# HSG-AIML/MaskedSST

Measured on AMD Instinct MI355X. Metric: pretrain samples/sec, higher is better.
Workload: dtype bf16; 1 GPU; SimMIM pretrain step (fwd+bwd+AdamW), EnMAP-shape cubes 8x8x200, depth 12x2, dim 96, heads 8, mlp 64, mask 0.7/4/tube, dropout 0.1; global_batch=256, per_gpu_batch=256, parallelism=dp1

## Files before the change

include/msst.h:

```cpp
#ifndef MSST_H
#define MSST_H
#include <stdint.h>

#ifdef __cplusplus
extern "C" {
#endif

#define MSST_VERSION 109
#define MSST_DIM 96
#define MSST_DIM_HEAD 64
#define MSST_MLP 64

#define MSST_PREC_F32 0
#define MSST_PREC_BF16 1

#define MSST_KERNEL_GENERIC (16 << 8)
#define MSST_KERNEL_FWD_4WAVE (64 << 8)
#define MSST_X1_BF16 (1024 << 8)
#define MSST_FWD_HALF (4096 << 8)
#define MSST_LSE_RENORM (8192 << 8)
#define MSST_LN1_FROM_XN (2048 << 8)
#define MSST_BWD_DEFER_REDUCE (512 << 8)
#define MSST_KERNEL_ATTN_R3 (128 << 8)

// ... 37 lines not shown
} MsstBlockWeights;

int msst_tokenize_fwd(const float* img, const float* pre_g, const float* pre_b, const float* w_emb,
                      const float* b_emb, const float* post_g, const float* post_b, const float* pos_a,
                      const float* pos_b, int pos_split, const float* mask_token, const uint8_t* mask,
                      float* out, int B, int S, int N, int P, float emb_dropout_p, uint32_t seed, void* stream);

int msst_tokenize_scene_fwd(const float* scene, const float* pre_g, const float* pre_b, const float* w_emb,
                            const float* b_emb, const float* post_g, const float* post_b, const float* pos_a,
                            const float* pos_b, int pos_split, float* out, int Bs, int Hs, int Ws, int window, int stride,
                            long win0, int nwin, int S, int P, void* stream);

int msst_tokenize_scene_fwd_train(const float* scene, const float* pre_g, const float* pre_b, const float* w_emb,
                                  const float* b_emb, const float* post_g, const float* post_b, const float* pos_a,
                                  const float* pos_b, int pos_split, float* out, int Bs, int Hs, int Ws, int window, int stride,
                                  long win0, int nwin, int S, int P, float emb_dropout_p, uint32_t seed, void* stream);
int msst_tokenize_scene_bwd(const float* scene, const float* pre_g, const float* pre_b, const float* w_emb,
                            const float* b_emb, const float* post_g, const float* post_b, const float* dx0, float* slab,
                            int nchunk, float* dpre_g, float* dpre_b, float* dw_emb, float* db_emb, float* dpost_g,
                            float* dpost_b, float* dpos_a, float* dpos_b, int pos_split, int Bs, int Hs, int Ws, int window,
                            int stride, long win0, int nwin, int S, int P, float emb_dropout_p, uint32_t seed, void* stream);

int msst_scene_assemble(const float* win_logits, long win0, int nwin, float* logits, int64_t* classes, int Bs,
                        int n_classes, int Hs, int Ws, int window, int stride, int finalize, void* stream);

int msst_tokenize_scene_fwd_masked(const float* scene, const float* pre_g, const float* pre_b, const float* w_emb,
                                   const float* b_emb, const float* post_g, const float* post_b, const float* pos_a,
                                   const float* pos_b, int pos_split, const float* mask_token, const uint8_t* scene_mask, float* out,
                                   int Bs, int Hs, int Ws, int window, int stride, long win0, int nwin, int S, int P, void* stream);

int msst_scene_recon_assemble(const float* win_recon, long win0, int nwin, const float* scene, const uint8_t* scene_mask, float* cube,
                              double* band_err , int32_t* band_cnt , int32_t* cover, int Bs, int S, int P,
                              int Hs, int Ws, int window, int stride, int finalize, int blend, void* stream);

int msst_pool_spectral_fwd(const float* y, float* out, int B, int S, int N, void* stream);

int msst_scene_embed_assemble(const float* win_feat, long win0, int nwin, float* feat, int32_t* cover, int Bs, int D, int Hs, int Ws,
                              int window, int stride, int finalize, int l2norm, void* stream);

#define MSST_SAVED_XN 1
#define MSST_SAVED_LSE 2
#define MSST_SAVED_RSTD 4
long msst_block_lse_floats(int mode, int B, int S, int N, int heads);
long msst_block_tiles(int mode, int B, int S, int N);
int msst_block_fwd(const MsstBlockWeights* w , const float* x, float* y, float* x1, int mode,
                   int B, int S, int N, int heads, int prec, int max_grid, float dropout_p, uint32_t seed,
                   int layer, void* xn_out, float* lse_out, int* saved , void* stream);

int msst_block_fwd_stack(const MsstBlockWeights* const* w , int nblk, const float* x0, float* const* y ,
                         float* const* x1 , void* const* xn_out , float* const* lse_out , int mode,
                         int B, int S, int N, int heads, int prec, int max_grid, float dropout_p, uint32_t seed, int layer0,
                         int* saved , void* stream);

int msst_head_fwd(const float* y, const float* img, const int32_t* idx, const float* w_pix,
                  const float* b_pix, int per_block, float* dpred, float* pred, float* partial,
                  float* loss, int B, int S, int N, int P, int K, void* stream);

int msst_recon_fwd(const float* y, const float* img, const uint8_t* mask, const float* w_pix, const float* b_pix, int per_block,
                   int blend, float* recon, double* band_err , int32_t* band_cnt , int B, int S, int N,
                   int P, void* stream);


int msst_head_bwd(const float* y, const float* dpred, const int32_t* csr_ptr, const int32_t* csr_pos,
                  const float* w_pix, int per_block, float gscale, const float* gout, float* dy, float* slab,
                  int nchunk, float* dw_pix, float* db_pix, int B, int S, int N, int P, int K, void* stream);

typedef struct MsstBlockGrads {
    float* ln1_g; float* ln1_b; float* wqkv; float* wout; float* bo;
    float* ln2_g; float* ln2_b; float* w1; float* b1; float* w2; float* b2;
} MsstBlockGrads;

#define MSST_MLP_SLAB (64 * 96 + 96 * 64 + 64 + 96 + 96 + 96)
#define MSST_ATTN_SLAB (3 * 64 * 96 + 96 * 64)
#define MSST_LN1_SLAB 288

int msst_block_bwd(const MsstBlockWeights* w , const MsstBlockGrads* g , const float* x,
                   const float* x1, const float* dy, float* dx, float* dx1, void* dxn_part, float* slab,
                   int grid_rows, int nchunk, int mode, int B, int S, int N, int heads, int prec,
                   float dropout_p, uint32_t seed, int layer, const void* xn_saved ,
                   const float* lse_saved ,
                   void* dab_ws ,
                   void* stream);

#define MSST_TILE_QUEUE_WORDS 64
int msst_block_bwd_chain(const MsstBlockWeights* w , const MsstBlockGrads* g ,
                         const MsstBlockWeights* w_prev , const MsstBlockGrads* g_prev ,
                         const float* x, const float* x1, const float* x1_prev, const float* dy, float* dx, float* dx1,
                         void* dxn_part, float* slab, int grid_rows, int nchunk, int mode, int B, int S, int N, int heads,
                         int prec, float dropout_p, uint32_t seed, int layer, const void* xn_saved, const float* lse_saved ,
                         void* dab_ws, int first, int32_t* tile_queue , void* stream);

int msst_block_bwd_reduce(const MsstBlockGrads* g , const MsstBlockGrads* g_prev ,
                          float* slab, long slab_stride, long grad_stride, int count, int count_prev, int first,
                          int grid_rows, int nchunk, int mode, int B, int S, int N, int heads, int prec, void* stream);

int msst_tokenize_bwd(const float* img, const float* pre_g, const float* pre_b, const float* w_emb,
                      const float* b_emb, const float* post_g, const float* post_b, const uint8_t* mask,
                      const float* dx0, float* slab, int nchunk, float* dpre_g, float* dpre_b,
                      float* dw_emb, float* db_emb, float* dpost_g, float* dpost_b, float* dpos_a,
                      float* dpos_b, int pos_split, float* dmask_token, int B, int S, int N, int P,
                      float emb_dropout_p, uint32_t seed, void* stream);

int msst_tokenize_bwd_input(const float* img, const float* pre_g, const float* pre_b, const float* w_emb, const float* b_emb,
                            const float* post_g, const float* post_b, const uint8_t* mask , const float* dx0,
                            const float* dtarget , float* dimg, int B, int S, int N, int P, float emb_dropout_p,
                            uint32_t seed, void* stream);
int msst_head_bwd_target(const float* dpred, const int32_t* csr_ptr, const int32_t* csr_pos, const float* gout ,
                         float* dtarget, int B, int S, int N, int P, int K, void* stream);
int msst_tokenize_scene_bwd_input(const float* scene, const float* pre_g, const float* pre_b, const float* w_emb, const float* b_emb,
                                  const float* post_g, const float* post_b, const float* dx0, float* dscene, int Bs, int Hs, int Ws,
                                  int window, int stride, long win0, int nwin, int S, int P, float emb_dropout_p, uint32_t seed,
                                  void* stream);

int msst_cls_head_fwd(const float* y, const float* ln_g, const float* ln_b, const float* w, const float* b,
                      float* logits, int B, int S, int N, int n_classes, void* stream);
int msst_cls_head_bwd(const float* y, const float* dlogits, const float* ln_g, const float* ln_b, const float* w,
                      float* dy, float* slab, float* dln_g, float* dln_b, float* dw, float* db, int B, int S,
                      int N, int n_classes, void* stream);

int msst_spec_head_fwd(const float* y, const float* ln_g, const float* ln_b, const float* w, const float* b,
                       float* logits, int B, int S, int N, int n_classes, void* stream);
long msst_spec_head_bwd_slab(int B, int S, int N, int n_classes);
int msst_spec_head_bwd(const float* y, const float* dlogits, const float* ln_g, const float* ln_b, const float* w,
                       float* dy, float* slab, float* dln_g, float* dln_b, float* dw, float* db, int B, int S,
                       int N, int n_classes, void* stream);

long msst_pix_head_fwd_ws(int B, int N);
int msst_pix_head_fwd(const float* y, const float* ln_g, const float* ln_b, const float* w, const float* b, float* logits,
                      float* ws, int B, int S, int N, int n_classes, void* stream);
long msst_pix_head_bwd_slab(int B, int S, int N, int n_classes);
int msst_pix_head_bwd(const float* y, const float* dlogits, const float* ln_g, const float* ln_b, const float* w, float* dy,
                      float* slab, float* dln_g, float* dln_b, float* dw, float* db, int B, int S, int N, int n_classes,
                      void* stream);

int msst_scene_centre_assemble(const float* win_logits, long win0, int nwin, float* logits, int64_t* classes, int Bs,
                               int n_classes, int Hs, int Ws, int window, int stride, int finalize, void* stream);

int msst_layernorm_fwd(const float* x, const float* gamma, const float* beta, float* y, float* mean ,
                       float* rstd , long rows, int D, float eps, void* stream);
long msst_layernorm_bwd_slab(long rows, int D);
int msst_layernorm_bwd(const float* x, const float* gamma, const float* dy, float* dx, float* dgamma, float* dbeta,
                       float* slab, long rows, int D, float eps, void* stream);

// ... 54 lines not shown
```

maskedsst_amd/_lib.py:

```python
import ctypes
import os
from ctypes import c_int, c_int32, c_uint32, c_long, c_float, c_void_p, c_char_p, POINTER, Structure

HERE = os.path.dirname(os.path.abspath(__file__))
LIB_PATH = os.path.join(HERE, "libmsst.so")
HEADER_PATH = os.path.normpath(os.path.join(HERE, "..", "include", "msst.h"))

PREC_F32 = 0
PREC_BF16 = 1
MODE_SPATIAL = 0
MODE_SPECTRAL = 1
MLP_SLAB = 64 * 96 + 96 * 64 + 64 + 96 + 96 + 96
ATTN_SLAB = 3 * 64 * 96 + 96 * 64
LN1_SLAB = 288


class MsstError(RuntimeError):
    pass


class MsstPrepJob(Structure):
    _fields_ = [("src", c_void_p), ("dst", c_void_p), ("rows", c_int32), ("cols", c_int32),
                ("transpose", c_int32), ("pack", c_int32), ("scale_rows", c_int32), ("scale", c_float)]


class MsstBlockWeights(Structure):
    _fields_ = [("struct_bytes", ctypes.c_uint64)] + [(n, c_void_p) for n in (
        "wqkv", "wout", "w1", "w2", "wqkvT", "woutT", "w1T", "w2T",
        "ln1_g", "ln1_b", "bo", "ln2_g", "ln2_b", "b1", "b2", "wqkv32", "woutT32", "wqkvT32",
        "wqkv_h", "wout_h", "w1_h", "w2_h")]


class MsstBlockGrads(Structure):
    _fields_ = [(n, c_void_p) for n in (
        "ln1_g", "ln1_b", "wqkv", "wout", "bo", "ln2_g", "ln2_b", "w1", "b1", "w2", "b2")]


class MsstAdamGroup(Structure):
    _fields_ = [("start", c_long), ("end", c_long), ("lr", c_float), ("weight_decay", c_float), ("step", c_int), ("flags", c_int)]


_P = c_void_p
ADAM_DECOUPLED = 1
ADAM_MAX_GROUPS = 64
BWD_DEFER_REDUCE = 512 << 8
X1_BF16 = 1024 << 8
SAVED_XN, SAVED_LSE, SAVED_RSTD = 1, 2, 4
LN1_FROM_XN = 2048 << 8
FWD_HALF = 4096 << 8
LSE_RENORM = 8192 << 8
PREP_HALF = 256
CE_LOSS_SUM, CE_N_VALID, CE_N_CORRECT, CE_BAD_LABELS, CE_NONFINITE, CE_SUPPORT = range(6)
CE_EXT_LOSS_SUM, CE_EXT_WEIGHT_SUM = range(2)
CE_CONFUSION_MAX_CLASSES = 128
_SIGS = {
    "msst_version": (c_int, []),
    "msst_last_error": (c_char_p, []),
    "msst_prep_weights": (c_int, [_P, c_int, c_int, c_int, c_int, _P, _P]),
    "msst_tokenize_fwd": (c_int, [_P] * 9 + [c_int, _P, _P, _P, c_int, c_int, c_int, c_int, c_float, c_uint32, _P]),
    "msst_tokenize_scene_fwd": (c_int, [_P] * 9 + [c_int, _P, c_int, c_int, c_int, c_int, c_int, c_long, c_int, c_int, c_int, _P]),
    "msst_tokenize_scene_fwd_train": (c_int, [_P] * 9 + [c_int, _P, c_int, c_int, c_int, c_int, c_int, c_long, c_int, c_int, c_int,
                                              c_float, c_uint32, _P]),
    "msst_tokenize_scene_bwd": (c_int, [_P] * 9 + [c_int] + [_P] * 8 + [c_int] * 6 + [c_long, c_int, c_int, c_int, c_float, c_uint32, _P]),
    "msst_tokenize_bwd_input": (c_int, [_P] * 11 + [c_int] * 4 + [c_float, c_uint32, _P]),
    "msst_head_bwd_target": (c_int, [_P] * 5 + [c_int] * 5 + [_P]),
    "msst_tokenize_scene_bwd_input": (c_int, [_P] * 9 + [c_int] * 5 + [c_long, c_int, c_int, c_int, c_float, c_uint32, _P]),
    "msst_tokenize_scene_fwd_masked": (c_int, [_P] * 9 + [c_int, _P, _P, _P, c_int, c_int, c_int, c_int, c_int, c_long, c_int, c_int, c_int, _P]),
    "msst_scene_recon_assemble": (c_int, [_P, c_long, c_int, _P, _P, _P, _P, _P, _P] + [c_int] * 9 + [_P]),
    "msst_pool_spectral_fwd": (c_int, [_P, _P, c_int, c_int, c_int, _P]),
    "msst_scene_embed_assemble": (c_int, [_P, c_long, c_int, _P, _P] + [c_int] * 8 + [_P]),
    "msst_scene_assemble": (c_int, [_P, c_long, c_int, _P, _P, c_int, c_int, c_int, c_int, c_int, c_int, c_int, _P]),
    "msst_cls_head_fwd": (c_int, [_P] * 6 + [c_int, c_int, c_int, c_int, _P]),
    "msst_cls_head_bwd": (c_int, [_P] * 11 + [c_int, c_int, c_int, c_int, _P]),
    "msst_spec_head_fwd": (c_int, [_P] * 6 + [c_int, c_int, c_int, c_int, _P]),
    "msst_spec_head_bwd_slab": (c_long, [c_int, c_int, c_int, c_int]),
    "msst_spec_head_bwd": (c_int, [_P] * 11 + [c_int, c_int, c_int, c_int, _P]),
    "msst_pix_head_fwd_ws": (c_long, [c_int, c_int]),
    "msst_pix_head_fwd": (c_int, [_P] * 7 + [c_int, c_int, c_int, c_int, _P]),
    "msst_pix_head_bwd_slab": (c_long, [c_int, c_int, c_int, c_int]),
    "msst_pix_head_bwd": (c_int, [_P] * 11 + [c_int, c_int, c_int, c_int, _P]),
    "msst_scene_centre_assemble": (c_int, [_P, c_long, c_int, _P, _P, c_int, c_int, c_int, c_int, c_int, c_int, c_int, _P]),
    "msst_block_lse_floats": (c_long, [c_int, c_int, c_int, c_int, c_int]),
    "msst_block_tiles": (c_long, [c_int, c_int, c_int, c_int]),
    "msst_block_fwd": (c_int, [POINTER(MsstBlockWeights), _P, _P, _P, c_int, c_int, c_int, c_int, c_int,
                               c_int, c_int, c_float, c_uint32, c_int, _P, _P, POINTER(c_int), _P]),
    "msst_block_fwd_stack": (c_int, [_P, c_int, _P, _P, _P, _P, _P, c_int, c_int, c_int, c_int, c_int, c_int, c_int, c_float, c_uint32, c_int,
                                     POINTER(c_int), _P]),
    "msst_head_fwd": (c_int, [_P, _P, _P, _P, _P, c_int, _P, _P, _P, _P, c_int, c_int, c_int, c_int,
                              c_int, _P]),
    "msst_head_bwd": (c_int, [_P, _P, _P, _P, _P, c_int, c_float, _P, _P, _P, c_int, _P, _P, c_int, c_int, c_int,
                              c_int, c_int, _P]),
    "msst_block_bwd": (c_int, [POINTER(MsstBlockWeights), POINTER(MsstBlockGrads), _P, _P, _P, _P, _P, _P, _P,
                               c_int, c_int, c_int, c_int, c_int, c_int, c_int, c_int, c_float, c_uint32, c_int, _P, _P, _P, _P]),
    "msst_block_bwd_chain": (c_int, [POINTER(MsstBlockWeights), POINTER(MsstBlockGrads), POINTER(MsstBlockWeights),
                                     POINTER(MsstBlockGrads), _P, _P, _P, _P, _P, _P, _P, _P,
                                     c_int, c_int, c_int, c_int, c_int, c_int, c_int, c_int, c_float, c_uint32, c_int, _P, _P, _P,
                                     c_int, _P, _P]),
    "msst_block_bwd_reduce": (c_int, [POINTER(MsstBlockGrads), POINTER(MsstBlockGrads), _P, ctypes.c_long, ctypes.c_long,
                                      c_int, c_int, c_int, c_int, c_int, c_int, c_int, c_int, c_int, c_int, c_int, _P]),
    "msst_tokenize_bwd": (c_int, [_P] * 10 + [c_int] + [_P] * 8 + [c_int, _P, c_int, c_int, c_int, c_int, c_float,
                                  c_uint32, _P]),
    "msst_debug_stamps": (c_int, [_P]),
    "msst_debug_cu_thief": (c_int, [c_int, c_int, _P, _P]),
    "msst_debug_box_probe": (c_int, [_P, _P, c_long, _P]),
    "msst_profile_enable": (c_int, [c_int]),
    "msst_profile_select": (c_int, [ctypes.c_ulonglong]),
    "msst_profile_sample": (c_int, [c_int]),
    "msst_profile_kernels": (c_int, []),
    "msst_profile_name": (c_char_p, [c_int]),
    "msst_profile_collect": (c_int, [_P, _P]),
    "msst_layernorm_fwd": (c_int, [_P, _P, _P, _P, _P, _P, c_long, c_int, c_float, _P]),
    "msst_layernorm_bwd_slab": (c_long, [c_long, c_int]),
    "msst_layernorm_bwd": (c_int, [_P, _P, _P, _P, _P, _P, _P, c_long, c_int, c_float, _P]),
    "msst_ce_scratch_bytes": (c_long, [c_int, c_int, c_int]),
    "msst_ce_stats_fwd": (c_int, [_P, _P, _P, c_long, _P, _P, _P, _P, c_int, c_int, c_int, _P]),
    "msst_ce_bwd": (c_int, [_P, _P, _P, _P, c_int, c_int, c_int, _P]),
    "msst_ce_ext_scratch_bytes": (c_long, [c_int, c_int, c_int, c_int]),
    "msst_ce_ext_fwd": (c_int, [_P, _P, _P, c_long, _P, c_float, _P, _P, _P, _P, _P, _P, c_int, c_int, c_int, _P]),
    "msst_ce_ext_bwd": (c_int, [_P, _P, _P, _P, c_int, c_int, c_int, _P]),
    "msst_recon_fwd": (c_int, [_P, _P, _P, _P, _P, c_int, c_int, _P, _P, _P, c_int, c_int, c_int, c_int, _P]),
    "msst_adamw": (c_int, [_P, _P, _P, _P, c_long, c_float, c_float, c_float, c_float, c_float, c_int,
                           c_float, c_float, _P]),
    "msst_adam_groups": (c_int, [_P, _P, _P, _P, POINTER(MsstAdamGroup), c_int, c_int, ctypes.c_double, ctypes.c_double,
                                 c_float, c_float, _P]),
}

_lib = None


def declared_symbols():
    return sorted(_SIGS)


def header_version(path=None):
    import re
    with open(path or HEADER_PATH) as f:
        m = re.search(r"^#define\s+MSST_VERSION\s+(\d+)", f.read(), re.M)
    if not m:
        raise MsstError(f"no MSST_VERSION in {path or HEADER_PATH}")
    return int(m.group(1))


def load():
    global _lib
    if _lib is not None:
        return _lib
    if not os.path.exists(LIB_PATH):
        raise MsstError(
            f"{LIB_PATH} not found: build the HIP extension first (python -m maskedsst_amd.build). "
            "maskedsst_amd has no CPU / eager fallback.")
# ... 26 lines not shown
```

maskedsst_amd/csrc/msst_api.hip:

```cpp
#include "../../include/msst.h"
#include "msst_kernels.h"
#include <stdio.h>
#include <stdlib.h>
#include <string.h>
#include <math.h>
#include <atomic>
#include <mutex>
#include <vector>

namespace msst {

static thread_local char g_err[256] = "";

static int fail(int code, const char* what) {
    if (code > 0) snprintf(g_err, sizeof(g_err), "%s: hip error %d (%s)", what, code, hipGetErrorString((hipError_t)code));
    else if (code < 0) snprintf(g_err, sizeof(g_err), "%s: msst error %d", what, code);
    return code;
}

template <class E>
__global__ __launch_bounds__(256) void prep_weights_kernel(const MsstPrepJob* jobs, int* err_flag) {
    const MsstPrepJob j = jobs[blockIdx.y];
    const bool half = sizeof(E) == 2 && (j.pack & MSST_PREP_HALF);
    if (j.pack < 0 || (j.pack & ~MSST_PREP_HALF) > 1 || (sizeof(E) != 2 && (j.pack & MSST_PREP_HALF)) || j.rows < 1 || j.cols < 1) {
// ... 373 lines not shown
        const long rows = s1 * Hs + r1 * stride + window - a.row0;
        rc = launch_scene_recon_accumulate(a, rows * Ws, st);
    }
    if (!rc && finalize) rc = launch_scene_recon_finalize(a, st);
    return fail(rc, "msst_scene_recon_assemble");
}

int msst_pool_spectral_fwd(const float* y, float* out, int B, int S, int N, void* stream) {
    if (B < 1 || S < 1 || N < 1) return fail(MSST_ERR_BADARG, "msst_pool_spectral_fwd");
    if (N > 64 || S > 64) return fail(MSST_ERR_UNSUPPORTED, "msst_pool_spectral_fwd (N <= 64, S <= 64)");
    if (!y || !out || ((uintptr_t)y & 15)) return fail(MSST_ERR_BADARG, "msst_pool_spectral_fwd (null argument, or y not 16-byte aligned)");
    return fail(launch_pool_spectral(y, out, B, S, N, (hipStream_t)stream), "msst_pool_spectral_fwd");
}

int msst_scene_embed_assemble(const float* win_feat, long win0, int nwin, float* feat, int32_t* cover, int Bs, int D, int Hs, int Ws,
                              int window, int stride, int finalize, int l2norm, void* stream) {
    if (Bs < 1 || D < 1 || Hs < 1 || Ws < 1 || window < 1 || stride < 1 || nwin < 0 || win0 < 0)
        return fail(MSST_ERR_BADARG, "msst_scene_embed_assemble");
    if (stride > window || window > Hs || window > Ws || window * window > 64 || D > 128)
        return fail(MSST_ERR_UNSUPPORTED, "msst_scene_embed_assemble (1 <= stride <= window <= Hs, Ws; window * window <= 64, D <= 128)");
    if ((nwin > 0 && !win_feat) || !feat || (finalize && !cover)) return fail(MSST_ERR_BADARG, "msst_scene_embed_assemble (null argument)");
    int nr = 0, nq = 0;
    scene_grid(Bs, Hs, Ws, window, stride, &nr, &nq);
    const long wps = (long)nr * nq;
    if (win0 + nwin > (long)Bs * wps) return fail(MSST_ERR_BADARG, "msst_scene_embed_assemble (windows out of range)");
    if (((long)Bs * Hs * Ws + 255) / 256 > 0x7fffffffL) return fail(MSST_ERR_UNSUPPORTED, "msst_scene_embed_assemble (scene batch too large)");
    SceneEmbedArgs a;
    a.win_feat = win_feat; a.feat = feat; a.cover = cover; a.win0 = win0; a.row0 = 0; a.nwin = nwin; a.Bs = Bs; a.D = D; a.Hs = Hs;
    a.Ws = Ws; a.win = window; a.stride = stride; a.nr = nr; a.nq = nq; a.l2norm = l2norm != 0;
    hipStream_t st = (hipStream_t)stream;
    int rc = 0;
    if (nwin > 0) {
        const long g0 = win0, g1 = win0 + nwin - 1;
        const long s0 = g0 / wps, s1 = g1 / wps;
        const long r0 = (g0 - s0 * wps) / nq, r1 = (g1 - s1 * wps) / nq;
        a.row0 = s0 * Hs + r0 * stride;
        const long rows = s1 * Hs + r1 * stride + window - a.row0;
        rc = launch_scene_embed_accumulate(a, rows * Ws, st);
    }
    if (!rc && finalize) rc = launch_scene_embed_finalize(a, st);
    return fail(rc, "msst_scene_embed_assemble");
}

long msst_block_lse_floats(int mode, int B, int S, int N, int heads) {
    if (B < 1 || S < 1 || N < 1 || heads < 1 || N > 64 || S > 64) return 0;
    return (long)ntiles_of(make_tilemap(mode, B, S, N)) * heads * 64 + (long)B * S * N;
}

long msst_block_tiles(int mode, int B, int S, int N) {
    if (B < 1 || S < 1 || N < 1 || N > 64 || S > 64) return 0;
    return (long)ntiles_of(make_tilemap(mode, B, S, N));
}

int msst_block_fwd(const MsstBlockWeights* w, const float* x, float* y, float* x1, int mode, int B, int S,
                   int N, int heads, int prec, int max_grid, float dropout_p, uint32_t seed, int layer,
                   void* xn_out, float* lse_out, int* saved, void* stream) {
    if (int rc = block_shape(mode, B, S, N, heads)) return fail(rc, "msst_block_fwd (B, S, N, heads < 1, mode not 0 / 1, or sequence length > 64)");
    if (!bw_ok(w) || !x || !y || x == y) return fail(MSST_ERR_BADARG, "msst_block_fwd (null argument, or MsstBlockWeights of another header revision)");
    const int dbg = (prec >> 8) & 0xffff;
    prec &= 0xff;
    BlockArgs a;
    a.w = to_bw(w);
    a.x = x; a.y = y; a.x1 = x1;
    a.tm = make_tilemap(mode, B, S, N);
    a.ntiles = ntiles_of(a.tm);
    a.max_grid = max_grid > 0 ? max_grid : a.ntiles;
    a.H = heads;
    a.scale = 0.125f;
    a.dbg = dbg & ~8;
    a.stamps = nullptr;
#ifdef MSST_STAMPS
    a.stamps = g_stamps;
    if (g_stamps) a.dbg = dbg;
#elif defined(MSST_LAB)
    a.stamps = g_stamps;
#endif
    a.x1_bf16 = (dbg & 1024) ? 1 : 0;
    if (a.x1_bf16 && !(prec == MSST_PREC_BF16 && heads == 8 && !(dbg & (16 | 64))))
        return fail(MSST_ERR_UNSUPPORTED, "msst_block_fwd (MSST_X1_BF16 needs the role-split bf16 forward: 8 heads, no MSST_KERNEL_* flags)");
    a.half = (dbg & 4096) ? 1 : 0;
    if (a.half) {
        if (!(prec == MSST_PREC_BF16 && heads == 8 && !(dbg & (16 | 64))))
            return fail(MSST_ERR_UNSUPPORTED, "msst_block_fwd (MSST_FWD_HALF needs the role-split bf16 forward: 8 heads, no MSST_KERNEL_* flags)");
        if (!w->wqkv_h || !w->wout_h || !w->w1_h || !w->w2_h) return fail(MSST_ERR_BADARG, "msst_block_fwd (MSST_FWD_HALF without the half weight copies)");
        a.w.wqkv = w->wqkv_h; a.w.wout = w->wout_h; a.w.w1 = w->w1_h; a.w.w2 = w->w2_h;
    }
    a.drop = make_drop(dropout_p, seed, layer);
    a.xn_out = (xn_out && block_fwd_writes_xn(a, prec)) ? xn_out : nullptr;
    a.lse_out = (lse_out && block_fwd_writes_lse(a, prec)) ? lse_out : nullptr;
    if (saved) *saved = (a.xn_out ? MSST_SAVED_XN : 0) | (a.lse_out ? (MSST_SAVED_LSE | MSST_SAVED_RSTD) : 0);
    return fail(launch_block_fwd(a, prec, (hipStream_t)stream), "msst_block_fwd");
}

int msst_block_fwd_stack(const MsstBlockWeights* const* w, int nblk, const float* x0, float* const* y, float* const* x1,
                         void* const* xn_out, float* const* lse_out, int mode, int B, int S, int N, int heads, int prec, int max_grid,
                         float dropout_p, uint32_t seed, int layer0, int* saved, void* stream) {
    if (int rc = block_shape(mode, B, S, N, heads)) return fail(rc, "msst_block_fwd_stack (B, S, N, heads < 1, mode not 0 / 1, or sequence length > 64)");
    if (!w || !x0 || !y || nblk < 1) return fail(MSST_ERR_BADARG, "msst_block_fwd_stack");
    if (nblk > MSST_MAX_STACK) return fail(MSST_ERR_UNSUPPORTED, "msst_block_fwd_stack (more than 16 blocks)");
    const int dbg = (prec >> 8) & 0xffff;
    prec &= 0xff;
    if (prec != MSST_PREC_BF16 || heads != 8 || (dbg & ~(1024 | 4096))) return fail(MSST_ERR_UNSUPPORTED, "msst_block_fwd_stack (bf16, 8 heads, no MSST_KERNEL_* flags)");
    const bool half = (dbg & 4096) != 0;
    for (int j = 0; j < nblk; ++j) {
        if (!bw_ok(w[j])) return fail(MSST_ERR_BADARG, "msst_block_fwd_stack (null block, or MsstBlockWeights of another header revision)");
        if (half && (!w[j]->wqkv_h || !w[j]->wout_h || !w[j]->w1_h || !w[j]->w2_h)) return fail(MSST_ERR_BADARG, "msst_block_fwd_stack (MSST_FWD_HALF without the half weight copies)");
    }
    StackArgs sa;
    BlockArgs& a = sa.base;
    memset(&a.w, 0, sizeof(a.w));
    a.x = x0; a.y = nullptr; a.x1 = nullptr; a.xn_out = nullptr; a.lse_out = nullptr;
    a.tm = make_tilemap(mode, B, S, N);
    a.ntiles = ntiles_of(a.tm);
    a.max_grid = max_grid > 0 ? max_grid : a.ntiles;
    a.H = heads;
    a.scale = 0.125f;
    a.dbg = 0;
    a.stamps = nullptr;
    a.x1_bf16 = (dbg & 1024) ? 1 : 0;
    a.half = half ? 1 : 0;
    a.drop = make_drop(dropout_p, seed, layer0);
    if (lse_out && !block_fwd_writes_lse(a, prec)) lse_out = nullptr;
    sa.nblk = nblk;
    auto blk_of = [&](int j, const float* xin) {
        StackBlk sb;
        sb.wqkv = half ? w[j]->wqkv_h : w[j]->wqkv; sb.wout = half ? w[j]->wout_h : w[j]->wout;
        sb.w1 = half ? w[j]->w1_h : w[j]->w1; sb.w2 = half ? w[j]->w2_h : w[j]->w2;
        sb.ln1_g = w[j]->ln1_g; sb.ln1_b = w[j]->ln1_b; sb.bo = w[j]->bo; sb.ln2_g = w[j]->ln2_g; sb.ln2_b = w[j]->ln2_b; sb.b1 = w[j]->b1; sb.b2 = w[j]->b2;
        sb.x = xin; sb.y = y[j]; sb.x1 = x1 ? x1[j] : nullptr; sb.xn_out = xn_out ? xn_out[j] : nullptr; sb.lse_out = lse_out ? lse_out[j] : nullptr;
        sb.layer = layer0 + j; sb.pad_ = 0;
        return sb;
    };
    for (int j = 0; j < nblk; ++j)
        if (!bw_ok(w[j]) || !y[j] || y[j] == (j ? y[j - 1] : x0))
            return fail(MSST_ERR_BADARG, "msst_block_fwd_stack (null argument, or MsstBlockWeights of another header revision)");
    sa.b0 = blk_of(0, x0);
    memset(&sa.st, 0, sizeof(sa.st));
    bool affine = true;
    if (nblk > 1) {
        const StackBlk b1 = blk_of(1, y[0]);
        auto dist = [&](const void* p1, const void* p0, int& out) {
            const long d = (const char*)p1 - (const char*)p0;
            if (d > 0x7fffffffL || d < -0x7fffffffL) affine = false;
            out = (int)d;
        };
        dist(b1.wqkv, sa.b0.wqkv, sa.st.wqkv); dist(b1.wout, sa.b0.wout, sa.st.wout); dist(b1.w1, sa.b0.w1, sa.st.w1); dist(b1.w2, sa.b0.w2, sa.st.w2);
        dist(b1.ln1_g, sa.b0.ln1_g, sa.st.ln1_g); dist(b1.ln1_b, sa.b0.ln1_b, sa.st.ln1_b); dist(b1.bo, sa.b0.bo, sa.st.bo);
        dist(b1.ln2_g, sa.b0.ln2_g, sa.st.ln2_g); dist(b1.ln2_b, sa.b0.ln2_b, sa.st.ln2_b); dist(b1.b1, sa.b0.b1, sa.st.b1); dist(b1.b2, sa.b0.b2, sa.st.b2);
        dist(b1.y, sa.b0.y, sa.st.y); dist(b1.x1, sa.b0.x1, sa.st.x1); dist(b1.xn_out, sa.b0.xn_out, sa.st.xn_out); dist(b1.lse_out, sa.b0.lse_out, sa.st.lse_out);
        sa.st.x = sa.st.y;
        const float* xin = y[0];
        for (int j = 1; j < nblk && affine; ++j) {
            const StackBlk bj = blk_of(j, xin);
            auto same = [&](const void* pj, const void* p0, int stride) { return !p0 ? !pj : (const char*)pj == (const char*)p0 + (long)j * stride; };
            affine = same(bj.wqkv, sa.b0.wqkv, sa.st.wqkv) && same(bj.wout, sa.b0.wout, sa.st.wout) && same(bj.w1, sa.b0.w1, sa.st.w1) &&
                     same(bj.w2, sa.b0.w2, sa.st.w2) && same(bj.ln1_g, sa.b0.ln1_g, sa.st.ln1_g) && same(bj.ln1_b, sa.b0.ln1_b, sa.st.ln1_b) &&
                     same(bj.bo, sa.b0.bo, sa.st.bo) && same(bj.ln2_g, sa.b0.ln2_g, sa.st.ln2_g) && same(bj.ln2_b, sa.b0.ln2_b, sa.st.ln2_b) &&
                     same(bj.b1, sa.b0.b1, sa.st.b1) && same(bj.b2, sa.b0.b2, sa.st.b2) && same(bj.y, sa.b0.y, sa.st.y) &&
                     same(bj.x1, sa.b0.x1, sa.st.x1) && same(bj.xn_out, sa.b0.xn_out, sa.st.xn_out) && same(bj.lse_out, sa.b0.lse_out, sa.st.lse_out);
            xin = y[j];
        }
    }
    if (!affine) return fail(MSST_ERR_UNSUPPORTED, "msst_block_fwd_stack (per-block operands not a constant stride apart)");
    sa.x_rest = nblk > 1 ? reinterpret_cast<const float*>(reinterpret_cast<const char*>(y[0]) - (long)sa.st.y) : x0;
    if (saved) *saved = (xn_out ? MSST_SAVED_XN : 0) | (lse_out ? (MSST_SAVED_LSE | MSST_SAVED_RSTD) : 0);
    if (a.ntiles < 1) return 0;
    int ncu = 256, dev = 0;
    hipGetDevice(&dev);
    if (hipDeviceGetAttribute(&ncu, hipDeviceAttributeMultiprocessorCount, dev) != hipSuccess || ncu < 1) ncu = 256;
    int grid = a.max_grid < a.ntiles ? a.max_grid : a.ntiles;
    if (grid > ncu) grid = ncu;
    return fail(launch_block_fwd_rs_stack(sa, grid, (hipStream_t)stream), "msst_block_fwd_stack");
}

int msst_head_fwd(const float* y, const float* img, const int32_t* idx, const float* w_pix,
                  const float* b_pix, int per_block, float* dpred, float* pred, float* partial,
                  float* loss, int B, int S, int N, int P, int K, void* stream) {
    HeadArgs a;
    a.y = y; a.img = img; a.idx = idx; a.w_pix = w_pix; a.b_pix = b_pix; a.dpred = dpred; a.pred = pred;
    a.partial = partial; a.B = B; a.S = S; a.N = N; a.T = S * N; a.P = P; a.K = K; a.per_block = per_block;
    return fail(launch_head_fwd(a, loss, (hipStream_t)stream), "msst_head_fwd");
}

int msst_head_bwd(const float* y, const float* dpred, const int32_t* csr_ptr, const int32_t* csr_pos,
                  const float* w_pix, int per_block, float gscale, const float* gout, float* dy, float* slab,
                  int nchunk, float* dw_pix, float* db_pix, int B, int S, int N, int P, int K, void* stream) {
    if (nchunk < 1) return fail(MSST_ERR_BADARG, "msst_head_bwd");
    hipStream_t st = (hipStream_t)stream;
    HeadBwdArgs a;
    a.y = y; a.dpred = dpred; a.csr_ptr = csr_ptr; a.csr_pos = csr_pos; a.w_pix = w_pix; a.dy = dy; a.slab = slab;
    a.gscale = gscale; a.gout = gout; a.B = B; a.S = S; a.N = N; a.T = S * N; a.P = P; a.K = K; a.per_block = per_block;
    int rc = launch_head_bwd(a, nchunk, st);
    if (rc) return fail(rc, "msst_head_bwd");
    const long ss = (long)P * 96 + P;
    RSegBuilder rb;
    bool ok = true;
    if (per_block) {
        for (int c = 0; c < S && ok; ++c) {
            ok = rb.add(slab + (long)c * nchunk * ss, ss, nchunk, dw_pix + (long)c * P * 96, P * 96);
            ok = ok && rb.add(slab + (long)c * nchunk * ss + P * 96, ss, nchunk, db_pix + (long)c * P, P);
            if (rb.r.nseg > MSST_MAX_RSEG - 2 && c + 1 < S) {
                rc = launch_reduce_segs(rb.r, st);
                if (rc) return fail(rc, "msst_head_bwd(reduce)");
                rb = RSegBuilder();
            }
        }
    } else {
        ok = rb.add(slab, ss, S * nchunk, dw_pix, P * 96);
        ok = ok && rb.add(slab + P * 96, ss, S * nchunk, db_pix, P);
    }
    if (!ok) return fail(MSST_ERR_UNSUPPORTED, "msst_head_bwd(reduce table)");
    rc = launch_reduce_segs(rb.r, st);
    return fail(rc, "msst_head_bwd(reduce)");
}

struct SlabLayout {
    int grid, grid_mlp, nc;
    float *mlp, *attn, *ln1, *mlp_prev;
};
static SlabLayout slab_layout(float* slab, long ntok, int grid_rows, int nchunk, int ntiles_attn, int heads, int prec) {
    SlabLayout l;
    const int ntiles_rows = (int)((ntok + 63) / 64);
    l.grid = grid_rows < ntiles_rows ? grid_rows : ntiles_rows;
    const int gmlp2 = (prec == MSST_PREC_BF16 && PBF16::WAVES_BWD_MLP == 2) ? 2 * grid_rows : grid_rows;
    l.grid_mlp = gmlp2 < ntiles_rows ? gmlp2 : ntiles_rows;
    l.nc = nchunk < ntiles_attn ? nchunk : ntiles_attn;
    l.mlp = slab;
    l.attn = l.mlp + (long)l.grid_mlp * MSST_MLP_SLAB_N;
    l.ln1 = l.attn + (long)l.nc * heads * MSST_ATTN_SLAB_N;
    l.mlp_prev = l.ln1 + (long)l.grid * MSST_LN1_SLAB;
    return l;
}
static int reduce_block_slabs(const SlabLayout& lay, int heads, const MsstBlockGrads* g, const MsstBlockGrads* g_mlp, int ny_mlp,
                              const MsstBlockGrads* g_prev, int ny_prev, int ny, long src_ystride, long dst_ystride, hipStream_t st) {
    RSegBuilder rb;
    auto fresh = [&]() { rb = RSegBuilder(); rb.r.src_ystride = src_ystride; rb.r.dst_ystride = dst_ystride; };
    fresh();
    const long ms = MSST_MLP_SLAB_N;
    bool ok = true;
    auto add_mlp = [&](const float* sm_, int nslab, const MsstBlockGrads* gg, int nyy) {
        ok = ok && rb.add(sm_, ms, nslab, gg->w1, 6144, 0, 0, nyy);
        ok = ok && rb.add(sm_ + 6144, ms, nslab, gg->w2, 6144, 0, 0, nyy);
        ok = ok && rb.add(sm_ + 12288, ms, nslab, gg->b1, 64, 0, 0, nyy);
        ok = ok && rb.add(sm_ + 12288 + 64, ms, nslab, gg->b2, 96, 0, 0, nyy);
        ok = ok && rb.add(sm_ + 12288 + 160, ms, nslab, gg->ln2_g, 96, 0, 0, nyy);
        ok = ok && rb.add(sm_ + 12288 + 256, ms, nslab, gg->ln2_b, 96, 0, 0, nyy);
    };
    if (g_mlp) add_mlp(lay.mlp, lay.grid_mlp, g_mlp, ny_mlp);
    if (g_prev) add_mlp(lay.mlp_prev, lay.grid, g_prev, ny_prev);
    if (g) {
        ok = ok && rb.add(lay.ln1, 288, lay.grid, g->ln1_g, 96, 0, 0, ny);
        ok = ok && rb.add(lay.ln1 + 96, 288, lay.grid, g->ln1_b, 96, 0, 0, ny);
        ok = ok && rb.add(lay.ln1 + 192, 288, lay.grid, g->bo, 96, 0, 0, ny);
        const long as = (long)heads * MSST_ATTN_SLAB_N;
        const int inner = heads * 64;
        for (int h = 0; h < heads && ok; ++h) {
            const float* sh = lay.attn + (long)h * MSST_ATTN_SLAB_N;
            for (int which = 0; which < 3 && ok; ++which)
                ok = rb.add(sh + which * 6144, as, lay.nc, g->wqkv + ((long)(which * heads + h) * 64) * 96, 6144, 0, 0, ny);
            ok = ok && rb.add(sh + 3 * 6144, as, lay.nc, g->wout + h * 64, 6144, 64, inner, ny);
            if (rb.r.nseg > MSST_MAX_RSEG - 4 && h + 1 < heads) {
                int rc = launch_reduce_segs(rb.r, st);
                if (rc) return rc;
                fresh();
            }
        }
    }
    if (!ok) return MSST_ERR_UNSUPPORTED;
    return launch_reduce_segs(rb.r, st);
}

static int block_bwd_impl(const MsstBlockWeights* w, const MsstBlockGrads* g, const MsstBlockWeights* w_prev,
                          const MsstBlockGrads* g_prev, const float* x, const float* x1, const float* x1_prev,
                          const float* dy, float* dx, float* dx1, void* dxn_part, float* slab, int grid_rows,
                          int nchunk, int mode, int B, int S, int N, int heads, int prec, float dropout_p,
                          uint32_t seed, int layer, const void* xn_saved, const float* lse_saved, void* dab_ws, int chain, int first,
                          int32_t* tile_queue, hipStream_t st) {
    if (int rc = block_shape(mode, B, S, N, heads)) return fail(rc, "msst_block_bwd (B, S, N, heads < 1, mode not 0 / 1, or sequence length > 64)");
    if (!bw_ok(w) || (w_prev && !bw_ok(w_prev)) || !g || grid_rows < 1 || nchunk < 1)
        return fail(MSST_ERR_BADARG, "msst_block_bwd (null argument, or MsstBlockWeights of another header revision)");
    const int dbg = (prec >> 8) & 0xffff;
    prec &= 0xff;
    const long ntok = (long)B * S * N;
    const BlockWeights bw = to_bw(w);
    const Drop drop = make_drop(dropout_p, seed, layer);
    AttnBwdArgs aa;
    aa.tm = make_tilemap(mode, B, S, N);
    aa.ntiles = ntiles_of(aa.tm);
    const SlabLayout lay = slab_layout(slab, ntok, grid_rows, nchunk, aa.ntiles, heads, prec);
    const int grid = lay.grid, grid_mlp = lay.grid_mlp, nc = lay.nc;
    float* slab_mlp = lay.mlp;
    float* slab_attn = lay.attn;
    float* slab_ln1 = lay.ln1;
    float* slab_mlp_prev = lay.mlp_prev;
    const bool fast_rows = xn_saved && dab_ws && prec == MSST_PREC_BF16 && !(dbg & 16);
    if (chain && (!fast_rows || (w_prev && (!g_prev || !x1_prev)) || (first && !dy) || (!w_prev && !dx)))
        return fail(MSST_ERR_BADARG, "msst_block_bwd_chain (bf16 with saved LN1 rows and the dab workspace only)");
    const bool run_mlp = !chain || first;
    const int x1b = (dbg & 1024) ? 1 : 0;
    if (x1b && prec != MSST_PREC_BF16)
        return fail(MSST_ERR_UNSUPPORTED, "msst_block_bwd (MSST_X1_BF16 needs the bf16 kernels)");
    if (tile_queue) {
        hipError_t e = hipMemsetAsync(tile_queue, 0, MSST_TILE_QUEUE_WORDS * sizeof(int32_t), st);
        if (e != hipSuccess) return fail((int)e, "msst_block_bwd_chain(tile queue)");
    }
    if (run_mlp) {
        MlpBwdArgs a;
        a.w = bw; a.x1 = x1; a.dy = dy; a.dx1 = dx1; a.slab = slab_mlp; a.ntok = ntok; a.drop = drop;
        a.dab = fast_rows ? dab_ws : nullptr;
        a.x1_bf16 = x1b;
        int rc = launch_block_bwd_mlp(a, grid_mlp, prec, st);
        if (rc) return fail(rc, "msst_block_bwd(mlp)");
    }
    int nparts = heads;
    {
        aa.w = bw; aa.x = x; aa.da = dx1; aa.dxn_part = dxn_part; aa.slab = slab_attn;
        aa.xn = fast_rows ? xn_saved : nullptr; aa.dab = fast_rows ? dab_ws : nullptr;
        aa.H = heads; aa.ntok = ntok; aa.scale = 0.125f; aa.drop = drop;
        aa.queue = (tile_queue && heads / 2 <= 32) ? tile_queue : nullptr;
        aa.lse = fast_rows ? lse_saved : nullptr;
        aa.lse_renorm = (dbg & 8192) ? 1 : 0;
        aa.dbg = dbg & ~8;
        aa.stamps = nullptr;
#ifdef MSST_STAMPS
        aa.stamps = g_stamps;
        if (g_stamps) aa.dbg = dbg;
#elif defined(MSST_LAB)
        aa.stamps = g_stamps;
#endif
        int rc = launch_block_bwd_attn(aa, nc, prec, st, &nparts);
        if (rc) return fail(rc, "msst_block_bwd(attn)");
    }
    const bool fused = chain && w_prev;
    if (fused) {
        if (nparts > 4) return fail(MSST_ERR_UNSUPPORTED, "msst_block_bwd_chain (more than four d(LN1 out) partials)");
        LnMlpArgs a;
        a.w = to_bw(w_prev); a.ln1_g = w->ln1_g; a.x = x; a.dx1 = dx1; a.dxn_part = dxn_part; a.x1 = x1_prev; a.dab = dab_ws;
        a.x1_bf16 = x1b;
        a.xn = nullptr; a.rstd = nullptr; a.ln1_b = w->ln1_b;
        if (dbg & 2048) {
            if (!xn_saved || !lse_saved) return fail(MSST_ERR_BADARG, "msst_block_bwd_chain (MSST_LN1_FROM_XN needs xn_saved and lse_saved)");
            a.xn = xn_saved; a.rstd = lse_saved + (long)aa.ntiles * heads * 64;
        }
        a.slab_mlp = slab_mlp_prev; a.slab_ln1 = slab_ln1; a.ntok = ntok; a.nparts = nparts;
        a.drop_i = drop; a.drop_p = make_drop(dropout_p, seed, layer - 1);
        a.stamps = nullptr;
#ifdef MSST_STAMPS
        a.stamps = g_stamps;
#endif
        a.queue = tile_queue ? tile_queue + 32 : nullptr;
        int rc = launch_block_bwd_ln1mlp(a, grid, st);
        if (rc) return fail(rc, "msst_block_bwd_chain(ln1 + mlp)");
    } else {
        Ln1BwdArgs a;
        a.x = x; a.dx1 = dx1; a.dxn_part = dxn_part; a.ln1_g = w->ln1_g; a.dx = dx; a.slab = slab_ln1; a.ntok = ntok; a.H = nparts; a.drop = drop;
        int rc = launch_block_bwd_ln1(a, grid, prec, st);
        if (rc) return fail(rc, "msst_block_bwd(ln1)");
    }
    if (!(chain && (dbg & 512))) {
        int rc = reduce_block_slabs(lay, heads, g, run_mlp ? g : nullptr, 1, fused ? g_prev : nullptr, 1, 1, 0, 0, st);
        if (rc) return fail(rc, "msst_block_bwd(reduce)");
    }
    return 0;
}

int msst_block_bwd(const MsstBlockWeights* w, const MsstBlockGrads* g, const float* x, const float* x1,
                   const float* dy, float* dx, float* dx1, void* dxn_part, float* slab, int grid_rows,
                   int nchunk, int mode, int B, int S, int N, int heads, int prec, float dropout_p,
                   uint32_t seed, int layer, const void* xn_saved, const float* lse_saved, void* dab_ws, void* stream) {
    return block_bwd_impl(w, g, nullptr, nullptr, x, x1, nullptr, dy, dx, dx1, dxn_part, slab, grid_rows, nchunk, mode, B, S, N,
                          heads, prec, dropout_p, seed, layer, xn_saved, lse_saved, dab_ws, 0, 0, nullptr, (hipStream_t)stream);
}

int msst_block_bwd_chain(const MsstBlockWeights* w, const MsstBlockGrads* g, const MsstBlockWeights* w_prev,
                         const MsstBlockGrads* g_prev, const float* x, const float* x1, const float* x1_prev,
                         const float* dy, float* dx, float* dx1, void* dxn_part, float* slab, int grid_rows,
                         int nchunk, int mode, int B, int S, int N, int heads, int prec, float dropout_p,
                         uint32_t seed, int layer, const void* xn_saved, const float* lse_saved, void* dab_ws, int first,
                         int32_t* tile_queue, void* stream) {
    return block_bwd_impl(w, g, w_prev, g_prev, x, x1, x1_prev, dy, dx, dx1, dxn_part, slab, grid_rows, nchunk, mode, B, S, N,
                          heads, prec, dropout_p, seed, layer, xn_saved, lse_saved, dab_ws, 1, first, tile_queue, (hipStream_t)stream);
}

int msst_block_bwd_reduce(const MsstBlockGrads* g, const MsstBlockGrads* g_prev, float* slab, long slab_stride, long grad_stride,
                          int count, int count_prev, int first, int grid_rows, int nchunk, int mode, int B, int S, int N, int heads,
                          int prec, void* stream) {
    if (int rc = block_shape(mode, B, S, N, heads)) return fail(rc, "msst_block_bwd_reduce (B, S, N, heads < 1, mode not 0 / 1, or sequence length > 64)");
    if (!g || count < 1 || count_prev < 0 || count_prev > count || (count_prev && !g_prev) || !slab || grid_rows < 1 || nchunk < 1 ||
        (count > 1 && ((slab_stride & 3) || (grad_stride & 3))))
        return fail(MSST_ERR_BADARG, "msst_block_bwd_reduce");
    prec &= 0xff;
    const long ntok = (long)B * S * N;
    const TileMap tm = make_tilemap(mode, B, S, N);
    const SlabLayout lay = slab_layout(slab, ntok, grid_rows, nchunk, ntiles_of(tm), heads, prec);
    return fail(reduce_block_slabs(lay, heads, g, first ? g : nullptr, 1, count_prev ? g_prev : nullptr, count_prev, count,
                                   slab_stride, grad_stride, (hipStream_t)stream), "msst_block_bwd_reduce");
}

static int tokenize_bwd_reduce(float* slab, int nchunk, float* dpre_g, float* dpre_b, float* dw_emb, float* db_emb, float* dpost_g,
                               float* dpost_b, float* dpos_a, float* dpos_b, int pos_split, float* dmask_token, int S, int N, int P,
                               hipStream_t st) {
    int rc = 0;
    const long ss = (long)N * 96 + 96 * P + 96 * 4 + 32;
    const long bs = (long)nchunk * ss;
    float* stage = slab + (long)S * nchunk * ss;
    float* dpos_dst = pos_split ? stage : dpos_a;
    const long v0 = (long)N * 96 + 96 * P;
    RSegBuilder rb;
    bool ok = true;
    for (int c = 0; c < S && ok; ++c) {
        const float* sc = slab + c * bs;
        if (dpos_a) ok = rb.add(sc, ss, nchunk, dpos_dst + (long)c * N * 96, N * 96);
        ok = ok && rb.add(sc + N * 96, ss, nchunk, dw_emb + (long)c * 96 * P, 96 * P);
        ok = ok && rb.add(sc + v0, ss, nchunk, db_emb + (long)c * 96, 96);
        if (rb.r.nseg > MSST_MAX_RSEG - 8) {
            rc = launch_reduce_segs(rb.r, st);
            if (rc) return fail(rc, "msst_tokenize_bwd(reduce)");
            rb = RSegBuilder();
        }
    }
    ok = ok && rb.add(slab + v0 + 96, ss, S * nchunk, dpost_g, 96);
    ok = ok && rb.add(slab + v0 + 192, ss, S * nchunk, dpost_b, 96);
    if (dmask_token) ok = ok && rb.add(slab + v0 + 288, ss, S * nchunk, dmask_token, 96);
    ok = ok && rb.add(slab + v0 + 384, ss, S * nchunk, dpre_g, P);
    ok = ok && rb.add(slab + v0 + 384 + 16, ss, S * nchunk, dpre_b, P);
    if (!ok) return fail(MSST_ERR_UNSUPPORTED, "msst_tokenize_bwd(reduce table)");
    rc = launch_reduce_segs(rb.r, st);
    if (!rc && pos_split && dpos_a) rc = launch_pos_split(stage, S, N, pos_split, dpos_a, dpos_b, st);
    return fail(rc, "msst_tokenize_bwd(reduce)");
}

int msst_tokenize_bwd(const float* img, const float* pre_g, const float* pre_b, const float* w_emb,
                      const float* b_emb, const float* post_g, const float* post_b, const uint8_t* mask,
                      const float* dx0, float* slab, int nchunk, float* dpre_g, float* dpre_b,
// ... 410 lines not shown
```

maskedsst_amd/csrc/msst_bwd4.hip:

```cpp
#include <atomic>
#include "msst_dev.h"
#include "msst_kernels.h"
#include <type_traits>

#ifndef MSST_B3_D3A
#define MSST_B3_D3A 2
#endif
#ifndef MSST_B3_D3B
#define MSST_B3_D3B 5
#endif
#ifndef MSST_B3_D4
#define MSST_B3_D4 3
#endif
#ifndef MSST_B3_W4
#define MSST_B3_W4 6
#endif
#ifndef MSST_B3_W1AT
#define MSST_B3_W1AT 8
#endif
#if defined(MSST_LAB) && !defined(MSST_LAB_EXP)
#define MSST_LAB_EXP 0
#endif
#ifndef MSST_B4_LAG
#define MSST_B4_LAG 2
#endif
#ifndef MSST_B4_PRA
#define MSST_B4_PRA 0x0011
#endif
#ifndef MSST_B4_PRB
#define MSST_B4_PRB 0x0011
#endif
#define B4_PRIO(ph) do { if (grp) __builtin_amdgcn_s_setprio((MSST_B4_PRB >> (4 * (4 - (ph)))) & 3); \
                         else __builtin_amdgcn_s_setprio((MSST_B4_PRA >> (4 * (4 - (ph)))) & 3); } while (0)

namespace msst {

namespace {

typedef float f32x16 __attribute__((ext_vector_type(16)));
typedef __bf16 hbf16x8 __attribute__((ext_vector_type(8)));
typedef __attribute__((address_space(3))) char lds_char;
typedef __attribute__((address_space(3))) s16x4 lds_s16x4;
typedef __attribute__((address_space(3))) s16x8 lds_s16x8;
typedef __attribute__((address_space(3))) u32x4 lds_u32x4;

constexpr int R4_ROWBUF = 24576, R4_DA = 12288;
constexpr int R4_G0 = 49152, R4_GSZ = 49152;
constexpr int R3_Q = 0, R3_K = 8192, R3_DO = 16384, R3_V = 24576, R3_P = 32768, R3_DS = 40960;
constexpr int R4_OUT = 147456, R4_MAP = 159744, R4_SEQ = 160000, R4_SEQO = 160272, R4_QT = 160272 + 272, R4_LSE = R4_QT + 16, R4_SMEM = R4_LSE + 1024;

__device__ __forceinline__ int fz(int r) { return (((r >> 1) & 1) << 2) | ((((r >> 2) ^ (r >> 3)) & 1) << 1) | ((r >> 3) & 1); }
__device__ __forceinline__ int fz2(int r) { return (((r >> 3) & 1) << 1) | ((r >> 2) & 1); }

__device__ __forceinline__ s16x8 lds_r128(lds_char* b, unsigned off) { return *reinterpret_cast<const lds_s16x8*>(b + off); }
__device__ __forceinline__ void lds_w64(lds_char* b, unsigned off, s16x4 v) { *reinterpret_cast<lds_s16x4*>(b + off) = v; }
__device__ __forceinline__ s16x8 lds_tr2(lds_char* b, unsigned off0, unsigned off1) {
    const s16x4 lo = __builtin_amdgcn_ds_read_tr16_b64_v4i16(reinterpret_cast<lds_s16x4*>(b + off0));
    const s16x4 hi = __builtin_amdgcn_ds_read_tr16_b64_v4i16(reinterpret_cast<lds_s16x4*>(b + off1));
    s16x8 r;
    r[0] = lo[0]; r[1] = lo[1]; r[2] = lo[2]; r[3] = lo[3];
    r[4] = hi[0]; r[5] = hi[1]; r[6] = hi[2]; r[7] = hi[3];
    return r;
}

__device__ __forceinline__ f32x16 mma32(s16x8 a, s16x8 b, f32x16 c) {
    return __builtin_amdgcn_mfma_f32_32x32x16_bf16(__builtin_bit_cast(hbf16x8, a), __builtin_bit_cast(hbf16x8, b), c, 0, 0, 0);
}
__device__ __forceinline__ f32x16 zero16() {
    f32x16 z;
#pragma unroll
    for (int i = 0; i < 16; ++i) z[i] = 0.f;
    return z;
}
__device__ __forceinline__ s16x4 pk4(const f32x16& c, int q4) {
    f32x4 t = {c[4 * q4], c[4 * q4 + 1], c[4 * q4 + 2], c[4 * q4 + 3]};
    return f2bf4(t);
}
__device__ __forceinline__ s16x8 pk8(const f32x16& c, int k0) {
    const s16x4 a = pk4(c, 2 * k0), b = pk4(c, 2 * k0 + 1);
    s16x8 r;
    r[0] = a[0]; r[1] = a[1]; r[2] = a[2]; r[3] = a[3];
    r[4] = b[0]; r[5] = b[1]; r[6] = b[2]; r[7] = b[3];
    return r;
}
__device__ __forceinline__ s16x8 ld_w32b(const void* w, int base_bytes, int imm_bytes, int lane16) {
    const __amdgpu_buffer_rsrc_t rs = __builtin_amdgcn_make_buffer_rsrc(const_cast<void*>(w), 0, 0x7fffffff, 0x00020000);
    return __builtin_bit_cast(s16x8, __builtin_amdgcn_raw_buffer_load_b128(rs, lane16 + imm_bytes, base_bytes, 0));
}
__device__ __forceinline__ int launder_s(int v) {
    asm volatile("" : "+s"(v));
    return v;
}
__device__ __forceinline__ void dma16(__amdgpu_buffer_rsrc_t rs, unsigned lds_dst, unsigned voff) {
    asm volatile("s_mov_b32 m0, %0\n\tbuffer_load_dwordx4 %1, %2, 0 offen lds" :: "s"(lds_dst), "v"(voff), "s"(rs) : "memory", "m0");
}
__device__ __forceinline__ void bar3() {
    lds_barrier();
}
__device__ __forceinline__ int launder3(int v) {
    asm volatile("" : "+v"(v));
    return v;
}

__device__ __forceinline__ s16x8 ident32_frag(int f, int i, int hi) {
    const int e = i - 16 * f - 8 * hi;
    const unsigned one = 0x3F80u << ((e & 1) << 4), d = (unsigned)(e >> 1);
    u32x4 w;
#pragma unroll
    for (int k = 0; k < 4; ++k) w[k] = d == (unsigned)k ? one : 0u;
    return __builtin_bit_cast(s16x8, w);
}

}

template <bool DROP, bool QUEUE, int LSE>
__global__ __launch_bounds__(512, 1) void block_bwd_attn_r4_kernel(AttnBwdArgs a) {
    extern __shared__ __attribute__((aligned(16))) char smem_raw[];
    lds_char* const sm = (lds_char*)smem_raw;

    const int tid = threadIdx.x & 255, wv = __builtin_amdgcn_readfirstlane((int)threadIdx.x >> 6);
    const int grp = wv >> 2, wave = wv & 3;
    const int H = a.H, inner = H * 64, h = 2 * blockIdx.y + grp;
    const int gb = R4_G0 + grp * R4_GSZ;
    const TileMap tm = a.tm;
    const int L = tm.L;
    bf16_t* part = reinterpret_cast<bf16_t*>(a.dxn_part) + (long)blockIdx.y * a.ntok * 96;

    const bool roleO = wave == 3;
    const void* w1p = roleO ? a.w.woutT32 : a.w.wqkv32;
    const int f1_0 = ((roleO ? h * 64 : (wave * H + h) * 64) >> 5) * 6;
    const int f4_0 = (wave < 3 ? wave : 0) * ((3 * inner) >> 4) + ((h * 64) >> 4);
    const int p1_row = roleO ? R4_DA : 0;
    const int p1_out = gb + (wave == 0 ? R3_Q : wave == 1 ? R3_K : wave == 2 ? R3_V : R3_DO);
    const bool pathX = wave == 0 || wave == 3;
    const int p3_a1 = gb + ((wave == 0 || wave == 1) ? R3_DS : R3_P);
    const int p3_a2 = gb + (wave == 0 ? R3_K : wave == 1 ? R3_Q : wave == 2 ? R3_DO : R3_V);

    f32x16 G[2][3];
#pragma unroll
    for (int i = 0; i < 2; ++i)
#pragma unroll
        for (int j = 0; j < 3; ++j) G[i][j] = zero16();

    unsigned* const rowmap = reinterpret_cast<unsigned*>(smem_raw + R4_MAP);
    if (threadIdx.x < 64) {
        const int sq = tid / L, ps = tid - sq * L;
        rowmap[tid] = ((unsigned)((sq >= tm.TS ? 0xffff : sq) & 0xffff) << 16) | (unsigned)ps;
    }
    __syncthreads();
    int kvalid = 0;
    if (LSE && L < 64) {
        const int l_ = tid & 63, qr = 16 * wave + (l_ & 15);
        const int qlo_ = qr - (int)(rowmap[qr] & 0xffffu), qhi_ = qlo_ + L;
        for (int t = 0; t < 4; ++t)
            for (int r = 0; r < 4; ++r) { const int key = 16 * t + 4 * (l_ >> 4) + r; kvalid |= (int)(key >= qlo_ && key < qhi_) << (4 * t + r); }
    }
    unsigned need;
    {
        const int r0 = 16 * wave, r1 = 16 * wave + 15;
        const int klo = r0 - (int)(rowmap[r0] & 0xffffu), khi = min(63, r1 - (int)(rowmap[r1] & 0xffffu) + L - 1);
        unsigned m = 0;
        for (int t = 0; t < 4; ++t) m |= (unsigned)(16 * t <= khi && 16 * t + 15 >= klo) << t;
        need = (unsigned)__builtin_amdgcn_readfirstlane((int)m);
    }
    auto row_slot = [&](int j) -> unsigned {
        const int t_ = launder3(tid);
        const int row = t_ >> 2, s = 4 * j + (t_ & 3);
        return (unsigned)(row * 192 + (((s & ~3) | ((s & 3) ^ fz2(row))) << 4));
    };
    const __amdgpu_buffer_rsrc_t rows_x = __builtin_amdgcn_make_buffer_rsrc(const_cast<void*>(a.xn), 0, (int)(a.ntok * 192), 0x00020000);
    const __amdgpu_buffer_rsrc_t rows_d = __builtin_amdgcn_make_buffer_rsrc(const_cast<void*>(a.dab), 0, (int)(a.ntok * 192), 0x00020000);
    int* const seqbase = reinterpret_cast<int*>(smem_raw + R4_SEQ);
    int* const seqout = reinterpret_cast<int*>(smem_raw + R4_SEQO);
    auto fill_seqbase = [&](int* table, int tile_) {
        const int sx = launder3(tid) & 63;
        const int q = tile_ * tm.TS + sx;
        int base = -1;
        if (tile_ < a.ntiles && sx < tm.TS && q < tm.nseq) {
            if (tm.mode == 0) base = q * tm.N;
            else { const int b = tm.nshift >= 0 ? (q >> tm.nshift) : q / tm.N; base = b * tm.T + (q - b * tm.N); }
        }
        table[sx] = base;
    };
    int* const qt = reinterpret_cast<int*>(smem_raw + R4_QT);
    int qpend = 0;
    if (wv == 3) {
        int t0 = (int)blockIdx.x;
        if (QUEUE) {
            int r = 0;
            if ((tid & 63) == 0) { r = __hip_atomic_fetch_add(a.queue + blockIdx.y, 2, __ATOMIC_RELAXED, __HIP_MEMORY_SCOPE_AGENT); qt[0] = r; qt[1] = r + 1; }
            t0 = __builtin_amdgcn_readfirstlane(r);
        }
        fill_seqbase(seqbase, t0);
        if ((tid & 63) == 0) { seqbase[64] = -1; seqout[64] = -1; }
    }
    __syncthreads();
    unsigned rinv[3], rsx[3];
#pragma unroll
    for (int jj = 0; jj < 3; ++jj) {
        const int p = 192 * wave + 64 * jj + (tid & 63);
        const int row = p / 12, sl = p - 12 * row;
        const int s_ = (sl & ~3) | ((sl & 3) ^ fz2(row));
        const unsigned sp = rowmap[row];
        rsx[jj] = (unsigned)(R4_SEQ + 4 * min((int)(sp >> 16), 64));
        rinv[jj] = (sp & 0xffffu) * (unsigned)(tm.mode == 0 ? 192 : 192 * tm.N) + (unsigned)s_ * 16u;
    }
    const __amdgpu_buffer_rsrc_t lse_rs = __builtin_amdgcn_make_buffer_rsrc(const_cast<float*>(a.lse), 0, LSE ? (int)min((long)a.ntiles * H * 256, 0x7fffffffL) : 0, 0x00020000);
    auto dma_lse = [&](int tile_, int buf) {
        if (!LSE || wv != 0) return;
        const unsigned dst = (unsigned)(R4_LSE + (buf ? 512 : 0));
        const unsigned voff = tile_ < a.ntiles ? (unsigned)(((tile_ * H + 2 * (int)blockIdx.y) * 64 + (launder3(tid) & 63)) * 4) : 0x80000000u;
        asm volatile("s_mov_b32 m0, %0\n\tbuffer_load_dword %1, %2, 0 offen lds" :: "s"(dst), "v"(voff), "s"(lse_rs) : "memory", "m0");
        asm volatile("s_mov_b32 m0, %0\n\tbuffer_load_dword %1, %2, 0 offen lds" :: "s"(dst + 256), "v"(voff + 256u), "s"(lse_rs) : "memory", "m0");
    };
    auto dma_rows = [&](int buf) {
        int base[3];
#pragma unroll
        for (int jj = 0; jj < 3; ++jj) base[jj] = *reinterpret_cast<const __attribute__((address_space(3))) int*>(sm + rsx[jj]);
#pragma unroll
        for (int jj = 0; jj < 3; ++jj) {
            const int bs = base[jj];
            const unsigned voff = bs < 0 ? 0x80000000u : (unsigned)bs * 192u + rinv[jj];
            const unsigned dst = (unsigned)(buf + 3072 * wave + 1024 * jj);
            dma16(rows_x, dst, voff);
            dma16(rows_d, dst + R4_DA, voff);
        }
    };
    if (!grp) { dma_rows(0); dma_lse(QUEUE ? __builtin_amdgcn_readfirstlane(qt[0]) : (int)blockIdx.x, 0); wait_vm0(); }
    unsigned cinv, csx;
    {
        const unsigned sp = rowmap[tid >> 2];
        csx = (unsigned)(R4_SEQO + 4 * min((int)(sp >> 16), 64));
        cinv = (sp & 0xffffu) * (unsigned)(tm.mode == 0 ? 192 : 192 * tm.N) + (unsigned)(tid & 3) * 16u;
    }
    auto copy_out = [&]() {
        const int bs = *reinterpret_cast<const __attribute__((address_space(3))) int*>(sm + csx);
        u32x4 v[3];
#pragma unroll
        for (int j = 0; j < 3; ++j) v[j] = *reinterpret_cast<const lds_u32x4*>(sm + R4_OUT + row_slot(j));
        const __amdgpu_buffer_rsrc_t rp = __builtin_amdgcn_make_buffer_rsrc(part, 0, (int)(a.ntok * 192), 0x00020000);
        const unsigned voff = bs < 0 ? 0x80000000u : (unsigned)bs * 192u + cinv;
#pragma unroll
        for (int j = 0; j < 3; ++j) __builtin_amdgcn_raw_buffer_store_b128(v[j], rp, voff + 64 * j, 0, 0);
    };
    s16x8 w1[2][6];
    auto load_w1 = [&]() {
        const int l16 = (launder3(tid) & 63) * 16;
        const int b1 = launder_s(f1_0 * 1024);
#pragma unroll
        for (int dt = 0; dt < 2; ++dt)
#pragma unroll
            for (int ks = 0; ks < 6; ++ks) {
                const int fi = 6 * dt + ks;
                w1[dt][ks] = ld_w32b(w1p, b1 + (fi >> 2) * 4096, (fi & 3) * 1024, l16);
            }
    };
    load_w1();
    lds_barrier();
    if (grp) {
#pragma unroll
        for (int i = 0; i < MSST_B4_LAG; ++i) lds_barrier();
    }

    s16x8 idf_h[2];
    {
        const int t0_ = launder3(tid);
#pragma unroll
        for (int f2 = 0; f2 < 2; ++f2) idf_h[f2] = ident32_frag(f2, t0_ & 31, (t0_ >> 5) & 1);
    }
    int xb = 0;
    int ks = 0;
    for (int tile = QUEUE ? __builtin_amdgcn_readfirstlane(qt[0]) : (int)blockIdx.x; tile < a.ntiles;
         xb = R4_ROWBUF - xb, ++ks, tile = QUEUE ? __builtin_amdgcn_readfirstlane(qt[ks & 3]) : tile + (int)gridDim.x) {
        const int p1_in = xb + p1_row, p3_x = p1_in;
#if defined(MSST_STAMPS)
        const bool stamp_on = (a.dbg & 8) && a.stamps && blockIdx.x == 7 && blockIdx.y == 1 && (threadIdx.x & 63) == 0 && tile == (int)blockIdx.x + 20 * (int)gridDim.x;
#define R4_STAMP(i) do { if (stamp_on) a.stamps[16 * wv + (i)] = __builtin_readcyclecounter(); } while (0)
#else
#define R4_STAMP(i) do { } while (0)
#endif
        R4_STAMP(0);
        B4_PRIO(1);
        unsigned p2a[4];
        {
            const int t_ = launder3(tid);
            const int l31 = t_ & 31, hi = (t_ >> 5) & 1;
            const int f2v = fz2(l31);
            unsigned bin[2];
#pragma unroll
            for (int p = 0; p < 2; ++p) bin[p] = p1_in + l31 * 192 + (((hi ^ f2v) << 4) ^ (p << 5));
            f32x16 c[2][2];
#pragma unroll
            for (int i = 0; i < 2; ++i)
#pragma unroll
                for (int j = 0; j < 2; ++j) c[i][j] = zero16();
            const unsigned L7 = p1_out + l31 * 128 + (fz(l31) << 4) + 8 * hi;
            auto ep1 = [&](int rt, int i) {
                const int dt = i >> 2, q4 = i & 3;
                lds_w64(sm, (L7 ^ ((4 * dt + q4) << 4)) + rt * 4096, pk4(c[dt][rt], q4));
            };
            auto p2a_part = [&](int part) {
                const int l = t_ & 63, g = l >> 4, c16 = l & 15, fzc = fz(c16);
                if (part == 0) {
                    p2a[0] = gb + c16 * 128 + ((g ^ fzc) << 4);
                    p2a[1] = gb + c16 * 128 + (((4 + g) ^ fzc) << 4);
                    asm volatile("" : "+v"(p2a[0]));
                    asm volatile("" : "+v"(p2a[1]));
                } else {
                    p2a[2] = gb + (16 * wave + c16) * 128 + (((g >> 1) ^ fzc) << 4) + 8 * (g & 1);
                    p2a[3] = (unsigned)(16 * wave + c16 - (int)(rowmap[16 * wave + c16] & 0xffffu));
                    asm volatile("" : "+v"(p2a[2]));
                    asm volatile("" : "+v"(p2a[3]));
                }
            };
            s16x8 fb[4];
            auto rd1 = [&](int s_) {
                const int rt = s_ / 6, ks = s_ % 6;
                fb[s_ & 3] = lds_r128(sm, bin[ks & 1] + 64 * (ks >> 1) + rt * 32 * 192);
            };
#ifdef MSST_LAB
            if ((MSST_LAB_EXP & 1) && !roleO) { p2a_part(0); p2a_part(1); } else
#ifdef MSST_LAB_QKV
            if (a.stamps && !roleO) {
                p2a_part(0); p2a_part(1);
                const char* src = reinterpret_cast<const char*>(a.stamps) + ((long)(tile * H + h) * 3 + wave) * 8192 + (t_ & 63) * 16;
#pragma unroll
                for (int i = 0; i < 8; ++i) {
                    const unsigned dst = (unsigned)(size_t)sm + p1_out + i * 1024;
                    asm volatile("s_mov_b32 m0, %0\n\tglobal_load_lds_dwordx4 %1, off" :: "s"(dst), "v"(src + i * 1024) : "memory", "m0");
                }
            } else
#endif
#endif
            {
            rd1(0); rd1(1); rd1(2);
#pragma unroll
            for (int s_ = 0; s_ < 12; ++s_) {
                const int rt = s_ / 6, ks = s_ % 6;
                if (s_ + 3 < 12) rd1(s_ + 3);
                MSST_SCHED_FENCE();
                c[0][rt] = mma32(w1[0][ks], fb[s_ & 3], c[0][rt]);
                if (s_ == 2) p2a_part(0);
                if (s_ >= 7 && s_ <= 10) ep1(0, 2 * (s_ - 7));
                MSST_SCHED_FENCE();
                c[1][rt] = mma32(w1[1][ks], fb[s_ & 3], c[1][rt]);
                if (s_ == 3) p2a_part(1);
                if (s_ >= 7 && s_ <= 10) ep1(0, 2 * (s_ - 7) + 1);
                MSST_SCHED_FENCE();
            }
            R4_STAMP(12);
#pragma unroll
            for (int i = 0; i < 8; ++i) ep1(1, i);
            }
        }
        R4_STAMP(1);
        bar3();
        R4_STAMP(2);
        B4_PRIO(2);
        if (wv == 3) {
            fill_seqbase(seqbase, QUEUE ? qt[(ks + 1) & 3] : tile + (int)gridDim.x);
            if (QUEUE && (tid & 63) == 0) qpend = __hip_atomic_fetch_add(a.queue + blockIdx.y, 1, __ATOMIC_RELAXED, __HIP_MEMORY_SCOPE_AGENT);
        }
        if (wv == 7) fill_seqbase(seqout, tile);
        {
            typedef PBF16 P;
            const int t_ = launder3(tid);
            const int l = t_ & 63, g = l >> 4, c16 = l & 15;
            const int qlo = (int)p2a[3], qhi = qlo + L;
            unsigned ak[2], aq[2];
#pragma unroll
            for (int ks2 = 0; ks2 < 2; ++ks2) {
                ak[ks2] = p2a[ks2];
                aq[ks2] = ak[ks2] + wave * 2048;
            }
            const unsigned L8 = p2a[2];
            f32x4 pr[4], dp[4];
            f32x4 dm[4];
#pragma unroll
            for (int t = 0; t < 4; ++t) dm[t] = zero4();
            const float cs = a.scale * 1.44269504088896340736f;
            int kv_ = kvalid;
            asm volatile("" : "+v"(kv_));
            float lse2 = 0.f;
            if (LSE) lse2 = *reinterpret_cast<const __attribute__((address_space(3))) float*>(sm + R4_LSE + (xb ? 512 : 0) + grp * 256 + (16 * wave + c16) * 4);
            if (DROP) {
                const unsigned t16 = a.drop.thr << 16;
#pragma unroll
                for (int t = 0; t < 4; ++t) {
                    unsigned ha, hb;
                    drop_bits(a.drop, 1, (unsigned)(((tile * H + h) * 64 + wave * 16 + c16) * 16 + t * 4 + g), ha, hb);
                    dm[t][0] = (ha << 16) >= t16 ? a.drop.scale : 0.f;
                    dm[t][1] = ha >= t16 ? a.drop.scale : 0.f;
                    dm[t][2] = (hb << 16) >= t16 ? a.drop.scale : 0.f;
                    dm[t][3] = hb >= t16 ? a.drop.scale : 0.f;
                }
            }
            auto softmax_phase = [&](auto mode_tag) {
                constexpr int NM = decltype(mode_tag)::value;
                constexpr bool MASKED = NM >= 0;
                const unsigned nm = NM > 0 ? (unsigned)NM : NM == 0 ? need : 0xfu;
                auto on = [&](int t) { return NM < 0 || ((nm >> t) & 1u); };
                {
                    s16x8 fq[2], fk[2][4];
#pragma unroll
                    for (int ks2 = 0; ks2 < 2; ++ks2) {
                        fq[ks2] = lds_r128(sm, R3_Q + aq[ks2]);
#pragma unroll
                        for (int t = 0; t < 4; ++t) if (NM == 0 || on(t)) fk[ks2][t] = lds_r128(sm, R3_K + ak[ks2] + t * 2048);
                    }
#pragma unroll
                    for (int t = 0; t < 4; ++t) pr[t] = zero4();
#pragma unroll
                    for (int ks2 = 0; ks2 < 2; ++ks2)
// ... 83 lines not shown
                    for (int t = 0; t < 4; ++t) if (on(t)) lvl[n++] = dp[t];
                    if (NM == 0) {
                        dsum = (dp[0] + dp[1]) + (dp[2] + dp[3]);
                    } else {
                        dsum = n == 4 ? (lvl[0] + lvl[1]) + (lvl[2] + lvl[3]) : n == 3 ? (lvl[0] + lvl[1]) + lvl[2] : n == 2 ? lvl[0] + lvl[1] : lvl[0];
                    }
                }
                float delta = -colgroup_sum((dsum[0] + dsum[1]) + (dsum[2] + dsum[3]));
#pragma unroll
                for (int t = 0; t < 4; ++t) {
                    if (!on(t)) { lds_w64(sm, R3_DS + (L8 ^ (t << 5)), s16x4{0, 0, 0, 0}); continue; }
                    f32x4 d4;
#pragma unroll
                    for (int r = 0; r < 4; ++r) d4[r] = fmaf(pr[t][r], delta, dp[t][r]);
                    lds_w64(sm, R3_DS + (L8 ^ (t << 5)), f2bf4(d4));
                }
            };
            {
                if (L == 64) softmax_phase(std::integral_constant<int, -1>{});
                else switch (need) {
                    case 0x3: softmax_phase(std::integral_constant<int, 0x3>{}); break;
                    case 0x7: softmax_phase(std::integral_constant<int, 0x7>{}); break;
                    case 0xe: softmax_phase(std::integral_constant<int, 0xe>{}); break;
                    case 0xc: softmax_phase(std::integral_constant<int, 0xc>{}); break;
                    case 0x6: softmax_phase(std::integral_constant<int, 0x6>{}); break;
                    case 0xf: softmax_phase(std::integral_constant<int, 0xf>{}); break;
                    default: softmax_phase(std::integral_constant<int, 0>{}); break;
                }
            }
        }
        {
            s16x8 w4[MSST_B3_W4];
            const int t_ = launder3(tid);
            const int l = t_ & 63, l31 = l & 31, hi = l >> 5, i = l & 15, u = (l >> 4) & 1, b = (i >> 1) & 1, r1 = (i >> 3) & 1;
            const unsigned Lt = (8 * hi + (i >> 2)) * 128 + (((2 * u + b) ^ ((r1 << 2) | (hi << 1) | hi)) << 4) + 8 * (i & 1);
            unsigned tr[2][2];
#pragma unroll
            for (int ct = 0; ct < 2; ++ct)
#pragma unroll
                for (int aa = 0; aa < 2; ++aa) tr[ct][aa] = (Lt ^ ((ct << 6) | (aa << 5))) + 512 * aa;
            const unsigned a1 = p3_a1 + l31 * 128 + ((hi ^ fz(l31)) << 4);
            f32x16 c[2][2];
#pragma unroll
            for (int ii = 0; ii < 2; ++ii)
#pragma unroll
                for (int j = 0; j < 2; ++j) c[ii][j] = zero16();
            s16x8 pa[2][4];
            s16x8 fb0[4];
#pragma unroll
            for (int kk = 0; kk < 4; ++kk) fb0[kk] = lds_tr2(sm, p3_a2 + tr[0][0] + 2048 * kk, p3_a2 + tr[0][1] + 2048 * kk);
            R4_STAMP(3);
            bar3();
            R4_STAMP(4);
            if (!grp) { dma_rows(R4_ROWBUF - xb); dma_lse(QUEUE ? __builtin_amdgcn_readfirstlane(qt[(ks + 1) & 3]) : tile + (int)gridDim.x, R4_ROWBUF - xb); }
            B4_PRIO(3);
            auto phase3 = [&](auto role_tag) {
                constexpr int ROLE = decltype(role_tag)::value;
                constexpr bool PX = ROLE < 2, WR = ROLE != 1;
                s16x8 fa[4][2], fb1[4];
                auto issue_a = [&](int kk) {
                    if (PX) {
                        fa[kk][0] = lds_r128(sm, a1 ^ (kk << 5));
                        fa[kk][1] = lds_r128(sm, (a1 ^ (kk << 5)) + 4096);
                    } else {
                        fa[kk][0] = lds_tr2(sm, p3_a1 + tr[0][0] + 2048 * kk, p3_a1 + tr[0][1] + 2048 * kk);
                        fa[kk][1] = lds_tr2(sm, p3_a1 + tr[1][0] + 2048 * kk, p3_a1 + tr[1][1] + 2048 * kk);
                    }
                };
                const unsigned L7 = p3_a2 + l31 * 128 + (fz(l31) << 4) + 8 * hi;
                s16x4 q0[2][4];
                auto ep3 = [&](int ct, int q4) {
                    q0[ct][q4] = pk4(c[ct][0], q4);
                    asm volatile("" : "+v"(q0[ct][q4]));
                    if (WR) lds_w64(sm, (L7 ^ ((4 * ct + q4) << 4)), q0[ct][q4]);
                };
                s16x4 q1[4];
                auto ep3b = [&](int q4) {
                    q1[q4] = pk4(c[0][1], q4);
                    asm volatile("" : "+v"(q1[q4]));
                    if (WR) lds_w64(sm, (L7 ^ (q4 << 4)) + 4096, q1[q4]);
                };
                issue_a(0); issue_a(1);
#pragma unroll
                for (int st = 0; st < 16; ++st) {
                    const int tl = st >> 2, kk = st & 3, ct = tl & 1, dt = tl >> 1;
                    if (st + 2 < 4) issue_a(st + 2);
                    if (st < 4) fb1[st] = lds_tr2(sm, p3_a2 + tr[1][0] + 2048 * st, p3_a2 + tr[1][1] + 2048 * st);
                    MSST_SCHED_FENCE();
                    c[ct][dt] = mma32(fa[kk][ct], dt ? fb1[kk] : fb0[kk], c[ct][dt]);
                    if (tl == 1) ep3(0, kk);
                    if (tl == 2) ep3(1, kk);
                    if (tl == 3) ep3b(kk);
                    MSST_SCHED_FENCE();
                }
                R4_STAMP(11);
#pragma unroll
                for (int kk = 0; kk < 4; ++kk) {
                    s16x8 r;
                    const s16x4 lo = q0[kk >> 1][2 * (kk & 1)], hi4 = q0[kk >> 1][2 * (kk & 1) + 1];
                    r[0] = lo[0]; r[1] = lo[1]; r[2] = lo[2]; r[3] = lo[3];
                    r[4] = hi4[0]; r[5] = hi4[1]; r[6] = hi4[2]; r[7] = hi4[3];
                    pa[0][kk] = r;
                }
#pragma unroll
                for (int kk = 0; kk < 2; ++kk) {
                    s16x8 r;
                    const s16x4 lo = q1[2 * kk], hi4 = q1[2 * kk + 1];
                    r[0] = lo[0]; r[1] = lo[1]; r[2] = lo[2]; r[3] = lo[3];
                    r[4] = hi4[0]; r[5] = hi4[1]; r[6] = hi4[2]; r[7] = hi4[3];
                    pa[1][kk] = r;
                    pa[1][2 + kk] = pk8(c[1][1], kk);
                }
                if (WR) {
#pragma unroll
                    for (int q4 = 0; q4 < 4; ++q4) lds_w64(sm, (L7 ^ ((4 + q4) << 4)) + 4096, pk4(c[1][1], q4));
                }
            };
            if (wave == 0) phase3(std::integral_constant<int, 0>{});
            else if (wave == 3) phase3(std::integral_constant<int, 1>{});
            else phase3(std::integral_constant<int, 2>{});
            const unsigned L4 = (4 * hi + (i >> 2)) * 192 + (((2 * u + b) ^ hi) << 4) + 8 * (i & 1);
            unsigned tx[2];
#pragma unroll
            for (int aa = 0; aa < 2; ++aa) tx[aa] = p3_x + (L4 ^ (aa << 5)) + 8 * aa * 192;
            auto wgrad = [&](auto lo_c, auto hi_c) {
                constexpr int LO = decltype(lo_c)::value, HI = decltype(hi_c)::value;
                if constexpr (HI > LO) {
                    s16x8 fx[MSST_B3_D3B + 1];
                    swpipe<HI - LO, MSST_B3_D3B>(
                        [&](int s0) {
                            const int st = s0 + LO, kk = st / 3, mt = st % 3;
                            fx[s0 % (MSST_B3_D3B + 1)] = lds_tr2(sm, tx[0] + 3072 * kk + 64 * mt, tx[1] + 3072 * kk + 64 * mt);
                        },
                        [&](int s0) {
                            const int st = s0 + LO, kk = st / 3, mt = st % 3;
                            G[0][mt] = mma32(pa[0][kk], fx[s0 % (MSST_B3_D3B + 1)], G[0][mt]);
                            G[1][mt] = mma32(pa[1][kk], fx[s0 % (MSST_B3_D3B + 1)], G[1][mt]);
                        });
                }
            };
            const int l16 = l * 16;
            const int b4 = launder_s(roleO ? 0 : f4_0 * 1024), b4s = launder_s(roleO ? 0 : (inner >> 4) * 1024);
            auto ld_w4 = [&](int k12) -> s16x8 {
                return ld_w32b(a.w.wqkvT32, b4 + (k12 >> 2) * b4s, (k12 & 3) * 1024, l16);
            };
#pragma unroll
            for (int k12 = 0; k12 < MSST_B3_W4; ++k12) w4[k12] = ld_w4(k12);
            if (!grp && ks != 0) copy_out();
            R4_STAMP(5);
            bar3();
            R4_STAMP(6);
            B4_PRIO(4);
            wgrad(std::integral_constant<int, 0>{}, std::integral_constant<int, 12>{});
            R4_STAMP(9);
            if (roleO) {
                if (QUEUE && !grp && (tid & 63) == 0) qt[(ks + 2) & 3] = qpend;
                load_w1();
            } else {
                f32x16 c4[2];
                c4[0] = zero16(); c4[1] = zero16();
                if (grp) {
                    s16x8 fs[2][2], idf[2];
#pragma unroll
                    for (int rt = 0; rt < 2; ++rt)
#pragma unroll
                        for (int f2 = 0; f2 < 2; ++f2)
                            fs[rt][f2] = lds_r128(sm, R4_OUT + (32 * rt + l31) * 192 + ((4 * wave + ((2 * f2 + hi) ^ fz2(l31))) << 4));
#pragma unroll
                    for (int f2 = 0; f2 < 2; ++f2) idf[f2] = idf_h[f2];
#pragma unroll
                    for (int f2 = 0; f2 < 2; ++f2) {
                        c4[0] = mma32(idf[f2], fs[0][f2], c4[0]);
                        c4[1] = mma32(idf[f2], fs[1][f2], c4[1]);
                    }
                }
                s16x8 fb4[MSST_B3_D4 + 1][2];
                swpipe<12, MSST_B3_D4>(
                    [&](int k12) {
                        const int which = k12 >> 2, ks = k12 & 3;
                        const int reg = gb + (which == 0 ? R3_K : which == 1 ? R3_Q : R3_DO);
                        fb4[k12 % (MSST_B3_D4 + 1)][0] = lds_tr2(sm, reg + tr[0][0] + 2048 * ks, reg + tr[0][1] + 2048 * ks);
                        fb4[k12 % (MSST_B3_D4 + 1)][1] = lds_tr2(sm, reg + tr[1][0] + 2048 * ks, reg + tr[1][1] + 2048 * ks);
                    },
                    [&](int k12) {
                        c4[0] = mma32(w4[k12 % MSST_B3_W4], fb4[k12 % (MSST_B3_D4 + 1)][0], c4[0]);
                        c4[1] = mma32(w4[k12 % MSST_B3_W4], fb4[k12 % (MSST_B3_D4 + 1)][1], c4[1]);
                        if (k12 + MSST_B3_W4 < 12) w4[k12 % MSST_B3_W4] = ld_w4(k12 + MSST_B3_W4);
                        if (k12 == MSST_B3_W1AT) load_w1();
                    });
                R4_STAMP(10);
                const unsigned L9 = R4_OUT + l31 * 192 + (fz2(l31) << 4) + 8 * hi + 64 * wave;
#pragma unroll
                for (int rt = 0; rt < 2; ++rt)
#pragma unroll
                    for (int q4 = 0; q4 < 4; ++q4) {
                        const unsigned o = (L9 ^ (q4 << 4)) + rt * 6144;
                        f32x4 t4 = {c4[rt][4 * q4], c4[rt][4 * q4 + 1], c4[rt][4 * q4 + 2], c4[rt][4 * q4 + 3]};
                        lds_w64(sm, o, f2bf4(t4));
                    }
            }
            if (!grp) wait_vm0();
        }
        R4_STAMP(7);
        bar3();
        R4_STAMP(8);
    }
    if (!grp) {
#pragma unroll
        for (int i = 0; i < MSST_B4_LAG; ++i) lds_barrier();
    } else if (ks > 0) {
        copy_out();
    }

    {
        float* slab = a.slab + ((long)blockIdx.x * H + h) * MSST_ATTN_SLAB_N;
        const int l = tid & 63, l31 = l & 31, hi = l >> 5;
#pragma unroll
        for (int dt = 0; dt < 2; ++dt)
#pragma unroll
            for (int mt = 0; mt < 3; ++mt)
#pragma unroll
                for (int r = 0; r < 16; ++r) {
                    const int d = 32 * dt + (r & 3) + 8 * (r >> 2) + 4 * hi, m = 32 * mt + l31;
                    if (roleO) slab[3 * 6144 + m * 64 + d] = G[dt][mt][r];
                    else slab[wave * 6144 + d * 96 + m] = wave < 2 ? G[dt][mt][r] * a.scale : G[dt][mt][r];
                }
    }
}

int launch_block_bwd_attn_r4(const AttnBwdArgs& a, int nchunk, hipStream_t st) {
    static std::atomic<bool> attr_set{false};
    if (a.tm.L > 64 || a.tm.L < 1 || (a.H & 1)) return MSST_ERR_UNSUPPORTED;
    if (!a.xn || !a.dab || !a.w.wqkv32 || !a.w.woutT32 || !a.w.wqkvT32 || nchunk < 1 || nchunk > a.ntiles) return MSST_ERR_BADARG;
    if (a.ntok * 192 >= 0x7ffffff0L) return MSST_ERR_UNSUPPORTED;
    typedef void (*kern_t)(AttnBwdArgs);
    const kern_t kerns[12] = {&block_bwd_attn_r4_kernel<false, false, 0>, &block_bwd_attn_r4_kernel<true, false, 0>,
                              &block_bwd_attn_r4_kernel<false, true, 0>, &block_bwd_attn_r4_kernel<true, true, 0>,
                              &block_bwd_attn_r4_kernel<false, false, 1>, &block_bwd_attn_r4_kernel<true, false, 1>,
                              &block_bwd_attn_r4_kernel<false, true, 1>, &block_bwd_attn_r4_kernel<true, true, 1>,
                              &block_bwd_attn_r4_kernel<false, false, 2>, &block_bwd_attn_r4_kernel<true, false, 2>,
                              &block_bwd_attn_r4_kernel<false, true, 2>, &block_bwd_attn_r4_kernel<true, true, 2>};
    if (a.lse && (long)a.ntiles * a.H * 256 >= 0x7ffffff0L) return MSST_ERR_UNSUPPORTED;
    if (!attr_set) {
        for (int i = 0; i < 12; ++i) {
            hipError_t e = hipFuncSetAttribute(reinterpret_cast<const void*>(kerns[i]), hipFuncAttributeMaxDynamicSharedMemorySize, R4_SMEM);
            if (e != hipSuccess) return (int)e;
        }
        attr_set = true;
    }
    ProfScope ps(K_BWD_ATTN, st);
    hipLaunchKernelGGL(kerns[(a.drop.thr ? 1 : 0) + (a.queue ? 2 : 0) + (a.lse ? (a.lse_renorm ? 8 : 4) : 0)], dim3(nchunk, a.H / 2), dim3(512), R4_SMEM, st, a);
    return (int)hipGetLastError();
}

}
```

maskedsst_amd/csrc/msst_fwd3.hip:

```cpp
#include <atomic>
#include "msst_dev.h"
#include "msst_kernels.h"
#include <type_traits>

#ifndef MSST_F3_RING
#define MSST_F3_RING 4
#endif
#ifndef MSST_F3_RPRIO
#define MSST_F3_RPRIO 1
#endif
#ifndef MSST_F3_BAND
#define MSST_F3_BAND 1
#endif
#ifndef MSST_F3_GROUP
#define MSST_F3_GROUP 10
#endif
#if defined(MSST_LAB) && !defined(MSST_LAB_X1OLD)
#define MSST_LAB_X1OLD 0
#endif
#if !defined(MSST_LAB) || !defined(MSST_LAB_NOLSE)
#define MSST_F3_LSE_STORE 1
#else
#define MSST_F3_LSE_STORE 0
#endif
// ... 67 lines not shown
    } else return P::mma(a, b, c);
}
template <bool HALF>
__device__ __forceinline__ frag pack2f(f32x4 lo, f32x4 hi) {
    const s16x4 a = cv4<HALF>(lo), b = cv4<HALF>(hi);
    frag r;
    r[0] = a[0]; r[1] = a[1]; r[2] = a[2]; r[3] = a[3];
    r[4] = b[0]; r[5] = b[1]; r[6] = b[2]; r[7] = b[3];
    return r;
}

__device__ __forceinline__ frag ld_w_gather3(const elem* w, int K, int row32, int k0, int voff) {
    const int f = (row32 >> 4) * (K >> 5) + (k0 >> 5);
    const __amdgpu_buffer_rsrc_t rs = __builtin_amdgcn_make_buffer_rsrc(const_cast<elem*>(w), 0, 0x7fffffff, 0x00020000);
    const u32x4 v = __builtin_amdgcn_raw_buffer_load_b128(rs, voff, f * 1024, 0);
    return __builtin_bit_cast(frag, v);
}

#ifndef MSST_F3_WOFF
#define MSST_F3_WOFF 1
#endif
__device__ __forceinline__ frag ld_wb3(const elem* w, int voff, int soff) {
    const __amdgpu_buffer_rsrc_t rs = __builtin_amdgcn_make_buffer_rsrc(const_cast<elem*>(w), 0, 0x7fffffff, 0x00020000);
    return __builtin_bit_cast(frag, __builtin_amdgcn_raw_buffer_load_b128(rs, voff, soff, 0));
}
__device__ __forceinline__ void load_pair3(int pi, frag (&out)[2], const elem* wqkv, int H, int h, const int (&voff)[2], int hb, int HB, int l16) {
    if (MSST_F3_WOFF) {
        if (pi < 12) {
            const int st = pi / 3, ks = pi % 3;
            const int o = hb + (st >> 1) * HB + (st & 1) * 6144 + ks * 1024;
            out[0] = ld_wb3(wqkv, l16, o);
            out[1] = ld_wb3(wqkv, l16, o + 3072);
        } else {
            const int mm = (pi - 12) / 3, ks = (pi - 12) % 3;
            const int o = hb + 2 * HB + mm * 6144 + ks * 1024;
            out[0] = ld_wb3(wqkv, voff[0], o);
            out[1] = ld_wb3(wqkv, voff[1], o);
        }
    } else if (pi < 12) {
        const int st = pi / 3, ks = pi % 3;
        const int r0 = ((st >> 1) * H + h) * 64 + (st & 1) * 32;
        out[0] = P::ld_w(wqkv, 96, r0, ks * 32);
        out[1] = P::ld_w(wqkv, 96, r0 + 16, ks * 32);
    } else {
        const int mm = (pi - 12) / 3, ks = (pi - 12) % 3;
        const int r32 = (2 * H + h) * 64 + mm * 32;
        out[0] = ld_w_gather3(wqkv, 96, r32, ks * 32, voff[0]);
        out[1] = ld_w_gather3(wqkv, 96, r32, ks * 32, voff[1]);
    }
}

}

template <bool DROP, bool STACK, bool HALF>
__global__ __launch_bounds__(512, 2) void block_fwd_rs_kernel(typename std::conditional<STACK, StackArgs, BlockArgs>::type args) {
    const BlockArgs& a = [&]() -> const BlockArgs& { if constexpr (STACK) return args.base; else return args; }();
    typedef Fwd3Smem SM;
    constexpr int LDX = SM::LDX, LDH = SM::LDH, LDO = SM::LDO;
    extern __shared__ __attribute__((aligned(16))) char smem_raw[];
    SM& sm = *reinterpret_cast<SM*>(smem_raw);

    const int tid = threadIdx.x, wv = __builtin_amdgcn_readfirstlane(tid >> 6), l = tid & 63, g = l >> 4, c = l & 15;
    const int H = a.H, inner = H * 64;
    const TileMap tm = a.tm;
    const int L = tm.L;
    const int G = (int)gridDim.x;
    const int nmine = ((int)blockIdx.x < a.ntiles) ? (a.ntiles - 1 - (int)blockIdx.x) / G + 1 : 0;
    int nsteps = nmine;
    if constexpr (STACK) {
        const int nblk = args.nblk;
        const int ng = max(1, nmine / MSST_F3_GROUP), gbase = nmine / ng, gextra = nmine - gbase * ng;
        const int p1 = max(gbase + 1, 3), p0 = max(gbase, 3);
        nsteps = nmine ? nblk * (gextra * p1 + (ng - gextra) * p0) : 0;
        for (int s_ = tid; s_ < nsteps; s_ += 512) {
            const int head = gextra * nblk * p1;
            int j, r, pp, sz, before;
            if (s_ < head) { j = s_ / (nblk * p1); r = s_ - j * nblk * p1; pp = p1; sz = gbase + 1; before = j * (gbase + 1); }
            else { j = gextra + (s_ - head) / (nblk * p0); r = s_ - head - (j - gextra) * nblk * p0; pp = p0; sz = gbase; before = gextra * (gbase + 1) + (j - gextra) * gbase; }
            const int blk = r / pp, pos = r - blk * pp;
            const unsigned idle = pos >= sz ? 1u : 0u;
            sm.steptab[s_] = (unsigned)(before + min(pos, sz - 1)) | ((unsigned)blk << 16) | ((unsigned)((j * nblk + blk) & 1) << 24) | (idle << 31);
        }
    }
    if constexpr (STACK) {
        static_assert(offsetof(StackBlk, lse_out) == 15 * 8 && offsetof(StackStride, lse_out) == 15 * 4, "blktab follows StackBlk's member order");
        for (int e = tid; e < args.nblk * 16; e += 512) {
            const int j = e >> 4, f = e & 15;
            auto kp = (const __attribute__((address_space(4))) char*)__builtin_amdgcn_kernarg_segment_ptr();
            const char* p0 = *(const char* const __attribute__((address_space(4)))*)(kp + offsetof(StackArgs, b0) + f * 8);
            const int stride = *(const int __attribute__((address_space(4)))*)(kp + offsetof(StackArgs, st) + f * 4);
            const char* pj = p0 ? p0 + (long)j * stride : nullptr;
            if (f == BT_X && j) pj = reinterpret_cast<const char*>(args.x_rest) + (long)j * args.st.y;
            sm.blktab[j][f] = pj;
        }
    }
    constexpr unsigned F3_IDLE = 0x80000000u;
    auto load_word = [&](int k) -> unsigned {
        if constexpr (STACK) return (k >= 0 && k < nsteps) ? (unsigned)__builtin_amdgcn_readfirstlane((int)sm.steptab[k]) : F3_IDLE;
        else return (k >= 0 && k < nmine) ? (unsigned)k : F3_IDLE;
    };
    int kc = 0;
    unsigned swm2 = F3_IDLE, swm1 = F3_IDLE, sw0 = F3_IDLE, swp1 = F3_IDLE, swp2 = F3_IDLE;
    auto step_word = [&](int k) -> unsigned {
        if constexpr (!STACK) return load_word(k);
        else { const int d = k - kc; return d == 0 ? sw0 : d == 1 ? swp1 : d == -1 ? swm1 : d == 2 ? swp2 : d == -2 ? swm2 : load_word(k); }
    };
    auto words_init = [&]() { kc = 0; swm2 = F3_IDLE; swm1 = F3_IDLE; sw0 = load_word(0); swp1 = load_word(1); swp2 = load_word(2); };
    auto words_advance = [&]() { swm2 = swm1; swm1 = sw0; sw0 = swp1; swp1 = swp2; swp2 = load_word(kc + 3); };
    auto tile_at = [&](int k) -> int {
        const unsigned w_ = step_word(k);
        return (w_ >> 31) ? -1 : (int)blockIdx.x + (int)(w_ & 0xffffu) * G;
    };
    auto blk_at = [&](int k) -> int { if constexpr (STACK) return (int)((step_word(k) >> 16) & 0xffu); else return 0; };
    auto slot_at = [&](int k) -> int { if constexpr (STACK) return (int)((step_word(k) >> 24) & 1u); else return 0; };
    auto in_walk = [&](int k) -> bool { return k >= 0 && k < nsteps; };
    auto epoch_differs = [&](int k1, int k0) -> bool {
        if constexpr (STACK) return in_walk(k1) && in_walk(k0) && ((step_word(k1) ^ step_word(k0)) & 0x01ff0000u) != 0u;
        else return false;
    };
    auto at_blk = [&](const void* p0, int stride, int blk) -> const char* { return reinterpret_cast<const char*>(p0) + (long)blk * (long)stride; };
    auto step_blk = [&](int k) -> StepBlk {
        StepBlk q;
        if constexpr (STACK) {
            const int j = blk_at(k);
            const StackBlk& b0 = args.b0;
            const StackStride& st = args.st;
            q.wqkv = reinterpret_cast<const elem*>(at_blk(b0.wqkv, st.wqkv, j)); q.wout = reinterpret_cast<const elem*>(at_blk(b0.wout, st.wout, j));
            q.x = reinterpret_cast<const float*>(sm.blktab[j][BT_X]);
            q.y = reinterpret_cast<float*>(const_cast<char*>(sm.blktab[j][BT_X + 1]));
            q.x1 = reinterpret_cast<float*>(const_cast<char*>(sm.blktab[j][BT_X + 2]));
            q.xn_out = reinterpret_cast<elem*>(const_cast<char*>(sm.blktab[j][BT_X + 3]));
            q.layer = b0.layer + j;
        } else {
            q.wqkv = reinterpret_cast<const elem*>(a.w.wqkv); q.wout = reinterpret_cast<const elem*>(a.w.wout);
            q.x = a.x; q.y = a.y; q.x1 = a.x1; q.xn_out = reinterpret_cast<elem*>(a.xn_out); q.layer = a.drop.layer;
        }
        return q;
    };
    auto drop_at = [&](int k) -> Drop { Drop d = a.drop; if constexpr (STACK) d.layer = args.b0.layer + blk_at(k); return d; };
    auto lnp_at = [&](int k) -> const float* { return sm.lnp[slot_at(k)]; };
    struct LnpRegs { float v[7]; };
    auto fetch_lnp = [&](int blk, int t96) -> LnpRegs {
        const float *g1, *b1_, *bo, *g2, *b2_, *bb2, *bb1;
        if constexpr (STACK) {
            auto fp_ = [&](int f) { return reinterpret_cast<const float*>(sm.blktab[blk][f]); };
            g1 = fp_(BT_LN1G); b1_ = fp_(BT_LN1G + 1); bo = fp_(BT_LN1G + 2); g2 = fp_(BT_LN1G + 3); b2_ = fp_(BT_LN1G + 4); bb1 = fp_(BT_LN1G + 5); bb2 = fp_(BT_LN1G + 6);
        }
        else { g1 = a.w.ln1_g; b1_ = a.w.ln1_b; bo = a.w.bo; g2 = a.w.ln2_g; b2_ = a.w.ln2_b; bb2 = a.w.b2; bb1 = a.w.b1; }
        LnpRegs r;
        r.v[0] = g1[t96]; r.v[1] = b1_[t96]; r.v[2] = bo[t96]; r.v[3] = g2[t96]; r.v[4] = b2_[t96]; r.v[5] = bb2[t96];
        r.v[6] = bb1[t96 < 64 ? t96 : 0];
        return r;
    };
    auto commit_lnp = [&](int slot, int t96, const LnpRegs& r) {
        float* lnp = sm.lnp[slot];
#pragma unroll
        for (int i = 0; i < 6; ++i) lnp[96 * i + t96] = r.v[i];
        if (t96 < 64) lnp[576 + t96] = r.v[6];
    };
    auto load_lnp = [&](int slot, int blk, int t96) { commit_lnp(slot, t96, fetch_lnp(blk, t96)); };
    auto mlp_w = [&](int blk, int which) -> const char* {
        if constexpr (STACK) return sm.blktab[blk][BT_W1 + which];
        else return reinterpret_cast<const char*>(which ? a.w.w2 : a.w.w1);
    };

    if (STACK) __syncthreads();
    words_init();
    if (tid < 96) load_lnp(slot_at(0), blk_at(0), tid);
#pragma unroll
    for (int i3 = 0; i3 < 3; ++i3) {
        const int f = wv * 3 + i3;
        dma_frag(f < 12 ? mlp_w(blk_at(0), 0) + f * 1024 : mlp_w(blk_at(0), 1) + (f - 12) * 1024, sm.wmlp + f * 1024);
    }
    wait_vm0();
    if (tid < 64) {
        const int sq = tid / L, ps = tid - sq * L;
        sm.rowmap[tid] = ((unsigned)(sq >= tm.TS ? 0xffff : sq) << 16) | (unsigned)ps;
    }
    auto fill_seq = [&](int k, int t64) {
        const int tile_ = tile_at(k);
        const int q = tile_ * tm.TS + t64;
        int base = -1;
        if (tile_ >= 0 && t64 < tm.TS && q < tm.nseq) {
            if (tm.mode == 0) base = q * tm.N;
            else { const int b = tm.nshift >= 0 ? (q >> tm.nshift) : q / tm.N; base = b * tm.T + (q - b * tm.N); }
        }
        sm.seqb[k & 3][t64] = base;
    };
    if (tid < 64) { fill_seq(0, tid); fill_seq(1, tid); }
    if (tid >= 64 && tid < 128) {
        const int r = tid - 64, sq = r / L;
        unsigned long long m = ~0ull;
        if (sq < tm.TS && L < 64) m = ((1ull << L) - 1ull) << (sq * L);
        sm.vm[r] = m;
    }
    __syncthreads();
    auto tok_of = [&](int k, int r) -> long {
        const unsigned sp = sm.rowmap[r];
        const int base = sm.seqb[k & 3][min((int)(sp >> 16), 63)];
        return ((sp >> 16) == 0xffffu || base < 0) ? -1 : (long)(base + (int)(sp & 0xffffu) * (tm.mode == 0 ? 1 : tm.N));
    };

    if (wv < 4) {
        int voff[2];
#pragma unroll
        for (int hi = 0; hi < 2; ++hi) {
            const int rs = 8 * (c >> 2) + (c & 3) + 4 * hi;
            voff[hi] = ((rs >> 4) * 3) * 1024 + (g * 16 + (rs & 15)) * 16;
        }
        bool band = L < 64 && MSST_F3_BAND;
#pragma unroll
        for (int j = 0; j < 4; ++j) {
            const int s_lo = (16 * j) / L, s_hi = min((16 * j + 15) / L, tm.TS - 1);
            const int k_lo = s_lo * L, k_hi = (s_hi + 1) * L - 1;
            const unsigned allow = j == 0 ? 0x3u : j == 1 ? 0x7u : j == 2 ? 0xeu : 0xcu;
            for (int t = 0; t < 4; ++t)
                if (s_lo <= s_hi && 16 * t <= k_hi && 16 * t + 15 >= k_lo && !((allow >> t) & 1u)) band = false;
// ... 490 lines not shown
            if (k >= 2 && epoch_differs(k - 1, k - 2)) {
                const int bk = blk_at(k - 1);
#pragma unroll
                for (int i6 = 0; i6 < 6; ++i6) {
                    const int f = rw * 6 + i6;
                    dma_frag_async(f < 12 ? mlp_w(bk, 0) + f * 1024 : mlp_w(bk, 1) + (f - 12) * 1024, sm.wmlp + f * 1024);
                }
            }
            lnp_switch = k + 1 < nsteps && epoch_differs(k + 1, k);
            if (lnp_switch && rt < 96) lnp_regs = fetch_lnp(blk_at(k + 1), rt);
        }
        if (have_prev) { request_xr(k - 1); outproj(1); F3_STAMP(1); epilogue1(k - 1); copy_lse(k - 1, 1); }
        F3_STAMP(2);
        if constexpr (STACK) {
            if (lnp_switch && rt < 96) commit_lnp(slot_at(k + 1), rt, lnp_regs);
            wait_vm0();
        }
        lds_barrier();
        F3_STAMP(3);
        if (MSST_F3_RPRIO02 != MSST_F3_RPRIO) __builtin_amdgcn_s_setprio(MSST_F3_RPRIO);
        if (have_prev) ln2(k - 1);
        if (rt < 64) fill_seq(k + 2, rt);
        if (have_cur) zero_acc();
        request_fw(0, have_cur ? k : k - 1);
        F3_STAMP(4);
        lds_barrier();
        F3_STAMP(5);
        if (MSST_F3_RPRIO02 != MSST_F3_RPRIO) __builtin_amdgcn_s_setprio(MSST_F3_RPRIO02);
        if (MSST_F3_LN1Q == 2 && k + 1 < nsteps) request_ln1(k + 1);
        if (have_cur) outproj(0);
        F3_STAMP(6);
        if (have_prev) { store_x1_bf16(k - 1); mlp1(k - 1); }
        if (have_cur) copy_lse(k, 0);
        if (MSST_F3_LN1Q == 2 && k + 1 < nsteps) ln1(k + 1);
        if (MSST_F3_LN1Q == 3 && k + 1 < nsteps) request_ln1(k + 1);
        F3_STAMP(7);
        lds_barrier();
        F3_STAMP(8);
        if (MSST_F3_RPRIO02 != MSST_F3_RPRIO) __builtin_amdgcn_s_setprio(MSST_F3_RPRIO);
        if (have_prev) mlp2(k - 1);
        F3_STAMP(9);
        if (MSST_F3_LN1Q == 3 && k + 1 < nsteps) ln1(k + 1);
        request_fw(1, have_cur ? k : k - 1);
        F3_STAMP(10);
        lds_barrier();
        F3_STAMP(11);
        if constexpr (STACK) words_advance();
    }
}

static int fwd3_attrs() {
    static std::atomic<bool> attr_set{false};
    if (attr_set) return 0;
    const void* ks[8] = {reinterpret_cast<const void*>(&block_fwd_rs_kernel<false, false, false>), reinterpret_cast<const void*>(&block_fwd_rs_kernel<true, false, false>),
                         reinterpret_cast<const void*>(&block_fwd_rs_kernel<false, true, false>), reinterpret_cast<const void*>(&block_fwd_rs_kernel<true, true, false>),
                         reinterpret_cast<const void*>(&block_fwd_rs_kernel<false, false, true>), reinterpret_cast<const void*>(&block_fwd_rs_kernel<true, false, true>),
                         reinterpret_cast<const void*>(&block_fwd_rs_kernel<false, true, true>), reinterpret_cast<const void*>(&block_fwd_rs_kernel<true, true, true>)};
    for (int i = 0; i < 8; ++i) {
        hipError_t e = hipFuncSetAttribute(ks[i], hipFuncAttributeMaxDynamicSharedMemorySize, (int)sizeof(Fwd3Smem));
        if (e != hipSuccess) return (int)e;
    }
    attr_set = true;
    return 0;
}

int block_fwd_stack_max_steps() { return F3_MAX_STEPS; }

int launch_block_fwd_rs_stack(const StackArgs& sa, int grid, hipStream_t st) {
    const BlockArgs& a = sa.base;
    if (a.H != 8 || sa.nblk < 1 || sa.nblk > MSST_MAX_STACK || grid < 1) return MSST_ERR_UNSUPPORTED;
    const int nmine = (a.ntiles + grid - 1) / grid;
    if (sa.nblk * (nmine < 3 ? 3 : nmine) > F3_MAX_STEPS) return MSST_ERR_UNSUPPORTED;
    int rc = fwd3_attrs();
    if (rc) return rc;
    ProfScope ps(K_BLOCK_FWD, st);
    const size_t smem = sizeof(Fwd3Smem);
    if (a.half) {
        if (a.drop.thr) hipLaunchKernelGGL((block_fwd_rs_kernel<true, true, true>), dim3(grid), dim3(512), smem, st, sa);
        else hipLaunchKernelGGL((block_fwd_rs_kernel<false, true, true>), dim3(grid), dim3(512), smem, st, sa);
    } else {
        if (a.drop.thr) hipLaunchKernelGGL((block_fwd_rs_kernel<true, true, false>), dim3(grid), dim3(512), smem, st, sa);
        else hipLaunchKernelGGL((block_fwd_rs_kernel<false, true, false>), dim3(grid), dim3(512), smem, st, sa);
    }
    return (int)hipGetLastError();
}

int launch_block_fwd_rs(const BlockArgs& a, int grid, hipStream_t st) {
    const size_t smem = sizeof(Fwd3Smem);
    if (a.H != 8) return MSST_ERR_UNSUPPORTED;
    int rc = fwd3_attrs();
    if (rc) return rc;
    ProfScope ps(K_BLOCK_FWD, st);
    if (a.half) {
        if (a.drop.thr) hipLaunchKernelGGL((block_fwd_rs_kernel<true, false, true>), dim3(grid), dim3(512), smem, st, a);
        else hipLaunchKernelGGL((block_fwd_rs_kernel<false, false, true>), dim3(grid), dim3(512), smem, st, a);
    } else {
        if (a.drop.thr) hipLaunchKernelGGL((block_fwd_rs_kernel<true, false, false>), dim3(grid), dim3(512), smem, st, a);
        else hipLaunchKernelGGL((block_fwd_rs_kernel<false, false, false>), dim3(grid), dim3(512), smem, st, a);
    }
    return (int)hipGetLastError();
}

}
```

maskedsst_amd/csrc/msst_kernels.h:

```cpp
#pragma once
#include <hip/hip_runtime.h>
#include <stdint.h>
#include "msst_dev.h"

#define MSST_PREC_F32 0
#define MSST_PREC_BF16 1
#define MSST_ERR_UNSUPPORTED (-2)
#define MSST_ERR_BADARG (-3)
#define MSST_ADAM_MAX_GROUPS 64

namespace msst {

struct BlockWeights {
    const void* wqkv;
    const void* wout;
    const void* w1;
    const void* w2;
    const void* wqkvT;
    const void* woutT;
    const void* w1T;
    const void* w2T;
    const float* ln1_g; const float* ln1_b; const float* bo;
    const float* ln2_g; const float* ln2_b; const float* b1; const float* b2;
    const void* wqkv32; const void* woutT32; const void* wqkvT32;
};

struct BlockArgs {
    BlockWeights w;
    const float* x;
    float* y;
    float* x1;
    int x1_bf16;
    int half;
    void* xn_out;
    float* lse_out;
    TileMap tm;
    int ntiles, max_grid, H;
    float scale;
    int dbg;
    unsigned long long* stamps;
    Drop drop;
};

#define MSST_MAX_STACK 16
struct StackBlk {
    const void* wqkv; const void* wout; const void* w1; const void* w2;
    const float* ln1_g; const float* ln1_b; const float* bo; const float* ln2_g; const float* ln2_b; const float* b1; const float* b2;
    const float* x; float* y; float* x1; void* xn_out; float* lse_out;
    int layer, pad_;
};
struct StackStride {
    int wqkv, wout, w1, w2, ln1_g, ln1_b, bo, ln2_g, ln2_b, b1, b2, x, y, x1, xn_out, lse_out;
};
struct StackArgs {
    BlockArgs base;
    int nblk;
    StackBlk b0;
    StackStride st;
    const float* x_rest;
};
static_assert(sizeof(StackArgs) <= 4096, "StackArgs travels as a kernel argument");

struct TokArgs {
    const float* img;
    const float* pre_g; const float* pre_b;
    const float* w_emb;
    const float* b_emb;
    const float* post_g; const float* post_b;
    const float* pos_a;
    const float* pos_b;
    const float* mask_token;
    const uint8_t* mask;
    float* out;
    int B, S, N, T, P, pos_split;
    Drop drop;
    long win0;
    int Hs, Ws, win, stride, nq, wps;
};

template <class Args>
__device__ __forceinline__ const float* scene_window_origin(const Args& a, int b) {
    const long i = a.win0 + b;
    const long s = i / a.wps;
    const int rem = (int)(i - s * a.wps), r = rem / a.nq, q = rem - r * a.nq;
    return a.img + ((s * a.S * a.P) * a.Hs + (long)r * a.stride) * a.Ws + (long)q * a.stride;
}

__device__ __forceinline__ const uint8_t* scene_window_mask(const TokArgs& a, int b, int c) {
    const long i = a.win0 + b;
    const long s = i / a.wps;
    const int rem = (int)(i - s * a.wps), r = rem / a.nq, q = rem - r * a.nq;
    return a.mask + (((s * a.S + c) * a.Hs) + (long)r * a.stride) * a.Ws + (long)q * a.stride;
}

// ... 12 lines not shown
    int64_t* classes;
    long win0, row0;
    int nwin, Bs, NC, Hs, Ws, win, stride, nr, nq;
};
int launch_scene_accumulate(const SceneArgs& a, long pixels, hipStream_t st);
int launch_scene_finalize(const SceneArgs& a, hipStream_t st);

struct HeadArgs {
    const float* y;
    const float* img;
    const int* idx;
    const float* w_pix;
    const float* b_pix;
    float* dpred;
    float* pred;
    float* partial;
    int B, S, N, T, P, K, per_block;
};

struct HeadBwdArgs {
    const float* y; const float* dpred; const int* csr_ptr; const int* csr_pos; const float* w_pix;
    float* dy; float* slab; float gscale;
    const float* gout;
    int B, S, N, T, P, K, per_block;
};

#define MSST_MLP_SLAB_N (64 * 96 + 96 * 64 + 64 + 96 + 96 + 96)
#define MSST_ATTN_SLAB_N (3 * 64 * 96 + 96 * 64)

struct MlpBwdArgs {
    BlockWeights w;
    const float* x1; const float* dy; float* dx1; float* slab;
    void* dab;
    long ntok;
    Drop drop;
    int x1_bf16;
};

struct AttnBwdArgs {
    BlockWeights w;
    const float* x; const float* da; void* dxn_part; float* slab;
    const void* dab;
    const void* xn;
    TileMap tm;
    int ntiles, H;
    long ntok;
    float scale;
    int dbg;
    unsigned long long* stamps;
    Drop drop;
    int* queue;
    const float* lse;
    int lse_renorm;
};

struct Ln1BwdArgs {
    const float* x; const float* dx1; const void* dxn_part; const float* ln1_g; float* dx; float* slab;
    long ntok;
    int H;
    Drop drop;
};

struct LnMlpArgs {
    BlockWeights w;
    const float* ln1_g;
    const float* ln1_b;
    const void* xn;
    const float* rstd;
    const float* x;
    float* dx1;
    const void* dxn_part;
    const float* x1;
    int x1_bf16;
    void* dab;
    float* slab_mlp;
    float* slab_ln1;
    long ntok;
    int nparts;
    Drop drop_i, drop_p;
    unsigned long long* stamps;
    int* queue;
};

struct TokBwdArgs {
    const float* img; const float* pre_g; const float* pre_b; const float* w_emb; const float* b_emb;
    const float* post_g; const float* post_b; const uint8_t* mask; const float* dx0; float* slab;
    int B, S, N, T, P;
    Drop drop;
};
struct TokSceneBwdArgs : TokBwdArgs {
    long win0;
    int Hs, Ws, win, stride, nq, wps;
};

struct TokInArgs {
    const float* img; const float* pre_g; const float* pre_b; const float* w_emb; const float* b_emb;
    const float* post_g; const float* post_b;
    const uint8_t* mask;
    const float* dx0;
    const float* dtarget;
    float* dimg;
    int B, S, N, T, P;
    Drop drop;
    long win0;
    int Hs, Ws, win, stride, nq, wps;
};
// ... 39 lines not shown
int launch_spec_head_bwd_rows(const SpecHeadArgs& a, hipStream_t st);
int launch_spec_head_wgrad(const SpecHeadArgs& a, hipStream_t st);
int launch_spec_head_wgrad_finish(const SpecHeadArgs& a, const float* A, const float* db, float* dw, float* dg, float* dbeta,
                                  hipStream_t st);
struct PixHeadArgs {
    const float* y; const float* ln_g; const float* ln_b; const float* w; const float* b; const float* dlogits;
    float* logits; float* xn; float* dy; float* slab;
    int B, S, N, T, NC, G;
};
int pix_head_groups(int B);
long pix_head_bwd_slab_floats(int B, int N, int NC);
int launch_pix_head_fwd(const PixHeadArgs& a, hipStream_t st);
int launch_pix_head_bwd(const PixHeadArgs& a, hipStream_t st);
int launch_scene_centre_scatter(const SceneArgs& a, hipStream_t st);
int launch_scene_centre_fill(const SceneArgs& a, hipStream_t st);

int launch_tokenize_fwd(const TokArgs& a, hipStream_t st);
int launch_tokenize_scene_fwd(const TokArgs& a, hipStream_t st);
int launch_tokenize_scene_fwd_masked(const TokArgs& a, hipStream_t st);
int launch_head_bwd(const HeadBwdArgs& a, int nchunk, hipStream_t st);
struct RSeg {
    const float* src; float* dst;
    long slab_stride;
    int nslab, n, row_len, row_stride, blk0, vec4;
    int ny;
};
#define MSST_MAX_RSEG 72
struct RSegs { RSeg s[MSST_MAX_RSEG]; int nseg; int nblocks; int ny_max; long src_ystride, dst_ystride; };
struct RSegBuilder {
    RSegs r;
    RSegBuilder() { r.nseg = 0; r.nblocks = 0; r.ny_max = 1; r.src_ystride = 0; r.dst_ystride = 0; }
    bool add(const float* src, long slab_stride, int nslab, float* dst, int n, int row_len = 0, int row_stride = 0, int ny = 1) {
        if (r.nseg >= MSST_MAX_RSEG) return false;
        if (ny < 1) return true;
        RSeg& g = r.s[r.nseg++];
        g.ny = ny;
        if (ny > r.ny_max) r.ny_max = ny;
        g.src = src; g.dst = dst; g.slab_stride = slab_stride; g.nslab = nslab; g.n = n;
        g.row_len = row_len > 0 ? row_len : n; g.row_stride = row_stride > 0 ? row_stride : n;
        g.blk0 = r.nblocks;
        g.vec4 = (n % 4 == 0 && g.row_len % 4 == 0 && g.row_stride % 4 == 0 && slab_stride % 4 == 0 &&
                  ((uintptr_t)src % 16) == 0 && ((uintptr_t)dst % 16) == 0) ? 1 : 0;
        const int per_block = g.vec4 ? 128 : 32;
        r.nblocks += (n + per_block - 1) / per_block;
        return true;
    }
};
static_assert(sizeof(RSegs) <= 4096, "RSegs travels as a kernel argument");
int launch_reduce_segs(const RSegs& r, hipStream_t st);
int launch_block_bwd_mlp(const MlpBwdArgs& a, int grid, int prec, hipStream_t st);
int launch_block_bwd_attn(const AttnBwdArgs& a, int nchunk, int prec, hipStream_t st, int* nparts);
int launch_block_bwd_attn_r3(const AttnBwdArgs& a, int nchunk, hipStream_t st);
int launch_block_bwd_attn_r4(const AttnBwdArgs& a, int nchunk, hipStream_t st);
int launch_block_bwd_ln1(const Ln1BwdArgs& a, int grid, int prec, hipStream_t st);
int launch_block_bwd_ln1mlp(const LnMlpArgs& a, int grid, hipStream_t st);
int launch_tokenize_bwd(const TokBwdArgs& a, int nchunk, hipStream_t st);
int launch_tokenize_scene_bwd(const TokSceneBwdArgs& a, int nchunk, hipStream_t st);
int launch_pos_split(const float* dpos, int S, int N, int split, float* dpe, float* dce, hipStream_t st);
int launch_adamw(float* p, const float* g, float* m, float* v, long n, float lr, float b1, float b2, float eps,
                 float wd, int step, float clamp, float gscale, hipStream_t st);
struct AdamSeg {
    long start, end;
    long a0, a1;
    float step_size, bc2_sqrt, wd, decay;
    int blk0, pad;
};
struct AdamTable {
    AdamSeg s[MSST_ADAM_MAX_GROUPS];
    float b2, omb1, omb2, eps, gscale;
    int nseg, nblocks;
};
constexpr int ADAM_QPB = 1024;
static_assert(sizeof(AdamTable) <= 4096, "AdamTable travels as a kernel argument");
int launch_adam_groups(float* p, const float* g, float* m, float* v, const AdamTable& t, hipStream_t st);
int launch_cu_thief(int nblocks, int us, unsigned* sink, hipStream_t st);
int launch_box_probe(double* out4, void* scratch, long bytes, hipStream_t st);
int launch_block_fwd_rs(const BlockArgs& a, int grid, hipStream_t st);
int launch_block_fwd_rs_stack(const StackArgs& a, int grid, hipStream_t st);
int block_fwd_stack_max_steps();
int launch_block_fwd(const BlockArgs& a, int prec, hipStream_t st);
bool block_fwd_writes_xn(const BlockArgs& a, int prec);
bool block_fwd_writes_lse(const BlockArgs& a, int prec);
int launch_head_fwd(const HeadArgs& a, float* loss, hipStream_t st);
int launch_layernorm_fwd(const float* x, const float* g, const float* b, float* y, float* mean, float* rstd, long rows, int D,
                         float eps, hipStream_t st);
int layernorm_bwd_grid(long rows, int D);
int launch_layernorm_bwd(const float* x, const float* g, const float* dy, float* dx, float* slab, int grid, long rows, int D,
                         float eps, hipStream_t st);
struct CeArgs {
    const float* logits; const int64_t* labels; const int64_t* skip;
    float* d;
    float* loss;
    int64_t* record;
    float* partial;
    int* slab;
    long rows, ignore_index;
    int NC, M;
};
int ce_workgroups(long rows);
int launch_ce_fwd(const CeArgs& a, hipStream_t st);
int launch_ce_finish(const CeArgs& a, hipStream_t st);
int launch_ce_bwd(const float* d, const int64_t* record, const float* gout, float* dlogits, long n, hipStream_t st);
constexpr int CE_CONF_MAX_CLASSES = 128;
struct CeExtArgs {
    CeArgs c;
    const float* w;
// ... 49 lines not shown
```

maskedsst_amd/engine.py:

```python
import collections
import ctypes
import os

import numpy as np
import torch

from . import _lib
from ._lib import (MsstBlockWeights, MsstBlockGrads, MsstPrepJob, PREC_BF16, PREC_F32, MODE_SPATIAL,
                   MODE_SPECTRAL, MLP_SLAB, ATTN_SLAB, LN1_SLAB)
from .flat import FlatParams

D = 96
DH = 64
STACK_MAX_TILES = 12
MLP = 64
_MODE = {"spatial": MODE_SPATIAL, "spectral": MODE_SPECTRAL}

_Head = collections.namedtuple("_Head", "fwd bwd linear shape fwd_ws bwd_slab assemble")
_HEADS = {
    "cls": _Head("msst_cls_head_fwd", "msst_cls_head_bwd", 1, lambda B, nc, N: (B, nc, N), None,
                 lambda lib, B, S, N, nc: B * (nc * 97 + 192), "msst_scene_assemble"),
    "spec": _Head("msst_spec_head_fwd", "msst_spec_head_bwd", 1, lambda B, nc, N: (B, nc, N), None,
                  lambda lib, B, S, N, nc: lib.msst_spec_head_bwd_slab(B, S, N, nc), "msst_scene_assemble"),
    "pix": _Head("msst_pix_head_fwd", "msst_pix_head_bwd", 2, lambda B, nc, N: (B, nc),
                 lambda lib, B, S, N, nc: lib.msst_pix_head_fwd_ws(B, N),
                 lambda lib, B, S, N, nc: lib.msst_pix_head_bwd_slab(B, S, N, nc), "msst_scene_centre_assemble"),
}


def _prec_of(name):
    name = (name or os.environ.get("MSST_PRECISION", "bf16")).lower()
    if name in ("fp32", "f32", "32-true", "float32"):
        return PREC_F32
    if name in ("bf16", "bf16-mixed", "bfloat16"):
        return PREC_BF16
    raise ValueError(f"unknown precision {name!r} (use 'bf16' or 'fp32')")


def _kernel_flags():
    v = int(os.environ.get("MSST_DBG", "0"))
    allowed = 16 | 64 | 128
    if v & 8:
        allowed |= 8 | 0x300
    return (v & allowed) << 8


def _stream():
    return ctypes.c_void_p(torch.cuda.current_stream().cuda_stream)


def _p(t):
    return ctypes.c_void_p(t.data_ptr()) if t is not None else ctypes.c_void_p(0)


def recon_fwd(y, img, mask_u8, w_pix, b_pix, per_block, blend, S, N, P, stats=True, lib=None):
    lib = lib or _lib.load()
    for t in (y, img, mask_u8):
        if not t.is_cuda:
            raise RuntimeError("maskedsst_amd runs on an MI355X only (tensor is on %s); there is no CPU fallback" % t.device)
    B = y.shape[0]
    if (y.dtype, img.dtype, mask_u8.dtype) != (torch.float32, torch.float32, torch.uint8):
        raise ValueError("recon_fwd takes fp32 y and img and a uint8 mask")
    if tuple(y.shape) != (B, S * N, D) or img.numel() != B * S * P * N or mask_u8.numel() != B * S * N:
        raise ValueError(f"recon_fwd: y {tuple(y.shape)}, img {tuple(img.shape)}, mask {tuple(mask_u8.shape)} do not fit "
                         f"B = {B}, S = {S}, N = {N}, P = {P}")
    y, img, mask_u8 = y.contiguous(), img.contiguous(), mask_u8.contiguous()
    tables = []
    for t, n in ((w_pix, P * D), (b_pix, P)):
        if torch.is_tensor(t):
            if not t.is_cuda or t.dtype != torch.float32 or t.numel() != (S if per_block else 1) * n:
                raise ValueError("recon_fwd: to_pixels tables must be fp32 cuda tensors [S or 1, P, 96] and [S or 1, P]")
            t = t.contiguous()
        tables.append(t)
    recon = torch.empty(B, S * P, N, dtype=torch.float32, device=y.device)
    err = torch.empty(B, S * P, dtype=torch.float64, device=y.device) if stats else None
    cnt = torch.empty(B, S * P, dtype=torch.int32, device=y.device) if stats else None
    wp, bp = (_p(t) if torch.is_tensor(t) else t for t in tables)
    _lib.check(lib.msst_recon_fwd(_p(y), _p(img), _p(mask_u8), wp, bp, int(bool(per_block)), int(bool(blend)), _p(recon), _p(err),
                                  _p(cnt), B, S, N, P, _stream()), "msst_recon_fwd")
    return recon, err, cnt


class Engine:
    def __init__(self, encoder, mim):
        self.enc = encoder
        self.mim = mim
        self.lib = _lib.load()
        self.fp = FlatParams(encoder, mim)
        self.prec = _prec_of(getattr(encoder, "precision", None))
        self.max_grid = int(os.environ.get("MSST_MAX_GRID", "0"))
        self.grid_rows = int(os.environ.get("MSST_BWD_GRID", "0")) or (self._cu_count() if torch.cuda.is_available() else 256)
        self.attn_chunks = int(os.environ.get("MSST_ATTN_CHUNKS", "0")) or \
            (self.default_attn_chunks() if torch.cuda.is_available() else 64)
        self.tok_chunks = int(os.environ.get("MSST_TOK_CHUNKS", "64"))
        self.bucket_hook = None
        self.tile_queue = False
        self._tpw = {}
        self._wbuf = None
        self._jobs = None
        self._bw = None
        self._zero_mask = None
# ... 210 lines not shown
        self.ensure()
        B = img.shape[0]
        S, N, P = self.S, self.N, self.P
        T = S * N
        img = img.contiguous().float()
        out = torch.empty(B, T, D, dtype=torch.float32, device=img.device)
        if mask_u8 is None:
            mask_u8 = self._zero_mask_for(B * T, img.device)
        fp = self.fp
        if not with_pos:
            if getattr(self, "_zero_pos", None) is None or self._zero_pos.numel() < T * D:
                self._zero_pos = torch.zeros(T * D, dtype=torch.float32, device=img.device)
            split, pos_a, pos_b = 0, self._zero_pos.data_ptr(), 0
        else:
            split, pos_a, pos_b = self._pos_tables()
        mt = fp.ptr("mask_token") if self.mim is not None else fp.ptr("post_b")
        V = ctypes.c_void_p
        _lib.check(self.lib.msst_tokenize_fwd(
            _p(img), V(fp.ptr("pre_g")), V(fp.ptr("pre_b")), V(fp.ptr("embed.w.0")), V(fp.ptr("embed.b.0")),
            V(fp.ptr("post_g")), V(fp.ptr("post_b")), V(pos_a), V(pos_b), split, V(mt), _p(mask_u8), _p(out),
            B, S, N, P, emb_drop[0], emb_drop[1], _stream()), "msst_tokenize_fwd")
        return out

    TILE_WINDOWS_PER_LAUNCH = 65535

    def tile_grid(self, tiles):
        s = self.enc.num_spatial_patches_sqrt
        return s, tiles.shape[-2] // s, tiles.shape[-1] // s

    def tokenize_windows(self, img, emb_drop=(0.0, 0), tiles=False):
        if not tiles:
            return self.tokenize(img, None, emb_drop=emb_drop)
        self._require_cuda(img)
        self.ensure()
        B, _, Ht, Wt = img.shape
        S, N, P = self.S, self.N, self.P
        s, nr, nq = self.tile_grid(img)
        total = B * nr * nq
        out = torch.empty(total, S * N, D, dtype=torch.float32, device=img.device)
        chunk = total if (P == 10 and s == 8) else min(total, self.TILE_WINDOWS_PER_LAUNCH)
        if chunk < total and emb_drop[0] > 0:
            raise NotImplementedError(f"embedding dropout over {total} windows in one step needs more than one launch of the generic "
                                      f"tokenizer ({self.TILE_WINDOWS_PER_LAUNCH} windows each): use fewer tiles per step")
        fp = self.fp
        split, pos_a, pos_b = self._pos_tables()
        V = ctypes.c_void_p
        for win0 in range(0, total, chunk):
            _lib.check(self.lib.msst_tokenize_scene_fwd_train(
                _p(img), V(fp.ptr("pre_g")), V(fp.ptr("pre_b")), V(fp.ptr("embed.w.0")), V(fp.ptr("embed.b.0")),
                V(fp.ptr("post_g")), V(fp.ptr("post_b")), V(pos_a), V(pos_b), split, _p(out[win0:]), B, Ht, Wt, s, s, win0,
                min(chunk, total - win0), S, P, emb_drop[0], emb_drop[1], _stream()), "msst_tokenize_scene_fwd_train")
        return out

    def blocks_fwd(self, x0, save=True, drop=(0.0, 0)):
        acts = [x0]
        x1s = []
        flags = _kernel_flags()
        role_split = self._role_split(flags)
        x1_bf16 = save and role_split and os.environ.get("MSST_X1_BF16", "1") != "0"
        want_lse = save and role_split and os.environ.get("MSST_LSE", "1") != "0"
        layers = self._layers()
        want_stack = os.environ.get("MSST_FWD_STACK", "auto")
        stacked = role_split and want_stack != "0"
        i0 = 0
        self.fwd_launch_blocks = []
        while i0 < len(layers):
            i1 = i0
            while i1 < len(layers) and layers[i1][0] == layers[i0][0] and i1 - i0 < 16:
                i1 += 1
            use = stacked and (want_stack == "1" or self._tiles_per_workgroup(layers[i0][0], x0.shape[0]) <= STACK_MAX_TILES)
            if use and self._fwd_stack(acts, x1s, i0, i1, save, drop, x1_bf16, want_lse):
                self.fwd_launch_blocks.append(i1 - i0)
            else:
                for i in range(i0, i1):
                    self._fwd_block(acts, x1s, i, save, drop, x1_bf16, want_lse, flags)
                self.fwd_launch_blocks += [1] * (i1 - i0)
            i0 = i1
        return acts, x1s

    def blocks_fwd_pingpong(self, x0, drop=(0.0, 0), other=None, n=None, stream=None):
        B = x0.shape[0] if n is None else n
        S, N, H = self.S, self.N, self.enc.heads
        flags = _kernel_flags()
        prec = self.prec | flags | self._half_flag(flags)
        x, y = x0, torch.empty_like(x0) if other is None else other
        wrote = ctypes.c_int(0)
        st = _stream() if stream is None else stream
        for i, (sname, _) in enumerate(self._layers()):
            _lib.check(self.lib.msst_block_fwd(ctypes.byref(self._bw[i]), _p(x), _p(y), None, _MODE[sname], B, S, N, H, prec, self.max_grid,
                                               drop[0], drop[1], i, None, None, ctypes.byref(wrote), st), "msst_block_fwd")
            x, y = y, x
        return x

    def _tiles_per_workgroup(self, sname, B):
        mode = _MODE[sname]
        key = (mode, B)
        hit = self._tpw.get(key)
        if hit is None:
            tiles = int(self.lib.msst_block_tiles(mode, B, self.S, self.N))
            grid = max(1, min(tiles, self._cu_count(), self.max_grid if self.max_grid > 0 else tiles))
            hit = self._tpw[key] = -(-tiles // grid)
        return hit

    def _role_split(self, flags):
        return self.prec == PREC_BF16 and self.enc.heads == 8 and flags == 0

    def _half_flag(self, flags):
        self.fwd_half = self._role_split(flags) and os.environ.get("MSST_FWD_HALF", "1") != "0" and self.half_ok()
        return _lib.FWD_HALF if self.fwd_half else 0

    def _attach_saved(self, x1, wrote, xn, lse):
        x1._msst_xn = xn if (wrote & _lib.SAVED_XN) else None
        x1._msst_lse = lse if (lse is not None and (wrote & _lib.SAVED_LSE)) else None
        x1._msst_rstd = bool(wrote & _lib.SAVED_RSTD) and x1._msst_lse is not None
        x1._msst_half = bool(self.fwd_half)

    def _fwd_block(self, acts, x1s, i, save, drop, x1_bf16, want_lse, flags):
        x = acts[-1]
        B = x.shape[0]
        S, N, H = self.S, self.N, self.enc.heads
        sname, l = self._layers()[i]
        y = torch.empty_like(x)
        x1 = (torch.empty(x.shape, dtype=torch.bfloat16, device=x.device) if x1_bf16 else torch.empty_like(x)) if save else None
        xn = torch.empty(x.shape, dtype=torch.bfloat16, device=x.device) if (save and self.prec != PREC_F32) else None
        mode = _MODE[sname]
        lse = None
        if xn is not None and want_lse:
            lse = torch.empty(int(self.lib.msst_block_lse_floats(mode, B, S, N, H)), dtype=torch.float32, device=x.device)
        wrote = ctypes.c_int(0)
        _lib.check(self.lib.msst_block_fwd(ctypes.byref(self._bw[i]), _p(x), _p(y), _p(x1), mode, B, S, N, H,
                                           self.prec | flags | (_lib.X1_BF16 if x1_bf16 else 0) | self._half_flag(flags), self.max_grid, drop[0], drop[1], i, _p(xn), _p(lse),
                                           ctypes.byref(wrote), _stream()),
                   "msst_block_fwd")
        if x1 is not None:
            self._attach_saved(x1, wrote.value, xn, lse)
        acts.append(y)
        x1s.append(x1)

    def _fwd_stack(self, acts, x1s, i0, i1, save, drop, x1_bf16, want_lse):
        x0 = acts[-1]
        B = x0.shape[0]
        S, N, H = self.S, self.N, self.enc.heads
        dev = x0.device
        n = i1 - i0
        mode = _MODE[self._layers()[i0][0]]
        def slices(dtype, shape=None):
            t = torch.empty((n,) + tuple(shape if shape is not None else x0.shape), dtype=dtype, device=dev)
            return [t[j] for j in range(n)]
        ys = slices(x0.dtype)
        x1 = slices(torch.bfloat16 if x1_bf16 else torch.float32) if save else None
        xn = slices(torch.bfloat16) if save else None
        lse = slices(torch.float32, (int(self.lib.msst_block_lse_floats(mode, B, S, N, H)),)) if (save and want_lse) else None
        wv = (ctypes.POINTER(MsstBlockWeights) * n)(*[ctypes.pointer(self._bw[i0 + j]) for j in range(n)])
        VP = ctypes.c_void_p * n

        def arr(ts):
            return VP(*[t.data_ptr() for t in ts]) if ts is not None else None
        wrote = ctypes.c_int(0)
        rc = self.lib.msst_block_fwd_stack(wv, n, _p(x0), arr(ys), arr(x1), arr(xn), arr(lse), mode, B, S, N, H,
                                           self.prec | (_lib.X1_BF16 if x1_bf16 else 0) | self._half_flag(0), self.max_grid, drop[0], drop[1], i0,
                                           ctypes.byref(wrote), _stream())
        if rc == -2:
            return False
        _lib.check(rc, "msst_block_fwd_stack")
        for j in range(n):
            acts.append(ys[j])
            if save:
                self._attach_saved(x1[j], wrote.value, xn[j], lse[j] if lse is not None else None)
                x1s.append(x1[j])
            else:
                x1s.append(None)
        return True

    def head_fwd(self, y, img, idx32, want_pred=False):
        B, T, _ = y.shape
        S, N, P = self.S, self.N, self.P
        K = idx32.shape[1]
        dev = y.device
        dpred = torch.empty(B, K, P, dtype=torch.float32, device=dev)
        pred = torch.empty(B, K, P, dtype=torch.float32, device=dev) if want_pred else None
        partial = torch.empty(B * ((K + 63) // 64), dtype=torch.float32, device=dev)
        loss = torch.empty((), dtype=torch.float32, device=dev)
        per_block = 1 if hasattr(self.mim.to_pixels, "layers") else 0
        V = ctypes.c_void_p
        _lib.check(self.lib.msst_head_fwd(
            _p(y), _p(img), _p(idx32), V(self.fp.ptr("to_pixels.w.0")), V(self.fp.ptr("to_pixels.b.0")), per_block,
            _p(dpred), _p(pred), _p(partial), _p(loss), B, S, N, P, K, _stream()), "msst_head_fwd")
        return loss, dpred, pred

    def recon_fwd(self, y, img, mask_u8, blend=True, stats=True):
        per_block = 1 if hasattr(self.mim.to_pixels, "layers") else 0
        V = ctypes.c_void_p
        return recon_fwd(y, img, mask_u8, V(self.fp.ptr("to_pixels.w.0")), V(self.fp.ptr("to_pixels.b.0")), per_block, blend,
                         self.S, self.N, self.P, stats=stats, lib=self.lib)

    def reconstruct(self, img, mask_u8, blend=True):
        self._require_cuda(img)
        if self.mim is None:
            raise RuntimeError("reconstruct needs the SimMIM wrapper's mask token and to_pixels (a bare encoder has neither)")
        img = img.contiguous().float()
        with torch.no_grad():
            self.prep_weights()
            x0 = self.tokenize(img, mask_u8)
            acts, _ = self.blocks_fwd(x0, save=False)
            return self.recon_fwd(acts[-1], img, mask_u8, blend)

    def tokenize_scene_masked(self, scene, scene_mask_u8, stride, win0, nwin, out=None):
        self._require_cuda(scene)
        self._require_cuda(scene_mask_u8)
        if self.mim is None:
            raise RuntimeError("tokenize_scene_masked needs the SimMIM wrapper's mask token (a bare encoder has none)")
        self.ensure()
        Bs, _, Hs, Ws = scene.shape
        S, N, P = self.S, self.N, self.P
# ... 52 lines not shown
            return cube, err, cnt, cover

    def _fire(self, bucket):
        if self.bucket_hook is not None:
            for name, start, end in self.fp.buckets:
                if name == bucket:
                    self.bucket_hook(name, start, end)

    def head_bwd(self, y, dpred, csr_ptr, csr_pos, gout=None):
        B, T, _ = y.shape
        S, N, P = self.S, self.N, self.P
        K = dpred.shape[1]
        dev = y.device
        nchunk = max(1, min(B, int(os.environ.get("MSST_HEAD_CHUNKS", "0")) or 512 // max(S, 1)))
        dy = torch.empty_like(y)
        slab = torch.empty(S * nchunk * (P * 96 + P), dtype=torch.float32, device=dev)
        per_block = 1 if hasattr(self.mim.to_pixels, "layers") else 0
        gscale = 1.0 / (B * K * P) / K
        V = ctypes.c_void_p
        g = self.fp.grad
        _lib.check(self.lib.msst_head_bwd(
            _p(y), _p(dpred), _p(csr_ptr), _p(csr_pos), V(self.fp.ptr("to_pixels.w.0")), per_block, gscale, _p(gout),
            _p(dy), _p(slab), nchunk, V(self.fp.ptr("to_pixels.w.0", g)), V(self.fp.ptr("to_pixels.b.0", g)),
            B, S, N, P, K, _stream()), "msst_head_bwd")
        self._fire("head")
        return dy

    def _grad_stride(self, nlayers):
        blocks = [f"{sname}.{l}" for sname, l in self._layers()[:nlayers]]
        d = self.fp.block_stride(blocks, [n for n, _ in MsstBlockGrads._fields_])
        return -d if d is not None and d < 0 and d % 4 == 0 else None

    def _bwd_workspace(self, B, device):
        H = self.enc.heads
        ntok = B * self.S * self.N
        esz = 4 if self.prec == PREC_F32 else 2
        dx1 = torch.empty(ntok * 96, dtype=torch.float32, device=device)
        part = torch.empty(H * ntok * 96 * esz, dtype=torch.uint8, device=device)
        slab = torch.empty(self.grid_rows * (3 * MLP_SLAB + LN1_SLAB) + self.attn_chunks * H * ATTN_SLAB, dtype=torch.float32, device=device)
        dab = torch.empty(ntok * 96, dtype=torch.bfloat16, device=device) if self.prec != PREC_F32 else None
        return dx1, part, slab, dab

    def blocks_bwd(self, acts, x1s, dy, drop=(0.0, 0)):
        H = self.enc.heads
        ntok = dy.shape[0] * self.S * self.N
        ws = self._bwd_workspace(dy.shape[0], dy.device)
        x1_bf16 = len(x1s) > 0 and all(t.dtype == torch.bfloat16 for t in x1s)
        if not x1_bf16 and any(t.dtype != torch.float32 for t in x1s):
            raise ValueError("saved x1 rows of mixed dtypes")
        nparts = H // 2 if H % 2 == 0 else H
        chain = (self.prec == PREC_BF16 and _kernel_flags() == 0 and all(getattr(t, "_msst_xn", None) is not None for t in x1s)
                 and nparts <= 4 and os.environ.get("MSST_BWD_CHAIN", "1") != "0" and self.enc.depth > 0
                 and ntok * 384 < 2 ** 31 - 16 and nparts * ntok * 192 < 2 ** 31 - 16)
        ln1_from_xn = (chain and x1_bf16 and os.environ.get("MSST_LN1_XN", "1") != "0"
                       and all(getattr(t, "_msst_rstd", False) for t in x1s) and self.ln1_xn_ok())
        self.last_bwd_ln1_from_xn = bool(ln1_from_xn)
        if chain:
            return self._blocks_bwd_chained(acts, x1s, dy, drop, ws,
                                            (_lib.X1_BF16 if x1_bf16 else 0) | (_lib.LN1_FROM_XN if ln1_from_xn else 0))
        return self._blocks_bwd_unchained(acts, x1s, dy, drop, ws)

    def _blocks_bwd_chained(self, acts, x1s, dy, drop, ws, x1flags):
        B = dy.shape[0]
        S, N, H = self.S, self.N, self.enc.heads
        dev = dy.device
        dx1, part, slab, dab = ws
        layers = self._layers()
        queue = None
        if self.tile_queue or os.environ.get("MSST_TILE_QUEUE", "0") == "1":
            if getattr(self, "_queue_ws", None) is None or self._queue_ws.device != dev:
                self._queue_ws = torch.zeros(64, dtype=torch.int32, device=dev)
            queue = self._queue_ws
        last = len(layers) - 1
        dx0 = torch.empty_like(dy)
        null_w = ctypes.POINTER(MsstBlockWeights)()
        null_g = ctypes.POINTER(MsstBlockGrads)()
        gstride = self._grad_stride(len(layers))
        defer = gstride is not None and os.environ.get("MSST_BWD_DEFER", "0") == "1"
        nslab_r = (slab.numel() + 3) // 4 * 4
        if defer:
            slab = torch.empty(nslab_r * len(layers), dtype=torch.float32, device=dev)
        run_start = last
        for i in reversed(range(len(layers))):
            sname, l = layers[i]
            prev = i > 0
            x1 = x1s[i]
            slab_i = slab[(last - i) * nslab_r:] if defer else slab
            _lib.check(self.lib.msst_block_bwd_chain(
                ctypes.byref(self._bw[i]), ctypes.byref(self._bg[i]),
                ctypes.byref(self._bw[i - 1]) if prev else null_w, ctypes.byref(self._bg[i - 1]) if prev else null_g,
                _p(acts[i]), _p(x1), _p(x1s[i - 1]) if prev else _p(None), _p(dy) if i == last else _p(None),
                _p(None) if prev else _p(dx0), _p(dx1), _p(part), _p(slab_i), self.grid_rows, self.attn_chunks, _MODE[sname],
                B, S, N, H, self.prec | x1flags | (_lib.LSE_RENORM if getattr(x1, "_msst_half", False) else 0) |
                (_lib.BWD_DEFER_REDUCE if defer else 0), drop[0], drop[1], i, _p(x1._msst_xn), _p(getattr(x1, "_msst_lse", None)), _p(dab),
                1 if i == last else 0, _p(queue), _stream()),
                "msst_block_bwd_chain")
            if not defer:
                self._fire(f"{sname}.{l}")
            elif i == 0 or layers[i - 1][0] != sname:
                count = run_start - i + 1
                _lib.check(self.lib.msst_block_bwd_reduce(
                    ctypes.byref(self._bg[run_start]), ctypes.byref(self._bg[run_start - 1]) if run_start > 0 else null_g,
                    _p(slab[(last - run_start) * nslab_r:]), nslab_r, gstride, count, count if i > 0 else count - 1,
                    1 if run_start == last else 0, self.grid_rows, self.attn_chunks, _MODE[sname], B, S, N, H, self.prec, _stream()),
                    "msst_block_bwd_reduce")
                for j in range(run_start, i - 1, -1):
                    self._fire(f"{layers[j][0]}.{layers[j][1]}")
                run_start = i - 1
        return dx0

    def _blocks_bwd_unchained(self, acts, x1s, dy, drop, ws):
        layers = self._layers()
        g, other = dy, torch.empty_like(dy)
        for i in reversed(range(len(layers))):
            self.block_bwd_single(i, acts[i], x1s[i], g, other, drop=drop, ws=ws)
            g, other = other, g
            self._fire(f"{layers[i][0]}.{layers[i][1]}")
        return g

    def block_bwd_single(self, i, x, x1, dy, dx=None, drop=(0.0, 0), ws=None):
        dx1, part, slab, dab = ws if ws is not None else self._bwd_workspace(dy.shape[0], dy.device)
        if dx is None:
            dx = torch.empty_like(dy)
        if x1.dtype not in (torch.float32, torch.bfloat16):
            raise ValueError("saved x1 rows must be fp32 or bf16")
        x1flag = _lib.X1_BF16 if x1.dtype == torch.bfloat16 else 0
        _lib.check(self.lib.msst_block_bwd(
            ctypes.byref(self._bw[i]), ctypes.byref(self._bg[i]), _p(x), _p(x1), _p(dy), _p(dx),
            _p(dx1), _p(part), _p(slab), self.grid_rows, self.attn_chunks, _MODE[self._layers()[i][0]], dy.shape[0], self.S, self.N, self.enc.heads,
            self.prec | _kernel_flags() | x1flag | (_lib.LSE_RENORM if getattr(x1, "_msst_half", False) else 0),
            drop[0], drop[1], i, _p(getattr(x1, "_msst_xn", None)), _p(getattr(x1, "_msst_lse", None)), _p(dab), _stream()), "msst_block_bwd")
        return dx

    def tokenize_bwd(self, img, mask_u8, dx0, emb_drop=(0.0, 0), with_pos=True):
        B = img.shape[0]
        S, N, P = self.S, self.N, self.P
        dev = img.device
        nchunk = max(1, min(B, self.tok_chunks))
        ss = N * 96 + 96 * P + 96 * 4 + 32
        slab = torch.empty(S * nchunk * ss + S * N * 96, dtype=torch.float32, device=dev)
        fp, g = self.fp, self.fp.grad
        V = ctypes.c_void_p
        split, dpa, dpb = self._pos_tables(g) if with_pos else (0, 0, 0)
        dmt = fp.ptr("mask_token", g) if (self.mim is not None and with_pos) else 0
        _lib.check(self.lib.msst_tokenize_bwd(
            _p(img), V(fp.ptr("pre_g")), V(fp.ptr("pre_b")), V(fp.ptr("embed.w.0")), V(fp.ptr("embed.b.0")),
            V(fp.ptr("post_g")), V(fp.ptr("post_b")), _p(mask_u8), _p(dx0), _p(slab), nchunk,
            V(fp.ptr("pre_g", g)), V(fp.ptr("pre_b", g)), V(fp.ptr("embed.w.0", g)), V(fp.ptr("embed.b.0", g)),
            V(fp.ptr("post_g", g)), V(fp.ptr("post_b", g)), V(dpa), V(dpb), split, V(dmt), B, S, N, P,
# ... 61 lines not shown
    def trainable(self):
        if self.fp.flat is None or getattr(self, "_trainable_key", None) != self.fp.version:
            groups, _ = self.fp._ordered()
            self._trainable = [(n, p) for _, g in groups for n, p in g]
            self._trainable_key = self.fp.version if self.fp.flat is not None else None
        return self._trainable

    def dropout_state(self):
        p = float(self.enc.dropout_p) if self.enc.training else 0.0
        if p <= 0.0:
            return 0.0, 0
        if not 0.0 < p < 1.0:
            raise ValueError(f"dropout probability {p} outside (0, 1)")
        seed = int(torch.randint(0, 2 ** 31 - 1, (1,)).item())
        rank = int(getattr(self.mim, "dp_rank", 0)) if self.mim is not None else 0
        if rank:
            seed = (seed ^ (rank * 0x9E3779B1)) & 0x7FFFFFFF
        return p, seed

    def _upload(self, dev, *arrays):
        if getattr(self, "_up", None) is None:
            self._up = {"sets": [None, None], "k": 0}
        up = self._up
        k = up["k"]
        up["k"] = 1 - k
        cur = up["sets"][k]
        sig = tuple((a.shape, a.dtype) for a in arrays)
        if cur is None or cur["sig"] != sig:
            cur = {"sig": sig,
                   "pin": [torch.empty(a.shape, dtype=torch.from_numpy(a).dtype, pin_memory=True) for a in arrays],
                   "ev": torch.cuda.Event()}
            up["sets"][k] = cur
        else:
            cur["ev"].synchronize()
        out = []
        for pin, a in zip(cur["pin"], arrays):
            pin.numpy()[...] = a
            d = torch.empty(pin.shape, dtype=pin.dtype, device=dev)
            d.copy_(pin, non_blocking=True)
            out.append(d)
        cur["ev"].record(torch.cuda.current_stream(dev))
        return out

    def simmim_loss(self, img, bool_mask, idx):
        self._require_cuda(img)
        self.ensure()
        dev = img.device
        T = self.S * self.N
        img = img.contiguous().float()
        from .masking import inverse_csr
        bm = bool_mask.cpu().numpy() if torch.is_tensor(bool_mask) else np.asarray(bool_mask)
        ix = idx.cpu().numpy() if torch.is_tensor(idx) else np.asarray(idx)
        ptr, pos = inverse_csr(ix, T)
        mask_u8, idx32, csr_ptr, csr_pos = self._upload(dev, bm.astype(np.uint8), ix.astype(np.int32), ptr, pos)
        names = [n for n, _ in self.trainable()]
        params = [p for _, p in self.trainable()]
        if not torch.is_grad_enabled() or not (img.requires_grad or any(p.requires_grad for p in params)):
            self.prep_weights()
            x0 = self.tokenize(img, mask_u8)
            acts, _ = self.blocks_fwd(x0, save=False, drop=self.dropout_state())
            loss, _, _ = self.head_fwd(acts[-1], img, idx32)
            return loss
        return _SimMIMLossFn.apply(self, names, self.dropout_state(), img, mask_u8, idx32, csr_ptr, csr_pos, *params)

    def _block_param_names(self):
        return [n for n, _ in self.trainable() if n.startswith(("spatial.", "spectral."))]

    def _embed_param_names(self):
        return [n for n, _ in self.trainable() if n.startswith(("embed.", "pre_", "post_"))]

    def transformer(self, tokens):
        self._require_cuda(tokens)
        self.ensure()
        drop = self.dropout_state()
        tokens = tokens.contiguous().float()
        by_name = dict(self.trainable())
        names = self._block_param_names()
        params = [by_name[n] for n in names]
        if torch.is_grad_enabled() and (tokens.requires_grad or any(p.requires_grad for p in params)):
            return _TransformerFn.apply(self, names, drop, tokens, *params)
        self.prep_weights()
        acts, _ = self.blocks_fwd(tokens, save=False, drop=drop)
        return acts[-1]

    def embed_patches(self, patches):
        self._require_cuda(patches)
        self.ensure()
        B, S, N, P = patches.shape
        want_input = torch.is_grad_enabled() and patches.requires_grad
        img = (patches if want_input else patches.detach()).permute(0, 1, 3, 2).reshape(B, S * P, N).contiguous().float()
        by_name = dict(self.trainable())
        names = self._embed_param_names()
        params = [by_name[n] for n in names]
        if torch.is_grad_enabled() and (want_input or any(p.requires_grad for p in params)):
            return _EmbedFn.apply(self, names, img, *params)
        return self.tokenize(img, None, with_pos=False)

    def features(self, img):
        enc = self.enc
        params = [q for _, q in self.trainable()]
        if torch.is_grad_enabled() and (img.requires_grad or any(q.requires_grad for q in params)):
            self._require_cuda(img)
            patches = enc.to_patch_embedding.to_patch(img.contiguous().float())
            tokens = self.embed_patches(patches).reshape(img.shape[0], -1, D)
            pos = enc.get_pos_embeddings() if enc.spectral_pos_embed else enc.pos_embedding[:, :tokens.shape[1]]
            tokens = tokens + pos
            if enc.training and float(enc.emb_dropout_p) > 0:
                tokens = torch.nn.functional.dropout(tokens, p=float(enc.emb_dropout_p), training=True)
            return self.transformer(tokens)
        pe = float(enc.emb_dropout_p) if enc.training else 0.0
        emb_drop = (pe, int(torch.randint(0, 2 ** 31 - 1, (1,)).item())) if pe > 0 else (0.0, 0)
        x0 = self.tokenize(img, None, with_pos=True, emb_drop=emb_drop)
        with torch.no_grad():
            return self.transformer(x0)

    def _head_kind(self):
# ... 131 lines not shown
        S, N, P = self.S, self.N, self.P
        w = self.enc.num_spatial_patches_sqrt
        self.prep_weights()
        split, pos_a, pos_b = self._pos_tables()
        bufs = [torch.empty(chunk, S * N, D, dtype=torch.float32, device=scene.device) for _ in range(2)]
        V = ctypes.c_void_p
        for win0 in range(0, total, chunk):
            n = min(chunk, total - win0)
            _lib.check(self.lib.msst_tokenize_scene_fwd(
                _p(scene), V(fp.ptr("pre_g")), V(fp.ptr("pre_b")), V(fp.ptr("embed.w.0")), V(fp.ptr("embed.b.0")),
                V(fp.ptr("post_g")), V(fp.ptr("post_b")), V(pos_a), V(pos_b), split, _p(bufs[0]), Bs, Hs, Ws, w, stride, win0, n, S, P, st),
                "msst_tokenize_scene_fwd")
            yield win0, n, self.blocks_fwd_pingpong(bufs[0], other=bufs[1], n=n, stream=st)

    def encode_scene(self, scene, stride, normalize=False, max_windows=2048):
        self._require_cuda(scene)
        with torch.no_grad():
            scene = scene.contiguous().float()
            Bs, _, Hs, Ws = scene.shape
            S, N = self.S, self.N
            w = self.enc.num_spatial_patches_sqrt
            total, chunk = self._scene_chunking(scene, stride, max_windows)
            dev = scene.device
            win_feat = torch.empty(chunk, D, N, dtype=torch.float32, device=dev)
            feat = torch.empty(Bs, D, Hs, Ws, dtype=torch.float32, device=dev)
            cover = torch.empty(Bs, Hs, Ws, dtype=torch.int32, device=dev)
            st = _stream()
            for win0, n, y in self._scene_encoder_chunks(scene, stride, total, chunk, st):
                _lib.check(self.lib.msst_pool_spectral_fwd(_p(y), _p(win_feat), n, S, N, st), "msst_pool_spectral_fwd")
                _lib.check(self.lib.msst_scene_embed_assemble(_p(win_feat), win0, n, _p(feat), _p(cover), Bs, D, Hs, Ws, w, stride,
                                                              int(win0 + n == total), int(bool(normalize)), st),
                           "msst_scene_embed_assemble")
            return feat, cover

    def simmim_forward_stages(self, img, bool_mask, idx, drop=(0.0, 0)):
        self._require_cuda(img)
        self.prep_weights()
        dev = img.device
        img = img.contiguous().float()
        mask_u8 = bool_mask.to(device=dev, dtype=torch.uint8).contiguous()
        idx32 = idx.to(device=dev, dtype=torch.int32).contiguous()
        tok_embed = self.tokenize(img, None, with_pos=False)
        x0 = self.tokenize(img, mask_u8)
        acts, x1s = self.blocks_fwd(x0, drop=drop)
        loss, dpred, pred = self.head_fwd(acts[-1], img, idx32, want_pred=True)
        L = self.enc.depth
        return dict(loss=loss, tok_embed=tok_embed, tok_masked=x0, after_spatial=acts[L], enc_out=acts[-1],
                    pred=pred, dpred=dpred, acts=acts, x1s=x1s)


class _SimMIMLossFn(torch.autograd.Function):

    @staticmethod
    def forward(ctx, eng, names, drop, img, mask_u8, idx32, csr_ptr, csr_pos, *params):
        eng.prep_weights()
        x0 = eng.tokenize(img, mask_u8)
        acts, x1s = eng.blocks_fwd(x0, save=True, drop=drop)
        ctx.drop = drop
        loss, dpred, _ = eng.head_fwd(acts[-1], img, idx32)
        ctx.eng = eng
        ctx.names = names
        ctx.stash = (img, mask_u8, csr_ptr, csr_pos, acts, x1s, dpred)
        return loss

    @staticmethod
    def backward(ctx, gout):
        eng = ctx.eng
        img, mask_u8, csr_ptr, csr_pos, acts, x1s, dpred = ctx.stash
        ctx.stash = None
        needs = ctx.needs_input_grad[8:]
        _refuse_accumulation(eng, ctx.names, needs)
        gout = gout.contiguous().float()
        dy = eng.head_bwd(acts[-1], dpred, csr_ptr, csr_pos, gout)
        dx0 = eng.blocks_bwd(acts, x1s, dy, drop=ctx.drop)
        dimg = None
        if ctx.needs_input_grad[3]:
            dimg = eng.tokenize_input_bwd(img, mask_u8, dx0, eng.head_bwd_target(dpred, csr_ptr, csr_pos, gout))
        if any(needs):
            eng.tokenize_bwd(img, mask_u8, dx0)
        return (None, None, None, dimg) + (None,) * 4 + _grad_views(eng, ctx.names, needs)


def _refuse_accumulation(eng, names, needs=None):
    by_name = dict(eng.trainable())
    lo, hi = eng.fp.grad.data_ptr(), eng.fp.grad.data_ptr() + 4 * eng.fp.grad.numel()
    for i, n in enumerate(names):
        if needs is not None and not needs[i]:
            continue
        p = by_name[n]
        if p.grad is not None and lo <= p.grad.data_ptr() < hi:
            raise RuntimeError(
                "maskedsst_amd hands autograd views of its flat gradient buffer: drop the previous gradients "
                "with optimizer.zero_grad(set_to_none=True) (the torch default) before the next backward; "
                "in-place gradient accumulation across backward calls is not supported")


def _grad_views(eng, names, needs=None):
    return tuple(eng.fp.view(n, eng.fp.grad) if needs is None or needs[i] else None for i, n in enumerate(names))


class _TransformerFn(torch.autograd.Function):

    @staticmethod
    def forward(ctx, eng, names, drop, tokens, *params):
        eng.prep_weights()
        acts, x1s = eng.blocks_fwd(tokens, save=True, drop=drop)
        ctx.eng, ctx.names, ctx.drop = eng, names, drop
        ctx.stash = (acts[:-1], x1s)
        return acts[-1]

    @staticmethod
    def backward(ctx, dy):
        eng = ctx.eng
        acts, x1s = ctx.stash
        ctx.stash = None
        needs = ctx.needs_input_grad[4:]
        _refuse_accumulation(eng, ctx.names, needs)
        dx0 = eng.blocks_bwd(acts, x1s, dy.contiguous().float().clone(), drop=ctx.drop)
        return (None, None, None, dx0) + _grad_views(eng, ctx.names, needs)


class _EmbedFn(torch.autograd.Function):

    @staticmethod
    def forward(ctx, eng, names, img, *params):
        ctx.eng, ctx.names = eng, names
        ctx.stash = (img,)
        return eng.tokenize(img, None, with_pos=False)

    @staticmethod
    def backward(ctx, dtok):
        eng = ctx.eng
        (img,) = ctx.stash
# ... 58 lines not shown
```

Baseline: 11060 samples/s.

## Skip dead spectral tiles in last block forward and chained backward

Builds per-batch live/dead tile lists from the loss-target indices, so the final spectral block's attention tiles whose outputs never reach the loss are not computed. The forward kernels walk only live tiles (optionally zeroing dead outputs), and the chained attention backward walks a per-chunk live list held in extra LDS. This removes compute for tokens that do not affect the masked reconstruction loss. In exchange it adds host-side list construction and upload each step, extra validation paths, and a strict coupling between forward and backward configuration.

```diff
diff --git a/include/msst.h b/include/msst.h
--- a/include/msst.h
+++ b/include/msst.h
@@ -113,6 +113,20 @@
                          int B, int S, int N, int heads, int prec, int max_grid, float dropout_p, uint32_t seed, int layer0,
                          int* saved , void* stream);
 
+typedef struct MsstTileLists {
+    int struct_bytes;
+    int nlive, ndead, zero_y;
+    const int32_t* live;
+    const int32_t* dead;
+} MsstTileLists;
+int msst_block_fwd_live(const MsstBlockWeights* w , const float* x, float* y, float* x1, int mode,
+                        int B, int S, int N, int heads, int prec, int max_grid, float dropout_p, uint32_t seed,
+                        int layer, void* xn_out, float* lse_out, int* saved , const MsstTileLists* lists , void* stream);
+int msst_block_fwd_stack_live(const MsstBlockWeights* const* w , int nblk, const float* x0, float* const* y ,
+                              float* const* x1 , void* const* xn_out , float* const* lse_out , int mode,
+                              int B, int S, int N, int heads, int prec, int max_grid, float dropout_p, uint32_t seed, int layer0,
+                              int* saved , const MsstTileLists* lists , void* stream);
+
 int msst_head_fwd(const float* y, const float* img, const int32_t* idx, const float* w_pix,
                   const float* b_pix, int per_block, float* dpred, float* pred, float* partial,
                   float* loss, int B, int S, int N, int P, int K, void* stream);
@@ -150,6 +164,13 @@
                          void* dxn_part, float* slab, int grid_rows, int nchunk, int mode, int B, int S, int N, int heads,
                          int prec, float dropout_p, uint32_t seed, int layer, const void* xn_saved, const float* lse_saved ,
                          void* dab_ws, int first, int32_t* tile_queue , void* stream);
+
+int msst_block_bwd_chain_live(const MsstBlockWeights* w , const MsstBlockGrads* g ,
+                              const MsstBlockWeights* w_prev , const MsstBlockGrads* g_prev ,
+                              const float* x, const float* x1, const float* x1_prev, const float* dy, float* dx, float* dx1,
+                              void* dxn_part, float* slab, int grid_rows, int nchunk, int mode, int B, int S, int N, int heads,
+                              int prec, float dropout_p, uint32_t seed, int layer, const void* xn_saved, const float* lse_saved,
+                              void* dab_ws, int first, int32_t* tile_queue , const MsstTileLists* lists , void* stream);
 
 int msst_block_bwd_reduce(const MsstBlockGrads* g , const MsstBlockGrads* g_prev ,
                           float* slab, long slab_stride, long grad_stride, int count, int count_prev, int first,
diff --git a/maskedsst_amd/_lib.py b/maskedsst_amd/_lib.py
--- a/maskedsst_amd/_lib.py
+++ b/maskedsst_amd/_lib.py
@@ -34,6 +34,10 @@
 class MsstBlockGrads(Structure):
     _fields_ = [(n, c_void_p) for n in (
         "ln1_g", "ln1_b", "wqkv", "wout", "bo", "ln2_g", "ln2_b", "w1", "b1", "w2", "b2")]
+
+
+class MsstTileLists(Structure):
+    _fields_ = [("struct_bytes", c_int), ("nlive", c_int), ("ndead", c_int), ("zero_y", c_int), ("live", c_void_p), ("dead", c_void_p)]
 
 
 class MsstAdamGroup(Structure):
@@ -86,6 +90,10 @@
                                c_int, c_int, c_float, c_uint32, c_int, _P, _P, POINTER(c_int), _P]),
     "msst_block_fwd_stack": (c_int, [_P, c_int, _P, _P, _P, _P, _P, c_int, c_int, c_int, c_int, c_int, c_int, c_int, c_float, c_uint32, c_int,
                                      POINTER(c_int), _P]),
+    "msst_block_fwd_live": (c_int, [POINTER(MsstBlockWeights), _P, _P, _P, c_int, c_int, c_int, c_int, c_int,
+                                    c_int, c_int, c_float, c_uint32, c_int, _P, _P, POINTER(c_int), POINTER(MsstTileLists), _P]),
+    "msst_block_fwd_stack_live": (c_int, [_P, c_int, _P, _P, _P, _P, _P, c_int, c_int, c_int, c_int, c_int, c_int, c_int, c_float, c_uint32,
+                                          c_int, POINTER(c_int), POINTER(MsstTileLists), _P]),
     "msst_head_fwd": (c_int, [_P, _P, _P, _P, _P, c_int, _P, _P, _P, _P, c_int, c_int, c_int, c_int,
                               c_int, _P]),
     "msst_head_bwd": (c_int, [_P, _P, _P, _P, _P, c_int, c_float, _P, _P, _P, c_int, _P, _P, c_int, c_int, c_int,
@@ -96,6 +104,10 @@
                                      POINTER(MsstBlockGrads), _P, _P, _P, _P, _P, _P, _P, _P,
                                      c_int, c_int, c_int, c_int, c_int, c_int, c_int, c_int, c_float, c_uint32, c_int, _P, _P, _P,
                                      c_int, _P, _P]),
+    "msst_block_bwd_chain_live": (c_int, [POINTER(MsstBlockWeights), POINTER(MsstBlockGrads), POINTER(MsstBlockWeights),
+                                          POINTER(MsstBlockGrads), _P, _P, _P, _P, _P, _P, _P, _P,
+                                          c_int, c_int, c_int, c_int, c_int, c_int, c_int, c_int, c_float, c_uint32, c_int, _P, _P, _P,
+                                          c_int, _P, POINTER(MsstTileLists), _P]),
     "msst_block_bwd_reduce": (c_int, [POINTER(MsstBlockGrads), POINTER(MsstBlockGrads), _P, ctypes.c_long, ctypes.c_long,
                                       c_int, c_int, c_int, c_int, c_int, c_int, c_int, c_int, c_int, c_int, c_int, _P]),
     "msst_tokenize_bwd": (c_int, [_P] * 10 + [c_int] + [_P] * 8 + [c_int, _P, c_int, c_int, c_int, c_int, c_float,
diff --git a/maskedsst_amd/csrc/msst_api.hip b/maskedsst_amd/csrc/msst_api.hip
--- a/maskedsst_amd/csrc/msst_api.hip
+++ b/maskedsst_amd/csrc/msst_api.hip
@@ -449,9 +449,20 @@
     return (long)ntiles_of(make_tilemap(mode, B, S, N));
 }
 
-int msst_block_fwd(const MsstBlockWeights* w, const float* x, float* y, float* x1, int mode, int B, int S,
-                   int N, int heads, int prec, int max_grid, float dropout_p, uint32_t seed, int layer,
-                   void* xn_out, float* lse_out, int* saved, void* stream) {
+static int tile_lists(const MsstTileLists* lists, int ntiles, bool forward, TileLists* tl) {
+    *tl = TileLists();
+    if (!lists) return 0;
+    if (lists->struct_bytes != (int)sizeof(MsstTileLists) || !lists->live || !lists->dead || lists->nlive < 1 || lists->ndead < 1 ||
+        lists->ndead >= ntiles)
+        return MSST_ERR_BADARG;
+    if (forward ? lists->nlive + lists->ndead != ntiles : (long)lists->nlive > 2L * ntiles) return MSST_ERR_BADARG;
+    tl->live = lists->live; tl->dead = lists->dead; tl->nlive = lists->nlive; tl->ndead = lists->ndead; tl->zero_y = lists->zero_y ? 1 : 0;
+    return 0;
+}
+
+static int block_fwd_impl(const MsstBlockWeights* w, const float* x, float* y, float* x1, int mode, int B, int S,
+                          int N, int heads, int prec, int max_grid, float dropout_p, uint32_t seed, int layer,
+                          void* xn_out, float* lse_out, int* saved, const MsstTileLists* lists, void* stream) {
     if (int rc = block_shape(mode, B, S, N, heads)) return fail(rc, "msst_block_fwd (B, S, N, heads < 1, mode not 0 / 1, or sequence length > 64)");
     if (!bw_ok(w) || !x || !y || x == y) return fail(MSST_ERR_BADARG, "msst_block_fwd (null argument, or MsstBlockWeights of another header revision)");
     const int dbg = (prec >> 8) & 0xffff;
@@ -486,12 +497,29 @@
     a.xn_out = (xn_out && block_fwd_writes_xn(a, prec)) ? xn_out : nullptr;
     a.lse_out = (lse_out && block_fwd_writes_lse(a, prec)) ? lse_out : nullptr;
     if (saved) *saved = (a.xn_out ? MSST_SAVED_XN : 0) | (a.lse_out ? (MSST_SAVED_LSE | MSST_SAVED_RSTD) : 0);
+    if (lists) {
+        if (!(prec == MSST_PREC_BF16 && heads == 8 && !(dbg & (16 | 64)))) return fail(MSST_ERR_UNSUPPORTED, "msst_block_fwd_live (the role-split bf16 forward only: 8 heads, no MSST_KERNEL_* flags)");
+        if (int rc = tile_lists(lists, a.ntiles, true, &a.tl)) return fail(rc, "msst_block_fwd_live (MsstTileLists)");
+        if (a.max_grid > a.tl.nlive) a.max_grid = a.tl.nlive;
+    }
     return fail(launch_block_fwd(a, prec, (hipStream_t)stream), "msst_block_fwd");
 }
 
-int msst_block_fwd_stack(const MsstBlockWeights* const* w, int nblk, const float* x0, float* const* y, float* const* x1,
-                         void* const* xn_out, float* const* lse_out, int mode, int B, int S, int N, int heads, int prec, int max_grid,
-                         float dropout_p, uint32_t seed, int layer0, int* saved, void* stream) {
+int msst_block_fwd(const MsstBlockWeights* w, const float* x, float* y, float* x1, int mode, int B, int S,
+                   int N, int heads, int prec, int max_grid, float dropout_p, uint32_t seed, int layer,
+                   void* xn_out, float* lse_out, int* saved, void* stream) {
+    return block_fwd_impl(w, x, y, x1, mode, B, S, N, heads, prec, max_grid, dropout_p, seed, layer, xn_out, lse_out, saved, nullptr, stream);
+}
+
+int msst_block_fwd_live(const MsstBlockWeights* w, const float* x, float* y, float* x1, int mode, int B, int S,
+                        int N, int heads, int prec, int max_grid, float dropout_p, uint32_t seed, int layer,
+                        void* xn_out, float* lse_out, int* saved, const MsstTileLists* lists, void* stream) {
+    return block_fwd_impl(w, x, y, x1, mode, B, S, N, heads, prec, max_grid, dropout_p, seed, layer, xn_out, lse_out, saved, lists, stream);
+}
+
+static int block_fwd_stack_impl(const MsstBlockWeights* const* w, int nblk, const float* x0, float* const* y, float* const* x1,
+                                void* const* xn_out, float* const* lse_out, int mode, int B, int S, int N, int heads, int prec, int max_grid,
+                                float dropout_p, uint32_t seed, int layer0, int* saved, const MsstTileLists* lists, void* stream) {
     if (int rc = block_shape(mode, B, S, N, heads)) return fail(rc, "msst_block_fwd_stack (B, S, N, heads < 1, mode not 0 / 1, or sequence length > 64)");
     if (!w || !x0 || !y || nblk < 1) return fail(MSST_ERR_BADARG, "msst_block_fwd_stack");
     if (nblk > MSST_MAX_STACK) return fail(MSST_ERR_UNSUPPORTED, "msst_block_fwd_stack (more than 16 blocks)");
@@ -562,12 +590,26 @@
     sa.x_rest = nblk > 1 ? reinterpret_cast<const float*>(reinterpret_cast<const char*>(y[0]) - (long)sa.st.y) : x0;
     if (saved) *saved = (xn_out ? MSST_SAVED_XN : 0) | (lse_out ? (MSST_SAVED_LSE | MSST_SAVED_RSTD) : 0);
     if (a.ntiles < 1) return 0;
+    if (int rc = tile_lists(lists, a.ntiles, true, &a.tl)) return fail(rc, "msst_block_fwd_stack_live (MsstTileLists)");
     int ncu = 256, dev = 0;
     hipGetDevice(&dev);
     if (hipDeviceGetAttribute(&ncu, hipDeviceAttributeMultiprocessorCount, dev) != hipSuccess || ncu < 1) ncu = 256;
-    int grid = a.max_grid < a.ntiles ? a.max_grid : a.ntiles;
+    const int nwalk = a.tl.live ? a.tl.nlive : a.ntiles;
+    int grid = a.max_grid < nwalk ? a.max_grid : nwalk;
     if (grid > ncu) grid = ncu;
     return fail(launch_block_fwd_rs_stack(sa, grid, (hipStream_t)stream), "msst_block_fwd_stack");
+}
+
+int msst_block_fwd_stack(const MsstBlockWeights* const* w, int nblk, const float* x0, float* const* y, float* const* x1,
+                         void* const* xn_out, float* const* lse_out, int mode, int B, int S, int N, int heads, int prec, int max_grid,
+                         float dropout_p, uint32_t seed, int layer0, int* saved, void* stream) {
+    return block_fwd_stack_impl(w, nblk, x0, y, x1, xn_out, lse_out, mode, B, S, N, heads, prec, max_grid, dropout_p, seed, layer0, saved, nullptr, stream);
+}
+
+int msst_block_fwd_stack_live(const MsstBlockWeights* const* w, int nblk, const float* x0, float* const* y, float* const* x1,
+                              void* const* xn_out, float* const* lse_out, int mode, int B, int S, int N, int heads, int prec, int max_grid,
+                              float dropout_p, uint32_t seed, int layer0, int* saved, const MsstTileLists* lists, void* stream) {
+    return block_fwd_stack_impl(w, nblk, x0, y, x1, xn_out, lse_out, mode, B, S, N, heads, prec, max_grid, dropout_p, seed, layer0, saved, lists, stream);
 }
 
 int msst_head_fwd(const float* y, const float* img, const int32_t* idx, const float* w_pix,
@@ -672,7 +714,7 @@
                           const float* dy, float* dx, float* dx1, void* dxn_part, float* slab, int grid_rows,
                           int nchunk, int mode, int B, int S, int N, int heads, int prec, float dropout_p,
                           uint32_t seed, int layer, const void* xn_saved, const float* lse_saved, void* dab_ws, int chain, int first,
-                          int32_t* tile_queue, hipStream_t st) {
+                          int32_t* tile_queue, hipStream_t st, const MsstTileLists* lists = nullptr) {
     if (int rc = block_shape(mode, B, S, N, heads)) return fail(rc, "msst_block_bwd (B, S, N, heads < 1, mode not 0 / 1, or sequence length > 64)");
     if (!bw_ok(w) || (w_prev && !bw_ok(w_prev)) || !g || grid_rows < 1 || nchunk < 1)
         return fail(MSST_ERR_BADARG, "msst_block_bwd (null argument, or MsstBlockWeights of another header revision)");
@@ -693,6 +735,14 @@
     const bool fast_rows = xn_saved && dab_ws && prec == MSST_PREC_BF16 && !(dbg & 16);
     if (chain && (!fast_rows || (w_prev && (!g_prev || !x1_prev)) || (first && !dy) || (!w_prev && !dx)))
         return fail(MSST_ERR_BADARG, "msst_block_bwd_chain (bf16 with saved LN1 rows and the dab workspace only)");
+    if (lists) {
+        if (!chain || !w_prev || !(dbg & 2048) || !(dbg & 1024) || (dbg & (16 | 128)) || (heads & 1) || !lse_saved)
+            return fail(MSST_ERR_UNSUPPORTED, "msst_block_bwd_chain_live (needs the two-head attention backward, a block before it, MSST_X1_BF16 and MSST_LN1_FROM_XN)");
+        if (int rc = tile_lists(lists, aa.ntiles, false, &aa.tl)) return fail(rc, "msst_block_bwd_chain_live (MsstTileLists)");
+        const int nc_ = nchunk < aa.ntiles ? nchunk : aa.ntiles;
+        if (!tile_queue && ((long)aa.tl.nlive + nc_ - 1) / nc_ > block_bwd_attn_live_max_steps())
+            return fail(MSST_ERR_UNSUPPORTED, "msst_block_bwd_chain_live (walk list longer than 511 steps per chunk)");
+    }
     const bool run_mlp = !chain || first;
     const int x1b = (dbg & 1024) ? 1 : 0;
     if (x1b && prec != MSST_PREC_BF16)
@@ -777,6 +827,16 @@
                          int32_t* tile_queue, void* stream) {
     return block_bwd_impl(w, g, w_prev, g_prev, x, x1, x1_prev, dy, dx, dx1, dxn_part, slab, grid_rows, nchunk, mode, B, S, N,
                           heads, prec, dropout_p, seed, layer, xn_saved, lse_saved, dab_ws, 1, first, tile_queue, (hipStream_t)stream);
+}
+
+int msst_block_bwd_chain_live(const MsstBlockWeights* w, const MsstBlockGrads* g, const MsstBlockWeights* w_prev,
+                              const MsstBlockGrads* g_prev, const float* x, const float* x1, const float* x1_prev,
+                              const float* dy, float* dx, float* dx1, void* dxn_part, float* slab, int grid_rows,
+                              int nchunk, int mode, int B, int S, int N, int heads, int prec, float dropout_p,
+                              uint32_t seed, int layer, const void* xn_saved, const float* lse_saved, void* dab_ws, int first,
+                              int32_t* tile_queue, const MsstTileLists* lists, void* stream) {
+    return block_bwd_impl(w, g, w_prev, g_prev, x, x1, x1_prev, dy, dx, dx1, dxn_part, slab, grid_rows, nchunk, mode, B, S, N,
+                          heads, prec, dropout_p, seed, layer, xn_saved, lse_saved, dab_ws, 1, first, tile_queue, (hipStream_t)stream, lists);
 }
 
 int msst_block_bwd_reduce(const MsstBlockGrads* g, const MsstBlockGrads* g_prev, float* slab, long slab_stride, long grad_stride,
diff --git a/maskedsst_amd/csrc/msst_bwd4.hip b/maskedsst_amd/csrc/msst_bwd4.hip
--- a/maskedsst_amd/csrc/msst_bwd4.hip
+++ b/maskedsst_amd/csrc/msst_bwd4.hip
@@ -47,7 +47,9 @@
 constexpr int R4_ROWBUF = 24576, R4_DA = 12288;
 constexpr int R4_G0 = 49152, R4_GSZ = 49152;
 constexpr int R3_Q = 0, R3_K = 8192, R3_DO = 16384, R3_V = 24576, R3_P = 32768, R3_DS = 40960;
-constexpr int R4_OUT = 147456, R4_MAP = 159744, R4_SEQ = 160000, R4_SEQO = 160272, R4_QT = 160272 + 272, R4_LSE = R4_QT + 16, R4_SMEM = R4_LSE + 1024;
+constexpr int R4_OUT = 147456, R4_MAP = 159744, R4_SEQ = 160000, R4_SEQO = 160272, R4_QT = 160272 + 272, R4_LSE = R4_QT + 16, R4_SMEM = R4_LSE + 1024,
+              R4_WALK = R4_SMEM, R4_WALK_N = 512, R4_SMEM_LIVE = R4_WALK + 4 * R4_WALK_N;
+static_assert(R4_SMEM_LIVE <= 160 * 1024, "LDS of a CU");
 
 __device__ __forceinline__ int fz(int r) { return (((r >> 1) & 1) << 2) | ((((r >> 2) ^ (r >> 3)) & 1) << 1) | ((r >> 3) & 1); }
 __device__ __forceinline__ int fz2(int r) { return (((r >> 3) & 1) << 1) | ((r >> 2) & 1); }
@@ -113,7 +115,7 @@
 
 }
 
-template <bool DROP, bool QUEUE, int LSE>
+template <bool DROP, bool QUEUE, int LSE, bool LIVE>
 __global__ __launch_bounds__(512, 1) void block_bwd_attn_r4_kernel(AttnBwdArgs a) {
     extern __shared__ __attribute__((aligned(16))) char smem_raw[];
     lds_char* const sm = (lds_char*)smem_raw;
@@ -125,6 +127,29 @@
     const TileMap tm = a.tm;
     const int L = tm.L;
     bf16_t* part = reinterpret_cast<bf16_t*>(a.dxn_part) + (long)blockIdx.y * a.ntok * 96;
+    const int* const walk_list = LIVE ? a.tl.live : nullptr;
+    const int nwalk = LIVE ? a.tl.nlive : 0;
+    auto walk = [&](int p) -> int { return walk_list ? ((unsigned)p < (unsigned)nwalk ? walk_list[p] : a.ntiles) : p; };
+    if (LIVE && !QUEUE) {
+        for (int k = (int)threadIdx.x; k < R4_WALK_N; k += 512)
+            *reinterpret_cast<__attribute__((address_space(3))) int*>(sm + R4_WALK + 4 * k) = walk((int)blockIdx.x + k * (int)gridDim.x);
+    }
+    if (LIVE && a.tl.dead) {
+        for (int di = (int)blockIdx.x; di < a.tl.ndead; di += (int)gridDim.x) {
+            const int dtile = a.tl.dead[di];
+            if (dtile < 0 || dtile >= a.ntiles) continue;
+            for (int e = (int)threadIdx.x; e < 64 * 12; e += 512) {
+                const int r = e / 12, s16 = e - 12 * r;
+                const int sq = r / L, ps = r - sq * L, q = dtile * tm.TS + sq;
+                if (sq >= tm.TS || q >= tm.nseq) continue;
+                long tok;
+                if (tm.mode == 0) tok = (long)q * tm.N + ps;
+                else { const int b = tm.nshift >= 0 ? (q >> tm.nshift) : q / tm.N; tok = (long)b * tm.T + (long)ps * tm.N + (q - b * tm.N); }
+                const u32x4 z = {0u, 0u, 0u, 0u};
+                *reinterpret_cast<u32x4*>(reinterpret_cast<char*>(part) + tok * 192 + 16 * s16) = z;
+            }
+        }
+    }
 
     const bool roleO = wave == 3;
     const void* w1p = roleO ? a.w.woutT32 : a.w.wqkv32;
@@ -188,9 +213,9 @@
         int t0 = (int)blockIdx.x;
         if (QUEUE) {
             int r = 0;
-            if ((tid & 63) == 0) { r = __hip_atomic_fetch_add(a.queue + blockIdx.y, 2, __ATOMIC_RELAXED, __HIP_MEMORY_SCOPE_AGENT); qt[0] = r; qt[1] = r + 1; }
+            if ((tid & 63) == 0) { r = __hip_atomic_fetch_add(a.queue + blockIdx.y, 2, __ATOMIC_RELAXED, __HIP_MEMORY_SCOPE_AGENT); qt[0] = walk(r); qt[1] = walk(r + 1); r = qt[0]; }
             t0 = __builtin_amdgcn_readfirstlane(r);
-        }
+        } else t0 = walk(t0);
         fill_seqbase(seqbase, t0);
         if ((tid & 63) == 0) { seqbase[64] = -1; seqout[64] = -1; }
     }
@@ -226,7 +251,7 @@
             dma16(rows_d, dst + R4_DA, voff);
         }
     };
-    if (!grp) { dma_rows(0); dma_lse(QUEUE ? __builtin_amdgcn_readfirstlane(qt[0]) : (int)blockIdx.x, 0); wait_vm0(); }
+    if (!grp) { dma_rows(0); dma_lse(QUEUE ? __builtin_amdgcn_readfirstlane(qt[0]) : walk((int)blockIdx.x), 0); wait_vm0(); }
     unsigned cinv, csx;
     {
         const unsigned sp = rowmap[tid >> 2];
@@ -270,9 +295,11 @@
     }
     int xb = 0;
     int ks = 0;
-    for (int tile = QUEUE ? __builtin_amdgcn_readfirstlane(qt[0]) : (int)blockIdx.x; tile < a.ntiles;
-         xb = R4_ROWBUF - xb, ++ks, tile = QUEUE ? __builtin_amdgcn_readfirstlane(qt[ks & 3]) : tile + (int)gridDim.x) {
+    int tile_next = 0;
+    for (int tile = QUEUE ? __builtin_amdgcn_readfirstlane(qt[0]) : walk((int)blockIdx.x); tile < a.ntiles;
+         xb = R4_ROWBUF - xb, ++ks, tile = QUEUE ? __builtin_amdgcn_readfirstlane(qt[ks & 3]) : LIVE ? tile_next : tile + (int)gridDim.x) {
         const int p1_in = xb + p1_row, p3_x = p1_in;
+        if (LIVE && !QUEUE) tile_next = __builtin_amdgcn_readfirstlane(*reinterpret_cast<const __attribute__((address_space(3))) int*>(sm + R4_WALK + 4 * (ks + 1)));
 #if defined(MSST_STAMPS)
         const bool stamp_on = (a.dbg & 8) && a.stamps && blockIdx.x == 7 && blockIdx.y == 1 && (threadIdx.x & 63) == 0 && tile == (int)blockIdx.x + 20 * (int)gridDim.x;
 #define R4_STAMP(i) do { if (stamp_on) a.stamps[16 * wv + (i)] = __builtin_readcyclecounter(); } while (0)
@@ -358,7 +385,7 @@
         R4_STAMP(2);
         B4_PRIO(2);
         if (wv == 3) {
-            fill_seqbase(seqbase, QUEUE ? qt[(ks + 1) & 3] : tile + (int)gridDim.x);
+            fill_seqbase(seqbase, QUEUE ? qt[(ks + 1) & 3] : LIVE ? tile_next : tile + (int)gridDim.x);
             if (QUEUE && (tid & 63) == 0) qpend = __hip_atomic_fetch_add(a.queue + blockIdx.y, 1, __ATOMIC_RELAXED, __HIP_MEMORY_SCOPE_AGENT);
         }
         if (wv == 7) fill_seqbase(seqout, tile);
@@ -548,7 +575,7 @@
             R4_STAMP(3);
             bar3();
             R4_STAMP(4);
-            if (!grp) { dma_rows(R4_ROWBUF - xb); dma_lse(QUEUE ? __builtin_amdgcn_readfirstlane(qt[(ks + 1) & 3]) : tile + (int)gridDim.x, R4_ROWBUF - xb); }
+            if (!grp) { dma_rows(R4_ROWBUF - xb); dma_lse(QUEUE ? __builtin_amdgcn_readfirstlane(qt[(ks + 1) & 3]) : LIVE ? tile_next : tile + (int)gridDim.x, R4_ROWBUF - xb); }
             B4_PRIO(3);
             auto phase3 = [&](auto role_tag) {
                 constexpr int ROLE = decltype(role_tag)::value;
@@ -650,7 +677,7 @@
             wgrad(std::integral_constant<int, 0>{}, std::integral_constant<int, 12>{});
             R4_STAMP(9);
             if (roleO) {
-                if (QUEUE && !grp && (tid & 63) == 0) qt[(ks + 2) & 3] = qpend;
+                if (QUEUE && !grp && (tid & 63) == 0) qt[(ks + 2) & 3] = walk(qpend);
                 load_w1();
             } else {
                 f32x16 c4[2];
@@ -724,28 +751,33 @@
     }
 }
 
+int block_bwd_attn_live_max_steps() { return R4_WALK_N - 1; }
+
 int launch_block_bwd_attn_r4(const AttnBwdArgs& a, int nchunk, hipStream_t st) {
     static std::atomic<bool> attr_set{false};
     if (a.tm.L > 64 || a.tm.L < 1 || (a.H & 1)) return MSST_ERR_UNSUPPORTED;
     if (!a.xn || !a.dab || !a.w.wqkv32 || !a.w.woutT32 || !a.w.wqkvT32 || nchunk < 1 || nchunk > a.ntiles) return MSST_ERR_BADARG;
     if (a.ntok * 192 >= 0x7ffffff0L) return MSST_ERR_UNSUPPORTED;
+    if (a.tl.live && !a.queue && ((long)a.tl.nlive + nchunk - 1) / nchunk > R4_WALK_N - 1) return MSST_ERR_UNSUPPORTED;
     typedef void (*kern_t)(AttnBwdArgs);
-    const kern_t kerns[12] = {&block_bwd_attn_r4_kernel<false, false, 0>, &block_bwd_attn_r4_kernel<true, false, 0>,
-                              &block_bwd_attn_r4_kernel<false, true, 0>, &block_bwd_attn_r4_kernel<true, true, 0>,
-                              &block_bwd_attn_r4_kernel<false, false, 1>, &block_bwd_attn_r4_kernel<true, false, 1>,
-                              &block_bwd_attn_r4_kernel<false, true, 1>, &block_bwd_attn_r4_kernel<true, true, 1>,
-                              &block_bwd_attn_r4_kernel<false, false, 2>, &block_bwd_attn_r4_kernel<true, false, 2>,
-                              &block_bwd_attn_r4_kernel<false, true, 2>, &block_bwd_attn_r4_kernel<true, true, 2>};
+#define R4_K(LIVE_) &block_bwd_attn_r4_kernel<false, false, 0, LIVE_>, &block_bwd_attn_r4_kernel<true, false, 0, LIVE_>, \
+                    &block_bwd_attn_r4_kernel<false, true, 0, LIVE_>, &block_bwd_attn_r4_kernel<true, true, 0, LIVE_>, \
+                    &block_bwd_attn_r4_kernel<false, false, 1, LIVE_>, &block_bwd_attn_r4_kernel<true, false, 1, LIVE_>, \
+                    &block_bwd_attn_r4_kernel<false, true, 1, LIVE_>, &block_bwd_attn_r4_kernel<true, true, 1, LIVE_>, \
+                    &block_bwd_attn_r4_kernel<false, false, 2, LIVE_>, &block_bwd_attn_r4_kernel<true, false, 2, LIVE_>, \
+                    &block_bwd_attn_r4_kernel<false, true, 2, LIVE_>, &block_bwd_attn_r4_kernel<true, true, 2, LIVE_>
+    const kern_t kerns[24] = {R4_K(false), R4_K(true)};
+#undef R4_K
     if (a.lse && (long)a.ntiles * a.H * 256 >= 0x7ffffff0L) return MSST_ERR_UNSUPPORTED;
     if (!attr_set) {
-        for (int i = 0; i < 12; ++i) {
-            hipError_t e = hipFuncSetAttribute(reinterpret_cast<const void*>(kerns[i]), hipFuncAttributeMaxDynamicSharedMemorySize, R4_SMEM);
+        for (int i = 0; i < 24; ++i) {
+            hipError_t e = hipFuncSetAttribute(reinterpret_cast<const void*>(kerns[i]), hipFuncAttributeMaxDynamicSharedMemorySize, i < 12 ? R4_SMEM : R4_SMEM_LIVE);
             if (e != hipSuccess) return (int)e;
         }
         attr_set = true;
     }
     ProfScope ps(K_BWD_ATTN, st);
-    hipLaunchKernelGGL(kerns[(a.drop.thr ? 1 : 0) + (a.queue ? 2 : 0) + (a.lse ? (a.lse_renorm ? 8 : 4) : 0)], dim3(nchunk, a.H / 2), dim3(512), R4_SMEM, st, a);
+    hipLaunchKernelGGL(kerns[(a.drop.thr ? 1 : 0) + (a.queue ? 2 : 0) + (a.lse ? (a.lse_renorm ? 8 : 4) : 0) + (a.tl.live ? 12 : 0)], dim3(nchunk, a.H / 2), dim3(512), a.tl.live ? R4_SMEM_LIVE : R4_SMEM, st, a);
     return (int)hipGetLastError();
 }
 
diff --git a/maskedsst_amd/csrc/msst_fwd3.hip b/maskedsst_amd/csrc/msst_fwd3.hip
--- a/maskedsst_amd/csrc/msst_fwd3.hip
+++ b/maskedsst_amd/csrc/msst_fwd3.hip
@@ -143,7 +143,7 @@
 
 }
 
-template <bool DROP, bool STACK, bool HALF>
+template <bool DROP, bool STACK, bool HALF, bool LIVE>
 __global__ __launch_bounds__(512, 2) void block_fwd_rs_kernel(typename std::conditional<STACK, StackArgs, BlockArgs>::type args) {
     const BlockArgs& a = [&]() -> const BlockArgs& { if constexpr (STACK) return args.base; else return args; }();
     typedef Fwd3Smem SM;
@@ -156,7 +156,9 @@
     const TileMap tm = a.tm;
     const int L = tm.L;
     const int G = (int)gridDim.x;
-    const int nmine = ((int)blockIdx.x < a.ntiles) ? (a.ntiles - 1 - (int)blockIdx.x) / G + 1 : 0;
+    const int* const live = LIVE ? a.tl.live : nullptr;
+    const int nwalk = live ? a.tl.nlive : a.ntiles;
+    const int nmine = ((int)blockIdx.x < nwalk) ? (nwalk - 1 - (int)blockIdx.x) / G + 1 : 0;
     int nsteps = nmine;
     if constexpr (STACK) {
         const int nblk = args.nblk;
@@ -200,7 +202,9 @@
     auto words_advance = [&]() { swm2 = swm1; swm1 = sw0; sw0 = swp1; swp1 = swp2; swp2 = load_word(kc + 3); };
     auto tile_at = [&](int k) -> int {
         const unsigned w_ = step_word(k);
-        return (w_ >> 31) ? -1 : (int)blockIdx.x + (int)(w_ & 0xffffu) * G;
+        if (w_ >> 31) return -1;
+        const int p_ = (int)blockIdx.x + (int)(w_ & 0xffffu) * G;
+        return live ? live[p_] : p_;
     };
     auto blk_at = [&](int k) -> int { if constexpr (STACK) return (int)((step_word(k) >> 16) & 0xffu); else return 0; };
     auto slot_at = [&](int k) -> int { if constexpr (STACK) return (int)((step_word(k) >> 24) & 1u); else return 0; };
@@ -254,6 +258,42 @@
         if constexpr (STACK) return sm.blktab[blk][BT_W1 + which];
         else return reinterpret_cast<const char*>(which ? a.w.w2 : a.w.w1);
     };
+
+    if (LIVE && a.tl.dead) {
+        const int nb_ = [&]() { if constexpr (STACK) return args.nblk; else return 1; }();
+        for (int di = (int)blockIdx.x; di < a.tl.ndead; di += G) {
+            const int dtile = a.tl.dead[di];
+            const int r = tid >> 3, part = tid & 7;
+            const int sq = r / L, ps = r - sq * L, q = dtile * tm.TS + sq;
+            if (dtile < 0 || dtile >= a.ntiles || sq >= tm.TS || q >= tm.nseq) continue;
+            long tok;
+            if (tm.mode == 0) tok = (long)q * tm.N + ps;
+            else { const int b = tm.nshift >= 0 ? (q >> tm.nshift) : q / tm.N; tok = (long)b * tm.T + (long)ps * tm.N + (q - b * tm.N); }
+            const f32x4 z4 = {0.f, 0.f, 0.f, 0.f};
+            for (int j = 0; j < nb_; ++j) {
+                float *y_, *x1_, *st_; elem* xn_;
+                if constexpr (STACK) {
+                    y_ = reinterpret_cast<float*>(reinterpret_cast<char*>(args.b0.y) + (long)j * args.st.y);
+                    x1_ = args.b0.x1 ? reinterpret_cast<float*>(reinterpret_cast<char*>(args.b0.x1) + (long)j * args.st.x1) : nullptr;
+                    xn_ = args.b0.xn_out ? reinterpret_cast<elem*>(reinterpret_cast<char*>(args.b0.xn_out) + (long)j * args.st.xn_out) : nullptr;
+                    st_ = args.b0.lse_out ? reinterpret_cast<float*>(reinterpret_cast<char*>(args.b0.lse_out) + (long)j * args.st.lse_out) : nullptr;
+                } else { y_ = a.y; x1_ = a.x1; xn_ = reinterpret_cast<elem*>(a.xn_out); st_ = a.lse_out; }
+                if (a.tl.zero_y && j == nb_ - 1) {
+#pragma unroll
+                    for (int i = 0; i < 3; ++i) *reinterpret_cast<f32x4*>(y_ + tok * 96 + 4 * (part + 8 * i)) = z4;
+                }
+                if (x1_) {
+                    if (a.x1_bf16) { if (part < 6) *reinterpret_cast<f32x4*>(reinterpret_cast<char*>(x1_) + tok * 192 + 32 * part) = z4, *reinterpret_cast<f32x4*>(reinterpret_cast<char*>(x1_) + tok * 192 + 32 * part + 16) = z4; }
+                    else {
+#pragma unroll
+                        for (int i = 0; i < 3; ++i) *reinterpret_cast<f32x4*>(x1_ + tok * 96 + 4 * (part + 8 * i)) = z4;
+                    }
+                }
+                if (xn_ && part < 6) { *reinterpret_cast<f32x4*>(reinterpret_cast<char*>(xn_) + tok * 192 + 32 * part) = z4; *reinterpret_cast<f32x4*>(reinterpret_cast<char*>(xn_) + tok * 192 + 32 * part + 16) = z4; }
+                if (MSST_F3_RSTD_STORE && st_ && part == 7) st_[(long)a.ntiles * H * 64 + tok] = 0.f;
+            }
+        }
+    }
 
     if (STACK) __syncthreads();
     words_init();
@@ -850,11 +890,13 @@
 static int fwd3_attrs() {
     static std::atomic<bool> attr_set{false};
     if (attr_set) return 0;
-    const void* ks[8] = {reinterpret_cast<const void*>(&block_fwd_rs_kernel<false, false, false>), reinterpret_cast<const void*>(&block_fwd_rs_kernel<true, false, false>),
-                         reinterpret_cast<const void*>(&block_fwd_rs_kernel<false, true, false>), reinterpret_cast<const void*>(&block_fwd_rs_kernel<true, true, false>),
-                         reinterpret_cast<const void*>(&block_fwd_rs_kernel<false, false, true>), reinterpret_cast<const void*>(&block_fwd_rs_kernel<true, false, true>),
-                         reinterpret_cast<const void*>(&block_fwd_rs_kernel<false, true, true>), reinterpret_cast<const void*>(&block_fwd_rs_kernel<true, true, true>)};
-    for (int i = 0; i < 8; ++i) {
+#define F3_K(LIVE_) reinterpret_cast<const void*>(&block_fwd_rs_kernel<false, false, false, LIVE_>), reinterpret_cast<const void*>(&block_fwd_rs_kernel<true, false, false, LIVE_>), \
+                    reinterpret_cast<const void*>(&block_fwd_rs_kernel<false, true, false, LIVE_>), reinterpret_cast<const void*>(&block_fwd_rs_kernel<true, true, false, LIVE_>), \
+                    reinterpret_cast<const void*>(&block_fwd_rs_kernel<false, false, true, LIVE_>), reinterpret_cast<const void*>(&block_fwd_rs_kernel<true, false, true, LIVE_>), \
+                    reinterpret_cast<const void*>(&block_fwd_rs_kernel<false, true, true, LIVE_>), reinterpret_cast<const void*>(&block_fwd_rs_kernel<true, true, true, LIVE_>)
+    const void* ks[16] = {F3_K(false), F3_K(true)};
+#undef F3_K
+    for (int i = 0; i < 16; ++i) {
         hipError_t e = hipFuncSetAttribute(ks[i], hipFuncAttributeMaxDynamicSharedMemorySize, (int)sizeof(Fwd3Smem));
         if (e != hipSuccess) return (int)e;
     }
@@ -862,24 +904,29 @@
     return 0;
 }
 
+template <class F>
+static void f3_dispatch(bool drop, bool half, bool live, F&& go) {
+    auto l3 = [&](auto d_, auto h_) { if (live) go(d_, h_, std::true_type{}); else go(d_, h_, std::false_type{}); };
+    auto l2 = [&](auto d_) { if (half) l3(d_, std::true_type{}); else l3(d_, std::false_type{}); };
+    if (drop) l2(std::true_type{}); else l2(std::false_type{});
+}
+
 int block_fwd_stack_max_steps() { return F3_MAX_STEPS; }
 
 int launch_block_fwd_rs_stack(const StackArgs& sa, int grid, hipStream_t st) {
     const BlockArgs& a = sa.base;
     if (a.H != 8 || sa.nblk < 1 || sa.nblk > MSST_MAX_STACK || grid < 1) return MSST_ERR_UNSUPPORTED;
-    const int nmine = (a.ntiles + grid - 1) / grid;
+    const int nwalk = a.tl.live ? a.tl.nlive : a.ntiles;
+    const int nmine = (nwalk + grid - 1) / grid;
     if (sa.nblk * (nmine < 3 ? 3 : nmine) > F3_MAX_STEPS) return MSST_ERR_UNSUPPORTED;
     int rc = fwd3_attrs();
     if (rc) return rc;
     ProfScope ps(K_BLOCK_FWD, st);
     const size_t smem = sizeof(Fwd3Smem);
-    if (a.half) {
-        if (a.drop.thr) hipLaunchKernelGGL((block_fwd_rs_kernel<true, true, true>), dim3(grid), dim3(512), smem, st, sa);
-        else hipLaunchKernelGGL((block_fwd_rs_kernel<false, true, true>), dim3(grid), dim3(512), smem, st, sa);
-    } else {
-        if (a.drop.thr) hipLaunchKernelGGL((block_fwd_rs_kernel<true, true, false>), dim3(grid), dim3(512), smem, st, sa);
-        else hipLaunchKernelGGL((block_fwd_rs_kernel<false, true, false>), dim3(grid), dim3(512), smem, st, sa);
-    }
+    auto go = [&](auto drop_, auto half_, auto live_) {
+        hipLaunchKernelGGL((block_fwd_rs_kernel<decltype(drop_)::value, true, decltype(half_)::value, decltype(live_)::value>), dim3(grid), dim3(512), smem, st, sa);
+    };
+    f3_dispatch(a.drop.thr != 0, a.half != 0, a.tl.live != nullptr, go);
     return (int)hipGetLastError();
 }
 
@@ -889,13 +936,10 @@
     int rc = fwd3_attrs();
     if (rc) return rc;
     ProfScope ps(K_BLOCK_FWD, st);
-    if (a.half) {
-        if (a.drop.thr) hipLaunchKernelGGL((block_fwd_rs_kernel<true, false, true>), dim3(grid), dim3(512), smem, st, a);
-        else hipLaunchKernelGGL((block_fwd_rs_kernel<false, false, true>), dim3(grid), dim3(512), smem, st, a);
-    } else {
-        if (a.drop.thr) hipLaunchKernelGGL((block_fwd_rs_kernel<true, false, false>), dim3(grid), dim3(512), smem, st, a);
-        else hipLaunchKernelGGL((block_fwd_rs_kernel<false, false, false>), dim3(grid), dim3(512), smem, st, a);
-    }
+    auto go = [&](auto drop_, auto half_, auto live_) {
+        hipLaunchKernelGGL((block_fwd_rs_kernel<decltype(drop_)::value, false, decltype(half_)::value, decltype(live_)::value>), dim3(grid), dim3(512), smem, st, a);
+    };
+    f3_dispatch(a.drop.thr != 0, a.half != 0, a.tl.live != nullptr, go);
     return (int)hipGetLastError();
 }
 
diff --git a/maskedsst_amd/csrc/msst_kernels.h b/maskedsst_amd/csrc/msst_kernels.h
--- a/maskedsst_amd/csrc/msst_kernels.h
+++ b/maskedsst_amd/csrc/msst_kernels.h
@@ -23,6 +23,13 @@
     const float* ln1_g; const float* ln1_b; const float* bo;
     const float* ln2_g; const float* ln2_b; const float* b1; const float* b2;
     const void* wqkv32; const void* woutT32; const void* wqkvT32;
+};
+
+struct TileLists {
+    const int* live = nullptr;
+    const int* dead = nullptr;
+    int nlive = 0, ndead = 0;
+    int zero_y = 0;
 };
 
 struct BlockArgs {
@@ -40,6 +47,7 @@
     int dbg;
     unsigned long long* stamps;
     Drop drop;
+    TileLists tl;
 };
 
 #define MSST_MAX_STACK 16
@@ -158,6 +166,7 @@
     int* queue;
     const float* lse;
     int lse_renorm;
+    TileLists tl;
 };
 
 struct Ln1BwdArgs {
@@ -303,6 +312,7 @@
 int launch_block_bwd_attn(const AttnBwdArgs& a, int nchunk, int prec, hipStream_t st, int* nparts);
 int launch_block_bwd_attn_r3(const AttnBwdArgs& a, int nchunk, hipStream_t st);
 int launch_block_bwd_attn_r4(const AttnBwdArgs& a, int nchunk, hipStream_t st);
+int block_bwd_attn_live_max_steps();
 int launch_block_bwd_ln1(const Ln1BwdArgs& a, int grid, int prec, hipStream_t st);
 int launch_block_bwd_ln1mlp(const LnMlpArgs& a, int grid, hipStream_t st);
 int launch_tokenize_bwd(const TokBwdArgs& a, int nchunk, hipStream_t st);
diff --git a/maskedsst_amd/engine.py b/maskedsst_amd/engine.py
--- a/maskedsst_amd/engine.py
+++ b/maskedsst_amd/engine.py
@@ -6,7 +6,7 @@
 import torch
 
 from . import _lib
-from ._lib import (MsstBlockWeights, MsstBlockGrads, MsstPrepJob, PREC_BF16, PREC_F32, MODE_SPATIAL,
+from ._lib import (MsstBlockWeights, MsstBlockGrads, MsstPrepJob, MsstTileLists, PREC_BF16, PREC_F32, MODE_SPATIAL,
                    MODE_SPECTRAL, MLP_SLAB, ATTN_SLAB, LN1_SLAB)
 from .flat import FlatParams
 
@@ -47,6 +47,50 @@
 
 def _stream():
     return ctypes.c_void_p(torch.cuda.current_stream().cuda_stream)
+
+
+def live_dead_tiles(idx, N, TS):
+    ix = np.asarray(idx)
+    B = ix.shape[0]
+    nseq = B * N
+    ntiles = -(-nseq // TS)
+    need = np.zeros(ntiles * TS, dtype=bool)
+    need[(np.arange(B, dtype=np.int64)[:, None] * N + ix % N).ravel()] = True
+    alive = need.reshape(ntiles, TS).any(axis=1)
+    return np.flatnonzero(alive).astype(np.int32), np.flatnonzero(~alive).astype(np.int32)
+
+
+def chunk_walk_list(live, ntiles, nchunk):
+    live = np.asarray(live, dtype=np.int32)
+    nc = max(1, min(int(nchunk), int(ntiles)))
+    c = live % nc
+    order = np.argsort(c, kind="stable")
+    cs = c[order]
+    rank = np.empty(live.shape[0], dtype=np.int64)
+    rank[order] = np.arange(live.shape[0]) - np.searchsorted(cs, cs, side="left")
+    walk = np.full(((int(rank.max()) + 1) if live.shape[0] else 1, nc), ntiles, dtype=np.int32)
+    walk[rank, c] = live
+    return walk.ravel()
+
+
+class _TileSkip:
+
+    def __init__(self, buf, ntiles, nlive, ndead, nwalk, nc, queue):
+        self.buf, self.ntiles, self.nlive, self.ndead, self.nwalk, self.nc, self.queue = buf, ntiles, nlive, ndead, nwalk, nc, queue
+
+    def _lists(self, live_off, nlive, zero_y):
+        t = MsstTileLists()
+        t.struct_bytes = ctypes.sizeof(MsstTileLists)
+        t.nlive, t.ndead, t.zero_y = nlive, self.ndead, int(zero_y)
+        t.live = self.buf.data_ptr() + 4 * live_off
+        t.dead = self.buf.data_ptr() + 4 * self.ntiles
+        return t
+
+    def fwd(self, zero_y):
+        return self._lists(0, self.nlive, zero_y)
+
+    def bwd(self):
+        return self._lists(2 * self.ntiles, self.nwalk, 0)
 
 
 def _p(t):
@@ -363,7 +407,7 @@
                 min(chunk, total - win0), S, P, emb_drop[0], emb_drop[1], _stream()), "msst_tokenize_scene_fwd_train")
         return out
 
-    def blocks_fwd(self, x0, save=True, drop=(0.0, 0)):
+    def blocks_fwd(self, x0, save=True, drop=(0.0, 0), skip=None):
         acts = [x0]
         x1s = []
         flags = _kernel_flags()
@@ -380,12 +424,19 @@
             while i1 < len(layers) and layers[i1][0] == layers[i0][0] and i1 - i0 < 16:
                 i1 += 1
             use = stacked and (want_stack == "1" or self._tiles_per_workgroup(layers[i0][0], x0.shape[0]) <= STACK_MAX_TILES)
-            if use and self._fwd_stack(acts, x1s, i0, i1, save, drop, x1_bf16, want_lse):
+            sk = skip if (skip is not None and layers[i0][0] == "spectral" and i1 == len(layers)) else None
+            if use and self._fwd_stack(acts, x1s, i0, i1, save, drop, x1_bf16, want_lse, sk):
                 self.fwd_launch_blocks.append(i1 - i0)
             else:
                 for i in range(i0, i1):
-                    self._fwd_block(acts, x1s, i, save, drop, x1_bf16, want_lse, flags)
+                    self._fwd_block(acts, x1s, i, save, drop, x1_bf16, want_lse, flags, sk, i == len(layers) - 1)
                 self.fwd_launch_blocks += [1] * (i1 - i0)
+            if sk is not None:
+                for t in x1s[i0:i1]:
+                    if getattr(t, "_msst_xn", None) is None or not getattr(t, "_msst_rstd", False) or t.dtype != torch.bfloat16:
+                        raise RuntimeError("a spectral block walked tile lists without saving bf16 x1 rows, LN1 rows and rstd: the "
+                                           "backward of its dead tiles would read undefined rows")
+                    t._msst_skip = sk
             i0 = i1
         return acts, x1s
 
@@ -426,7 +477,7 @@
         x1._msst_rstd = bool(wrote & _lib.SAVED_RSTD) and x1._msst_lse is not None
         x1._msst_half = bool(self.fwd_half)
 
-    def _fwd_block(self, acts, x1s, i, save, drop, x1_bf16, want_lse, flags):
+    def _fwd_block(self, acts, x1s, i, save, drop, x1_bf16, want_lse, flags, skip=None, last=False):
         x = acts[-1]
         B = x.shape[0]
         S, N, H = self.S, self.N, self.enc.heads
@@ -439,16 +490,19 @@
         if xn is not None and want_lse:
             lse = torch.empty(int(self.lib.msst_block_lse_floats(mode, B, S, N, H)), dtype=torch.float32, device=x.device)
         wrote = ctypes.c_int(0)
-        _lib.check(self.lib.msst_block_fwd(ctypes.byref(self._bw[i]), _p(x), _p(y), _p(x1), mode, B, S, N, H,
-                                           self.prec | flags | (_lib.X1_BF16 if x1_bf16 else 0) | self._half_flag(flags), self.max_grid, drop[0], drop[1], i, _p(xn), _p(lse),
-                                           ctypes.byref(wrote), _stream()),
-                   "msst_block_fwd")
+        args = (ctypes.byref(self._bw[i]), _p(x), _p(y), _p(x1), mode, B, S, N, H,
+                self.prec | flags | (_lib.X1_BF16 if x1_bf16 else 0) | self._half_flag(flags), self.max_grid, drop[0], drop[1], i, _p(xn), _p(lse),
+                ctypes.byref(wrote))
+        if skip is None:
+            _lib.check(self.lib.msst_block_fwd(*args, _stream()), "msst_block_fwd")
+        else:
+            _lib.check(self.lib.msst_block_fwd_live(*args, ctypes.byref(skip.fwd(last)), _stream()), "msst_block_fwd_live")
         if x1 is not None:
             self._attach_saved(x1, wrote.value, xn, lse)
         acts.append(y)
         x1s.append(x1)
 
-    def _fwd_stack(self, acts, x1s, i0, i1, save, drop, x1_bf16, want_lse):
+    def _fwd_stack(self, acts, x1s, i0, i1, save, drop, x1_bf16, want_lse, skip=None):
         x0 = acts[-1]
         B = x0.shape[0]
         S, N, H = self.S, self.N, self.enc.heads
@@ -468,9 +522,12 @@
         def arr(ts):
             return VP(*[t.data_ptr() for t in ts]) if ts is not None else None
         wrote = ctypes.c_int(0)
-        rc = self.lib.msst_block_fwd_stack(wv, n, _p(x0), arr(ys), arr(x1), arr(xn), arr(lse), mode, B, S, N, H,
-                                           self.prec | (_lib.X1_BF16 if x1_bf16 else 0) | self._half_flag(0), self.max_grid, drop[0], drop[1], i0,
-                                           ctypes.byref(wrote), _stream())
+        args = (wv, n, _p(x0), arr(ys), arr(x1), arr(xn), arr(lse), mode, B, S, N, H,
+                self.prec | (_lib.X1_BF16 if x1_bf16 else 0) | self._half_flag(0), self.max_grid, drop[0], drop[1], i0, ctypes.byref(wrote))
+        if skip is None:
+            rc = self.lib.msst_block_fwd_stack(*args, _stream())
+        else:
+            rc = self.lib.msst_block_fwd_stack_live(*args, ctypes.byref(skip.fwd(True)), _stream())
         if rc == -2:
             return False
         _lib.check(rc, "msst_block_fwd_stack")
@@ -629,15 +686,21 @@
         chain = (self.prec == PREC_BF16 and _kernel_flags() == 0 and all(getattr(t, "_msst_xn", None) is not None for t in x1s)
                  and nparts <= 4 and os.environ.get("MSST_BWD_CHAIN", "1") != "0" and self.enc.depth > 0
                  and ntok * 384 < 2 ** 31 - 16 and nparts * ntok * 192 < 2 ** 31 - 16)
+        skip = getattr(x1s[-1], "_msst_skip", None) if len(x1s) else None
         ln1_from_xn = (chain and x1_bf16 and os.environ.get("MSST_LN1_XN", "1") != "0"
-                       and all(getattr(t, "_msst_rstd", False) for t in x1s) and self.ln1_xn_ok())
+                       and all(getattr(t, "_msst_rstd", False) for t in x1s) and (skip is not None or self.ln1_xn_ok()))
         self.last_bwd_ln1_from_xn = bool(ln1_from_xn)
+        self.last_bwd_skipped_tiles = skip.ndead if skip is not None else 0
+        if skip is not None and not ln1_from_xn:
+            raise RuntimeError("the forward skipped dead spectral tiles, but the chained bf16 backward with MSST_LN1_FROM_XN is no longer "
+                               "selected (MSST_BWD_CHAIN / MSST_LN1_XN / MSST_DBG changed between forward and backward?): every "
+                               "other backward reads block inputs the forward never wrote")
         if chain:
             return self._blocks_bwd_chained(acts, x1s, dy, drop, ws,
-                                            (_lib.X1_BF16 if x1_bf16 else 0) | (_lib.LN1_FROM_XN if ln1_from_xn else 0))
+                                            (_lib.X1_BF16 if x1_bf16 else 0) | (_lib.LN1_FROM_XN if ln1_from_xn else 0), skip)
         return self._blocks_bwd_unchained(acts, x1s, dy, drop, ws)
 
-    def _blocks_bwd_chained(self, acts, x1s, dy, drop, ws, x1flags):
+    def _blocks_bwd_chained(self, acts, x1s, dy, drop, ws, x1flags, skip=None):
         B = dy.shape[0]
         S, N, H = self.S, self.N, self.enc.heads
         dev = dy.device
@@ -648,6 +711,9 @@
             if getattr(self, "_queue_ws", None) is None or self._queue_ws.device != dev:
                 self._queue_ws = torch.zeros(64, dtype=torch.int32, device=dev)
             queue = self._queue_ws
+        if skip is not None and (skip.queue != (queue is not None) or skip.nc != min(self.attn_chunks, skip.ntiles)):
+            raise RuntimeError("attn_chunks / the tile queue changed between the forward that built the attention backward's walk "
+                               "list and its backward")
         last = len(layers) - 1
         dx0 = torch.empty_like(dy)
         null_w = ctypes.POINTER(MsstBlockWeights)()
@@ -663,15 +729,18 @@
             prev = i > 0
             x1 = x1s[i]
             slab_i = slab[(last - i) * nslab_r:] if defer else slab
-            _lib.check(self.lib.msst_block_bwd_chain(
+            args = (
                 ctypes.byref(self._bw[i]), ctypes.byref(self._bg[i]),
                 ctypes.byref(self._bw[i - 1]) if prev else null_w, ctypes.byref(self._bg[i - 1]) if prev else null_g,
                 _p(acts[i]), _p(x1), _p(x1s[i - 1]) if prev else _p(None), _p(dy) if i == last else _p(None),
                 _p(None) if prev else _p(dx0), _p(dx1), _p(part), _p(slab_i), self.grid_rows, self.attn_chunks, _MODE[sname],
                 B, S, N, H, self.prec | x1flags | (_lib.LSE_RENORM if getattr(x1, "_msst_half", False) else 0) |
                 (_lib.BWD_DEFER_REDUCE if defer else 0), drop[0], drop[1], i, _p(x1._msst_xn), _p(getattr(x1, "_msst_lse", None)), _p(dab),
-                1 if i == last else 0, _p(queue), _stream()),
-                "msst_block_bwd_chain")
+                1 if i == last else 0, _p(queue))
+            if skip is not None and getattr(x1, "_msst_skip", None) is skip:
+                _lib.check(self.lib.msst_block_bwd_chain_live(*args, ctypes.byref(skip.bwd()), _stream()), "msst_block_bwd_chain_live")
+            else:
+                _lib.check(self.lib.msst_block_bwd_chain(*args, _stream()), "msst_block_bwd_chain")
             if not defer:
                 self._fire(f"{sname}.{l}")
             elif i == 0 or layers[i - 1][0] != sname:
@@ -839,16 +908,52 @@
         bm = bool_mask.cpu().numpy() if torch.is_tensor(bool_mask) else np.asarray(bool_mask)
         ix = idx.cpu().numpy() if torch.is_tensor(idx) else np.asarray(idx)
         ptr, pos = inverse_csr(ix, T)
-        mask_u8, idx32, csr_ptr, csr_pos = self._upload(dev, bm.astype(np.uint8), ix.astype(np.int32), ptr, pos)
         names = [n for n, _ in self.trainable()]
         params = [p for _, p in self.trainable()]
-        if not torch.is_grad_enabled() or not (img.requires_grad or any(p.requires_grad for p in params)):
+        train = torch.is_grad_enabled() and (img.requires_grad or any(p.requires_grad for p in params))
+        plan = self._skip_dead_plan(ix) if train else None
+        up = self._upload(dev, bm.astype(np.uint8), ix.astype(np.int32), ptr, pos, *(() if plan is None else (plan[0],)))
+        mask_u8, idx32, csr_ptr, csr_pos = up[:4]
+        if not train:
             self.prep_weights()
             x0 = self.tokenize(img, mask_u8)
             acts, _ = self.blocks_fwd(x0, save=False, drop=self.dropout_state())
             loss, _, _ = self.head_fwd(acts[-1], img, idx32)
             return loss
-        return _SimMIMLossFn.apply(self, names, self.dropout_state(), img, mask_u8, idx32, csr_ptr, csr_pos, *params)
+        skip = self._skip_from_plan(plan, up[4] if plan is not None else None)
+        return _SimMIMLossFn.apply(self, names, self.dropout_state(), skip, img, mask_u8, idx32, csr_ptr, csr_pos, *params)
+
+    def skip_dead_static_ok(self, B):
+        env = os.environ.get
+        layers = self._layers()
+        H = int(self.enc.heads)
+        ntok = B * self.S * self.N
+        return (env("MSST_SKIP_DEAD", "1") != "0" and len(layers) >= 2 and layers[-1][0] == "spectral" and layers[0][0] != "spectral"
+                and self._role_split(_kernel_flags()) and H // 2 <= 4
+                and all(env(k, "1") != "0" for k in ("MSST_X1_BF16", "MSST_LSE", "MSST_BWD_CHAIN", "MSST_LN1_XN"))
+                and ntok * 384 < 2 ** 31 - 16 and (H // 2) * ntok * 192 < 2 ** 31 - 16
+                and B * self.N <= 500 * (64 // self.S) * max(1, min(self.attn_chunks, B * self.N // (64 // self.S))))
+
+    @staticmethod
+    def _skip_from_plan(plan, buf):
+        return _TileSkip(buf, *plan[1:]) if (plan is not None and plan[3] > 0) else None
+
+    def _skip_dead_plan(self, ix):
+        B = ix.shape[0]
+        if not self.skip_dead_static_ok(B):
+            return None
+        ntiles = int(self.lib.msst_block_tiles(MODE_SPECTRAL, B, self.S, self.N))
+        live, dead = live_dead_tiles(ix, self.N, 64 // self.S)
+        assert live.shape[0] + dead.shape[0] == ntiles
+        nc = min(self.attn_chunks, ntiles)
+        queue = bool(self.tile_queue or os.environ.get("MSST_TILE_QUEUE", "0") == "1")
+        compact = queue or os.environ.get("MSST_SKIP_DEAD", "1") == "2"
+        walk = live if compact else chunk_walk_list(live, ntiles, nc)
+        buf = np.full(3 * ntiles + nc, ntiles, dtype=np.int32)
+        buf[:live.shape[0]] = live
+        buf[ntiles:ntiles + dead.shape[0]] = dead
+        buf[2 * ntiles:2 * ntiles + walk.shape[0]] = walk
+        return buf, ntiles, int(live.shape[0]), int(dead.shape[0]), int(walk.shape[0]), nc, queue
 
     def _block_param_names(self):
         return [n for n, _ in self.trainable() if n.startswith(("spatial.", "spectral."))]
@@ -1086,10 +1191,12 @@
 class _SimMIMLossFn(torch.autograd.Function):
 
     @staticmethod
-    def forward(ctx, eng, names, drop, img, mask_u8, idx32, csr_ptr, csr_pos, *params):
+    def forward(ctx, eng, names, drop, skip, img, mask_u8, idx32, csr_ptr, csr_pos, *params):
         eng.prep_weights()
         x0 = eng.tokenize(img, mask_u8)
-        acts, x1s = eng.blocks_fwd(x0, save=True, drop=drop)
+        if skip is not None and not eng.ln1_xn_ok():
+            skip = None
+        acts, x1s = eng.blocks_fwd(x0, save=True, drop=drop, skip=skip)
         ctx.drop = drop
         loss, dpred, _ = eng.head_fwd(acts[-1], img, idx32)
         ctx.eng = eng
@@ -1102,17 +1209,17 @@
         eng = ctx.eng
         img, mask_u8, csr_ptr, csr_pos, acts, x1s, dpred = ctx.stash
         ctx.stash = None
-        needs = ctx.needs_input_grad[8:]
+        needs = ctx.needs_input_grad[9:]
         _refuse_accumulation(eng, ctx.names, needs)
         gout = gout.contiguous().float()
         dy = eng.head_bwd(acts[-1], dpred, csr_ptr, csr_pos, gout)
         dx0 = eng.blocks_bwd(acts, x1s, dy, drop=ctx.drop)
         dimg = None
-        if ctx.needs_input_grad[3]:
+        if ctx.needs_input_grad[4]:
             dimg = eng.tokenize_input_bwd(img, mask_u8, dx0, eng.head_bwd_target(dpred, csr_ptr, csr_pos, gout))
         if any(needs):
             eng.tokenize_bwd(img, mask_u8, dx0)
-        return (None, None, None, dimg) + (None,) * 4 + _grad_views(eng, ctx.names, needs)
+        return (None, None, None, None, dimg) + (None,) * 4 + _grad_views(eng, ctx.names, needs)
 
 
 def _refuse_accumulation(eng, names, needs=None):
```

Result: no change. 11140 samples/s (median of 6 runs) (+0.7%).
